# openGemini/openGemini

Hardware: NVIDIA B200
Metric: decoded+aggregated rows/s (higher is better)
Workload: dtype f64

## Files before the change

opengemini_b200/csrc/agg_kernels.cuh:

```cuda
#pragma once
#include "agg_ops.cuh"
#include "decode.cuh"
#include "internal.h"

namespace ogpu {

#define OG_NO_BUCKET 0xFFFFFFFFu

struct DirP {
    const uint8_t *data;
    const uint64_t *page_off;
    const uint32_t *page_len;
    const uint32_t *seg_series, *seg_rows, *series_seg_begin;
    const int64_t *seg_tmin, *seg_tmax;
    uint32_t n_segments, n_columns;
};

struct ChunkP {
    uint32_t series_begin, series_end;
    uint32_t seg_begin, seg_end;
    Tri cells[OG_MAX_CALLS];
    uint32_t nb;
    Tri edges[OG_MAX_CALLS];
    uint32_t *edge_bucket;
    Tri gcells[OG_MAX_CALLS];
    uint32_t gc_cols, gc_edge0, gc_col0;
    uint32_t J;
    int *err;
    int *flags;
};

__device__ __forceinline__ size_t cell_idx(const ChunkP &ch, uint32_t series, uint32_t b) { return (size_t)(series - ch.series_begin) * ch.nb + b; }

__device__ __forceinline__ void report_err(int *err, int code, uint32_t seg) {
    if (atomicCAS(&err[0], 0, code) == 0) err[1] = (int)seg;
}

__device__ __forceinline__ void store_part(const Tri &a, size_t i, const Part &p) {
    a.val[i] = p.v; a.ok[i] = (uint8_t)p.ok;
    if (a.tim) a.tim[i] = p.t;
}
__device__ __forceinline__ Part load_part(const Tri &a, size_t i) {
    Part p; p.ok = a.ok[i]; p.v = a.val[i]; p.t = a.tim ? a.tim[i] : 0; return p;
}
__device__ __forceinline__ void store_cell(const ChunkP &ch, int call, uint32_t series, uint32_t b, const Part &p) {
    store_part(ch.cells[call], cell_idx(ch, series, b), p);
    ch.flags[0] = 1;
}

struct LastTime { int64_t last; int unsorted = 0; __device__ __forceinline__ void operator()(uint32_t i, int64_t t) { if (i && t < last) unsorted = 1; last = t; } };

__global__ void k_validate(DirP d, const int32_t *col_types, uint32_t *seg_rows, unsigned long long *totals ,
                           uint32_t *max_rows, int *err) {
    uint32_t seg = blockIdx.x * blockDim.x + threadIdx.x;
    if (seg >= d.n_segments) return;
    size_t ti = (size_t)d.n_columns * d.n_segments + seg;
    TimeDesc t;
    int rc = parse_time_page(d.data + d.page_off[ti], d.page_len[ti], t);
    if (rc == D_OK && t.rows == 0) rc = D_CORRUPT;
    if (rc == D_OK) {
        LastTime lt; lt.last = t.t0;
        if (t.kind == 0) lt.last = (int64_t)((uint64_t)t.t0 + (uint64_t)(t.rows - 1) * t.delta);
        else rc = decode_time_values(t, lt);
        if (rc == D_OK && (t.t0 < d.seg_tmin[seg] || lt.last > d.seg_tmax[seg] || lt.last < t.t0 || lt.unsorted)) rc = D_CORRUPT;
    }
    if (rc != D_OK) { report_err(err, rc, seg); seg_rows[seg] = 0; return; }
    seg_rows[seg] = t.rows;
    unsigned long long bytes = d.page_len[ti];
    for (uint32_t c = 0; c < d.n_columns; c++) {
        size_t pi = (size_t)c * d.n_segments + seg;
        uint32_t len = d.page_len[pi];
        if (len == 0) continue;
        bytes += len;
        PageHdr h;
        rc = parse_field_header(d.data + d.page_off[pi], len, col_types[c], t.rows, h);
        if (rc == D_OK && h.rows != t.rows) rc = D_CORRUPT;
        if (rc == D_OK && !h.one_row && h.nil_count < h.rows) {
            if (h.block_len < 1) rc = D_CORRUPT;
            else {
                int tag = __ldg(h.block) >> 4, ty = col_types[c];
                if (ty == OG_TYPE_FLOAT) rc = (tag == 0 || tag == 3 || tag == 4 || tag == 5) ? D_OK : (tag == 1 || tag == 2 || tag == 6) ? D_UNSUPPORTED : D_CORRUPT;
                else if (ty == OG_TYPE_INT) rc = (tag == 1 || tag == 2 || tag == 4) ? D_OK : tag == 3 ? D_UNSUPPORTED : D_CORRUPT;
                else if (ty == OG_TYPE_BOOL) rc = tag == 1 ? D_OK : D_CORRUPT;
                else if (ty == OG_TYPE_STRING) rc = D_OK;
                else rc = D_UNSUPPORTED;
            }
        }
        if (rc != D_OK) { report_err(err, rc, seg); return; }
    }
    atomicAdd(&totals[0], (unsigned long long)t.rows);
    atomicAdd(&totals[1], bytes);
    atomicMax(max_rows, t.rows);
    if (t.kind != 0 && t.kind != 3) atomicAdd(&totals[2], 1ull);
}

__global__ void k_fill_seg_series(const uint32_t *series_seg_begin, uint32_t n_series, uint32_t *seg_series) {
    uint32_t s = blockIdx.x;
    if (s >= n_series) return;
    for (uint32_t g = series_seg_begin[s] + threadIdx.x; g < series_seg_begin[s + 1]; g += blockDim.x) seg_series[g] = s;
}

struct TileP {
    uint32_t tile_begin, tile_end, R;
    uint32_t S;
    uint64_t *vals[OG_MAX_COLS];
    uint8_t *okb[OG_MAX_COLS];
    int64_t *times;
    uint8_t *keep;
};

struct ExpandEmit {
    uint64_t *out; uint8_t *okb; const PageHdr *h; uint32_t row; size_t stride;
    __device__ __forceinline__ void operator()(uint32_t, uint64_t bits) {
        while (row < h->rows && !hdr_row_valid(*h, row)) { out[row * stride] = 0; okb[row * stride] = 0; row++; }
        if (row < h->rows) { out[row * stride] = bits; okb[row * stride] = 1; row++; }
    }
};
struct TimeStore { int64_t *out; size_t stride; __device__ __forceinline__ void operator()(uint32_t i, int64_t t) { out[i * stride] = t; } };

__global__ void k_decode_tile(DirP d, QueryP q, TileP tp, int *err) {
    uint32_t seg = tp.tile_begin + blockIdx.x * blockDim.x + threadIdx.x;
    if (seg >= tp.tile_end) return;
    uint32_t slot = blockIdx.y;
    const size_t base = seg - tp.tile_begin, S = tp.S;
    uint32_t rows = d.seg_rows[seg];
    if (slot == q.n_cols) {
        size_t ti = (size_t)d.n_columns * d.n_segments + seg;
        TimeDesc t;
        int rc = parse_time_page(d.data + d.page_off[ti], d.page_len[ti], t);
        if (rc == D_OK) { TimeStore ts{tp.times + base, S}; rc = decode_time_values(t, ts); }
        if (rc != D_OK) report_err(err, rc, seg);
        return;
    }
    int col = q.col_index[slot], type = q.col_type[slot];
    size_t pi = (size_t)col * d.n_segments + seg;
    uint64_t *out = tp.vals[slot] + base; uint8_t *okb = tp.okb[slot] + base;
    uint32_t len = d.page_len[pi];
    if (len == 0) { for (uint32_t i = 0; i < rows; i++) { out[i * S] = 0; okb[i * S] = 0; } return; }
    PageHdr h;
    int rc = parse_field_header(d.data + d.page_off[pi], len, type, rows, h);
    if (rc == D_OK) {
        ExpandEmit em{out, okb, &h, 0, S};
        rc = decode_block(type, h, em);
        for (uint32_t i = em.row; i < rows; i++) { out[i * S] = 0; okb[i * S] = 0; }
    }
    if (rc != D_OK) report_err(err, rc, seg);
}

__device__ __forceinline__ bool term_pass(const FilterP &f, uint64_t raw) {
    if (f.type == OG_TYPE_FLOAT || (f.type == OG_TYPE_INT && f.const_is_float)) {
        double v = f.type == OG_TYPE_FLOAT ? u2d(raw) : (double)(int64_t)raw;
        double c = f.const_is_float ? f.fval : (double)f.ival;
        switch (f.op) {
        case OG_OP_LT: return !(v >= c);
        case OG_OP_LTE: return !(v > c);
        case OG_OP_GT: return !(v <= c);
        case OG_OP_GTE: return !(v < c);
        case OG_OP_EQ: return !(v != c);
        default: return !(v == c);
        }
    }
    int64_t v = f.type == OG_TYPE_BOOL ? (int64_t)(raw != 0) : (int64_t)raw, c = f.ival;
    switch (f.op) {
    case OG_OP_LT: return !(v >= c);
    case OG_OP_LTE: return !(v > c);
    case OG_OP_GT: return !(v <= c);
    case OG_OP_GTE: return !(v < c);
    case OG_OP_EQ: return !(v != c);
    default: return !(v == c);
    }
}

__global__ void k_filter_tile(DirP d, QueryP q, TileP tp) {
    size_t idx = (size_t)blockIdx.x * blockDim.x + threadIdx.x;
    size_t total = (size_t)tp.S * tp.R;
    if (idx >= total) return;
    uint32_t row = (uint32_t)(idx / tp.S), sl = (uint32_t)(idx % tp.S);
    if (sl >= tp.tile_end - tp.tile_begin) return;
    if (row >= d.seg_rows[tp.tile_begin + sl]) { tp.keep[idx] = 0; return; }
    int64_t t = tp.times[idx];
    bool keep = t >= q.tmin && t <= q.tmax;
    if (keep && q.n_filter) {
        uint32_t stack = 0; int sp = 0;
        for (uint32_t i = 0; i < q.n_filter; i++) {
            const FilterP &f = q.filter[i];
            if (f.kind == OG_F_TERM) {
                bool pass = tp.okb[f.col_slot][idx] && term_pass(f, tp.vals[f.col_slot][idx]);
                stack |= (uint32_t)pass << sp; sp++;
            } else {
                uint32_t b = (stack >> (sp - 1)) & 1, a = (stack >> (sp - 2)) & 1;
                uint32_t r = f.kind == OG_F_AND ? (a & b) : (a | b);
                sp -= 2; stack &= ~(3u << sp); stack |= r << sp; sp++;
            }
        }
        keep = stack & 1;
    }
    tp.keep[idx] = keep;
}

__device__ __forceinline__ void emit_window(const QueryP &q, const ChunkP &ch, uint32_t seg, uint32_t series, uint32_t b,
                                            bool is_head, bool is_tail, int call, const Part &p) {
    if (is_head) store_part(ch.edges[call], 2 * (size_t)(seg - ch.seg_begin), p);
    else if (is_tail) store_part(ch.edges[call], 2 * (size_t)(seg - ch.seg_begin) + 1, p);
    else if (p.ok) store_cell(ch, call, series, b, p);
}

__global__ void k_window_reduce(DirP d, QueryP q, TileP tp, ChunkP ch) {
    uint32_t sl = blockIdx.x * blockDim.x + threadIdx.x;
    uint32_t seg = tp.tile_begin + sl;
    if (seg >= tp.tile_end) return;
    const uint32_t rows = d.seg_rows[seg], series = d.seg_series[seg];
    const size_t S = tp.S, e = 2 * (size_t)(seg - ch.seg_begin);
    Part parts[OG_MAX_CALLS];
    uint32_t cur_b = OG_NO_BUCKET, head_b = OG_NO_BUCKET; bool head_done = false;
    int64_t we = 0;
    auto flush = [&](bool final) {
        if (cur_b == OG_NO_BUCKET) return;
        for (uint32_t c = 0; c < q.n_calls; c++) {
            if (!head_done) store_part(ch.edges[c], e, parts[c]);
            else if (final) store_part(ch.edges[c], e + 1, parts[c]);
            else if (parts[c].ok) store_cell(ch, (int)c, series, cur_b, parts[c]);
        }
        if (!head_done) { head_done = true; head_b = cur_b; }
    };
    for (uint32_t r = 0; r < rows; r++) {
        const size_t ix = (size_t)r * S + sl;
        const int64_t t = tp.times[ix];
        if (t < q.tmin) continue;
        if (t > q.tmax) break;
        if (cur_b == OG_NO_BUCKET || t >= we) {
            flush(false);
            cur_b = bucket_of(t, q.start, q.interval);
            if (cur_b >= q.n_buckets) { report_err(ch.err, D_CORRUPT, seg); cur_b = OG_NO_BUCKET; break; }
            we = q.start + (int64_t)(cur_b + 1) * q.interval;
#pragma unroll
            for (uint32_t c = 0; c < OG_MAX_CALLS; c++) parts[c] = part_empty();
        }
        if (!tp.keep[ix]) continue;
#pragma unroll
        for (uint32_t c = 0; c < OG_MAX_CALLS; c++) {
            if (c >= q.n_calls) break;
            const CallP &cp = q.calls[c];
            if (tp.okb[cp.col_slot][ix]) acc_row(cp.func, cp.type, parts[c], tp.vals[cp.col_slot][ix], t);
        }
    }
    flush(true);
    ch.edge_bucket[e] = head_b;
    ch.edge_bucket[e + 1] = (head_b == OG_NO_BUCKET || cur_b == head_b) ? OG_NO_BUCKET : cur_b;
}

struct EdgeRuns { uint32_t hb, tb, s_end; bool head_leader; };
__device__ __forceinline__ EdgeRuns edge_runs(const DirP &d, const ChunkP &ch, uint32_t seg, uint32_t series) {
    EdgeRuns r;
    const uint32_t s_first = d.series_seg_begin[series];
    r.s_end = d.series_seg_begin[series + 1];
    const uint32_t *eb = ch.edge_bucket;
    const size_t e = 2 * (size_t)(seg - ch.seg_begin);
    r.hb = eb[e]; r.tb = eb[e + 1];
    r.head_leader = true;
    if (r.hb != OG_NO_BUCKET && seg > s_first) {
        const size_t pe = e - 2;
        const uint32_t pb = eb[pe + 1] != OG_NO_BUCKET ? eb[pe + 1] : eb[pe];
        if (pb != OG_NO_BUCKET && pb == r.hb) r.head_leader = false;
    }
    return r;
}
__device__ __forceinline__ Part edge_stitch(const QueryP &q, const ChunkP &ch, const EdgeRuns &r, uint32_t seg, int which, uint32_t c) {
    const CallP &cp = q.calls[c];
    const uint32_t *eb = ch.edge_bucket;
    const size_t e = 2 * (size_t)(seg - ch.seg_begin);
    const uint32_t b = which == 0 ? r.hb : r.tb;
    Part acc = load_part(ch.edges[c], e + which);
    if (which == 1 || r.tb == OG_NO_BUCKET) {
        for (uint32_t nx = seg + 1; nx < r.s_end; nx++) {
            const size_t ne = 2 * (size_t)(nx - ch.seg_begin);
            if (eb[ne] != b) break;
            acc = series_merge(cp.func, cp.type, acc, load_part(ch.edges[c], ne));
            if (eb[ne + 1] != OG_NO_BUCKET) break;
        }
    }
    return acc;
}

__global__ void k_fix_edges(DirP d, QueryP q, ChunkP ch) {
    uint32_t seg = ch.seg_begin + blockIdx.x * blockDim.x + threadIdx.x;
    if (seg >= ch.seg_end) return;
    const uint32_t series = d.seg_series[seg];
    const EdgeRuns r = edge_runs(d, ch, seg, series);
    if (r.hb == OG_NO_BUCKET) return;
    for (int which = 0; which < 2; which++) {
        if (which == 0 && !r.head_leader) continue;
        if (which == 1 && r.tb == OG_NO_BUCKET) continue;
        const uint32_t b = which == 0 ? r.hb : r.tb;
        if (b >= q.n_buckets) { report_err(ch.err, D_CORRUPT, seg); continue; }
        for (uint32_t c = 0; c < q.n_calls; c++) {
            const Part acc = edge_stitch(q, ch, r, seg, which, c);
            if (acc.ok) store_cell(ch, (int)c, series, b, acc);
        }
    }
}

__device__ __forceinline__ Part shfl_xor_part(const Part &p, int o, bool with_time) {
    Part r; r.v = __shfl_xor_sync(0xffffffffu, p.v, o); r.ok = __shfl_xor_sync(0xffffffffu, p.ok, o);
    r.t = with_time ? __shfl_xor_sync(0xffffffffu, p.t, o) : 0;
    return r;
}
__device__ __forceinline__ Part warp_fold(int func, int type, bool multi, Part p, bool with_time) {
#pragma unroll
    for (int o = 16; o; o >>= 1) { const Part other = shfl_xor_part(p, o, with_time); group_update(func, type, multi, p, other); }
    return p;
}
__device__ __forceinline__ bool call_has_time(const QueryP &q, uint32_t c) { return q.calls[c].func >= OG_AGG_MIN && !(q.multi && q.calls[c].func <= OG_AGG_MAX); }
__device__ __forceinline__ int call_ftype(const QueryP &q, uint32_t c) { return q.calls[c].func == OG_AGG_COUNT ? OG_TYPE_INT : q.calls[c].type; }

__global__ void k_fix_edges_fold(DirP d, QueryP q, ChunkP ch) {
    const uint32_t w = (blockIdx.x * blockDim.x + threadIdx.x) >> 5, lane = threadIdx.x & 31;
    const uint32_t n_blk = (ch.series_end - ch.series_begin + 31) / 32;
    if (w >= n_blk * ch.J) return;
    const uint32_t blk = w / ch.J, j = w % ch.J;
    const uint32_t series = ch.series_begin + blk * 32 + lane;
    const bool in = series < ch.series_end;
    const uint32_t seg = in ? d.series_seg_begin[series] + j : 0;
    EdgeRuns r; r.hb = r.tb = OG_NO_BUCKET; r.head_leader = false; r.s_end = 0;
    if (in) r = edge_runs(d, ch, seg, series);
    const uint32_t gcol = ch.gc_edge0 + ch.series_begin / 32 + blk - ch.gc_col0;
    for (int which = 0; which < 2; which++) {
        const bool has = r.hb != OG_NO_BUCKET && (which == 0 ? r.head_leader : r.tb != OG_NO_BUCKET);
        const uint32_t b = which == 0 ? r.hb : r.tb;
        const uint32_t hm = __ballot_sync(0xffffffffu, has);
        if (hm == 0) continue;
        const int leader = __ffs(hm) - 1;
        const uint32_t bL = __shfl_sync(0xffffffffu, b, leader);
        const bool unif = __all_sync(0xffffffffu, !has || b == bL) && bL < q.n_buckets;
        if (!unif && has && b >= q.n_buckets) { report_err(ch.err, D_CORRUPT, seg); continue; }
        for (uint32_t c = 0; c < q.n_calls; c++) {
            Part acc = part_empty();
            if (has) acc = edge_stitch(q, ch, r, seg, which, c);
            if (unif) {
                acc = warp_fold(q.calls[c].func, call_ftype(q, c), q.multi != 0, acc, call_has_time(q, c));
                if ((int)lane == leader && acc.ok) store_part(ch.gcells[c], (size_t)bL * ch.gc_cols + gcol, acc);
            } else if (has && acc.ok) store_cell(ch, (int)c, series, b, acc);
        }
    }
}

struct GroupP {
    const uint32_t *grp_begin;
    const uint32_t *grp_series;
    uint32_t n_groups;
    Tri dense[OG_MAX_CALLS];
};

__global__ void k_merge_groups(QueryP q, ChunkP ch, GroupP gp) {
    if (ch.flags[0] == 0) return;
    size_t idx = (size_t)blockIdx.x * blockDim.x + threadIdx.x;
    size_t total = (size_t)gp.n_groups * q.n_buckets;
    if (idx >= total) return;
    uint32_t g = (uint32_t)(idx / q.n_buckets), b = (uint32_t)(idx % q.n_buckets);
    uint32_t lo = gp.grp_begin[g], hi = gp.grp_begin[g + 1];
    {
        uint32_t a = lo, z = hi;
        while (a < z) { uint32_t m = (a + z) >> 1; if (gp.grp_series[m] < ch.series_begin) a = m + 1; else z = m; }
        lo = a;
    }
    if (lo >= hi || gp.grp_series[lo] >= ch.series_end) return;
    {
        const uint32_t c = blockIdx.y;
        const CallP &cp = q.calls[c];
        Part acc = load_part(gp.dense[c], idx);
        const Tri cells = ch.cells[c];
        constexpr int U = 16;
        for (uint32_t i = lo; i < hi; i += U) {
            uint32_t okv[U]; uint64_t vv[U]; int64_t tt[U];
#pragma unroll
            for (int u = 0; u < U; u++) {
                uint32_t ii = i + u;
                uint32_t s = ii < hi ? gp.grp_series[ii] : 0xffffffffu;
                bool in = s < ch.series_end;
                size_t ci = in ? cell_idx(ch, s, b) : 0;
                okv[u] = in ? cells.ok[ci] : 0;
                vv[u] = okv[u] ? cells.val[ci] : 0;
                tt[u] = (okv[u] && cells.tim) ? cells.tim[ci] : 0;
            }
#pragma unroll
            for (int u = 0; u < U; u++) {
                if (!okv[u]) continue;
                Part p; p.ok = 1; p.v = vv[u]; p.t = tt[u];
                group_update(cp.func, cp.out_type == OG_TYPE_INT && cp.func == OG_AGG_COUNT ? OG_TYPE_INT : cp.type, q.multi != 0, acc, p);
            }
        }
        store_part(gp.dense[c], idx, acc);
    }
}

__global__ void k_merge_per_series(QueryP q, ChunkP ch, GroupP gp) {
    const uint32_t c = blockIdx.y;
    const size_t n = (size_t)(ch.series_end - ch.series_begin) * q.n_buckets;
    const size_t i = (size_t)blockIdx.x * blockDim.x + threadIdx.x;
    if (i >= n) return;
    const CallP &cp = q.calls[c];
    const int ftype = cp.out_type == OG_TYPE_INT && cp.func == OG_AGG_COUNT ? OG_TYPE_INT : cp.type;
    const uint32_t b = (uint32_t)(i % q.n_buckets);
    Part p; p.ok = ch.cells[c].ok[i]; p.v = p.ok ? ch.cells[c].val[i] : 0; p.t = (p.ok && ch.cells[c].tim) ? ch.cells[c].tim[i] : 0;
    Part a; a.v = 0; a.ok = 0; a.t = q.multi ? 0 : q.start + (int64_t)b * q.interval;
    group_update(cp.func, ftype, q.multi != 0, a, p);
    store_part(gp.dense[c], (size_t)ch.series_begin * q.n_buckets + i, a);
}

#define OG_MERGE_SB 256u
__global__ void __launch_bounds__(128) k_merge_all_blocks(QueryP q, ChunkP ch, GroupP gp) {
    if (ch.flags[0] == 0) return;
    const uint32_t b = blockIdx.x * blockDim.x + threadIdx.x, blk = blockIdx.y, c = blockIdx.z;
    if (b >= q.n_buckets) return;
    const uint32_t nS = ch.series_end - ch.series_begin;
    const uint32_t s0 = blk * OG_MERGE_SB, s1 = min(nS, s0 + OG_MERGE_SB);
    const int func = q.calls[c].func, ftype = call_ftype(q, c);
    const bool multi = q.multi != 0;
    const Tri cells = ch.cells[c];
    Part acc = part_empty();
    constexpr int U = 8;
    for (uint32_t s = s0; s < s1; s += U) {
        uint32_t okv[U]; uint64_t vv[U]; int64_t tt[U];
#pragma unroll
        for (int u = 0; u < U; u++) {
            const bool in = s + u < s1;
            const size_t ci = in ? (size_t)(s + u) * ch.nb + b : 0;
            okv[u] = in ? cells.ok[ci] : 0;
            vv[u] = okv[u] ? cells.val[ci] : 0;
            tt[u] = (okv[u] && cells.tim) ? cells.tim[ci] : 0;
        }
#pragma unroll
        for (int u = 0; u < U; u++) {
            if (!okv[u]) continue;
            Part p; p.ok = 1; p.v = vv[u]; p.t = tt[u];
            group_update(func, ftype, multi, acc, p);
        }
    }
    if (acc.ok) store_part(ch.gcells[c], (size_t)b * ch.gc_cols + blk, acc);
}

__global__ void k_merge_folded(QueryP q, ChunkP ch, GroupP gp) {
    const uint32_t b = (blockIdx.x * blockDim.x + threadIdx.x) >> 5, lane = threadIdx.x & 31, c = blockIdx.y;
    if (b >= q.n_buckets) return;
    const int func = q.calls[c].func, ftype = call_ftype(q, c);
    const bool wt = call_has_time(q, c), multi = q.multi != 0;
    const Tri g = ch.gcells[c];
    Part acc = part_empty();
    const size_t row = (size_t)b * ch.gc_cols;
    for (uint32_t col = lane; col < ch.gc_cols; col += 32) {
        if (!g.ok[row + col]) continue;
        Part p; p.ok = 1; p.v = g.val[row + col]; p.t = wt ? g.tim[row + col] : 0;
        group_update(func, ftype, multi, acc, p);
    }
    acc = warp_fold(func, ftype, multi, acc, wt);
    if (lane == 0 && acc.ok) {
        Part a = load_part(gp.dense[c], b);
        group_update(func, ftype, multi, a, acc);
        store_part(gp.dense[c], b, a);
    }
}

__global__ void k_init_dense(QueryP q, GroupP gp) {
    size_t idx = (size_t)blockIdx.x * blockDim.x + threadIdx.x;
    size_t total = (size_t)gp.n_groups * q.n_buckets;
    if (idx >= total) return;
    uint32_t b = (uint32_t)(idx % q.n_buckets);
    for (uint32_t c = 0; c < q.n_calls; c++) {
        gp.dense[c].val[idx] = 0; gp.dense[c].ok[idx] = 0;
        if (gp.dense[c].tim) gp.dense[c].tim[idx] = q.multi ? 0 : q.start + (int64_t)b * q.interval;
    }
}

__global__ void k_merge_dense(QueryP q, GroupP mine, GroupP other) {
    size_t idx = (size_t)blockIdx.x * blockDim.x + threadIdx.x;
    size_t total = (size_t)mine.n_groups * q.n_buckets;
    if (idx >= total) return;
    for (uint32_t c = 0; c < q.n_calls; c++) {
        const CallP &cp = q.calls[c];
        Part a = load_part(mine.dense[c], idx), p = load_part(other.dense[c], idx);
        group_update(cp.func, cp.func == OG_AGG_COUNT ? OG_TYPE_INT : cp.type, q.multi != 0, a, p);
        store_part(mine.dense[c], idx, a);
    }
}

}
```

opengemini_b200/csrc/agg_ops.cuh:

```cuda
#pragma once
#include <cstdint>

#include "../../include/ogpu.h"

namespace ogpu {

__device__ __forceinline__ double u2d(uint64_t u) { return __longlong_as_double((long long)u); }
__device__ __forceinline__ uint64_t d2u(double d) { return (uint64_t)__double_as_longlong(d); }

__device__ __forceinline__ bool v_lt(int type, uint64_t a, uint64_t b) {
    if (type == OG_TYPE_FLOAT) return u2d(a) < u2d(b);
    if (type == OG_TYPE_INT) return (int64_t)a < (int64_t)b;
    return a != b && !a;
}
__device__ __forceinline__ bool v_gt(int type, uint64_t a, uint64_t b) {
    if (type == OG_TYPE_FLOAT) return u2d(a) > u2d(b);
    if (type == OG_TYPE_INT) return (int64_t)a > (int64_t)b;
    return a != b && a;
}
__device__ __forceinline__ bool v_eq(int type, uint64_t a, uint64_t b) { return type == OG_TYPE_FLOAT ? u2d(a) == u2d(b) : a == b; }
__device__ __forceinline__ bool v_le(int type, uint64_t a, uint64_t b) {
    if (type == OG_TYPE_FLOAT) return u2d(a) <= u2d(b);
    if (type == OG_TYPE_INT) return (int64_t)a <= (int64_t)b;
    return a == b || !a;
}
__device__ __forceinline__ bool v_ge(int type, uint64_t a, uint64_t b) {
    if (type == OG_TYPE_FLOAT) return u2d(a) >= u2d(b);
    if (type == OG_TYPE_INT) return (int64_t)a >= (int64_t)b;
    return a == b || a;
}

struct Part { uint64_t v; int64_t t; uint32_t ok; };

__device__ __forceinline__ void acc_row(int func, int type, Part &p, uint64_t v, int64_t t) {
    switch (func) {
    case OG_AGG_COUNT: p.v += 1; p.ok = 1; break;
    case OG_AGG_SUM:
        if (type == OG_TYPE_FLOAT) p.v = d2u(u2d(p.v) + u2d(v)); else p.v += v;
        p.ok = 1; break;
    case OG_AGG_MIN:
        if (!p.ok || v_gt(type, p.v, v)) { p.v = v; p.t = t; }
        p.ok = 1; break;
    case OG_AGG_MAX:
        if (!p.ok || v_lt(type, p.v, v)) { p.v = v; p.t = t; }
        p.ok = 1; break;
    case OG_AGG_FIRST: if (!p.ok) { p.v = v; p.t = t; p.ok = 1; } break;
    default: p.v = v; p.t = t; p.ok = 1; break;
    }
}
__device__ __forceinline__ Part part_empty() { Part p; p.v = 0; p.t = 0; p.ok = 0; return p; }

__device__ __forceinline__ Part series_merge(int func, int type, const Part &prev, const Part &curr) {
    if (!curr.ok) return prev;
    if (!prev.ok) return curr;
    Part r = prev;
    switch (func) {
    case OG_AGG_COUNT: r.v = prev.v + curr.v; break;
    case OG_AGG_SUM: r.v = type == OG_TYPE_FLOAT ? d2u(u2d(prev.v) + u2d(curr.v)) : prev.v + curr.v; break;
    case OG_AGG_MIN: if (v_lt(type, curr.v, prev.v)) r = curr; break;
    case OG_AGG_MAX: if (v_gt(type, curr.v, prev.v)) r = curr; break;
    case OG_AGG_FIRST: break;
    default: r = curr; break;
    }
    return r;
}

__device__ __forceinline__ void group_update(int func, int type, bool multi, Part &a, const Part &p) {
    if (!p.ok) return;
    switch (func) {
    case OG_AGG_COUNT: a.v = (uint64_t)((int64_t)p.v + (int64_t)a.v); a.ok = 1; return;
    case OG_AGG_SUM:
        a.v = type == OG_TYPE_FLOAT ? d2u(u2d(p.v) + u2d(a.v)) : p.v + a.v; a.ok = 1; return;
    case OG_AGG_MIN:
    case OG_AGG_MAX: {
        bool is_min = func == OG_AGG_MIN;
        if (multi) {
            if ((is_min ? v_le(type, a.v, p.v) : v_ge(type, a.v, p.v)) && a.ok) return;
            a.v = p.v; a.ok = 1; return;
        }
        if ((is_min ? v_lt(type, a.v, p.v) : v_gt(type, a.v, p.v)) && a.ok) return;
        bool t_le = type == OG_TYPE_FLOAT ? (__longlong_as_double(a.t) <= __longlong_as_double(p.t)) : (a.t <= p.t);
        if (v_eq(type, a.v, p.v) && t_le && a.ok) return;
        a = p; a.ok = 1; return;
    }
    default: {
        bool is_first = func == OG_AGG_FIRST;
        int64_t t1 = a.t, t2 = p.t;
        if (is_first ? (t1 > t2) : (t1 < t2)) { a = p; a.ok = 1; return; }
        if (a.ok && (is_first ? (t2 > t1) : (t2 < t1))) return;
        if (a.ok && v_ge(type, a.v, p.v)) return;
        a = p; a.ok = 1; return;
    }
    }
}

__device__ __forceinline__ uint32_t bucket_of(int64_t t, int64_t start, int64_t interval) {
    return (uint32_t)((uint64_t)(t - start) / (uint64_t)interval);
}

}
```

opengemini_b200/csrc/api.cu:

```cuda
#include <algorithm>
#include <cstdarg>
#include <cstdio>
#include <cstring>
#include <numeric>

#include "agg_kernels.cuh"
#include "fused.cuh"
#include "il_build.cuh"
#include "fused_multi.cuh"
#include "fused_cols.cuh"
#include "snappy_load.cuh"
#include <cub/device/device_scan.cuh>
#include <cub/device/device_radix_sort.cuh>
#include "internal.h"

namespace ogpu {

static thread_local char g_err[512] = "";
void set_error(const char *fmt, ...) {
    va_list ap; va_start(ap, fmt); vsnprintf(g_err, sizeof g_err, fmt, ap); va_end(ap);
}
int cuda_fail(cudaError_t e, const char *what, const char *file, int line) {
    set_error("CUDA error %d (%s) at %s:%d: %s", (int)e, cudaGetErrorString(e), file, line, what);
    return OG_E_CUDA;
}
static int g_device = -1;
cudaError_t dev_mem_info(size_t *free_b, size_t *total_b) {
    cudaError_t e = cudaMemGetInfo(free_b, total_b);
    if (e != cudaSuccess) return e;
    cudaMemPool_t pool; uint64_t reserved = 0, used = 0; int dev = 0;
    if (cudaGetDevice(&dev) == cudaSuccess && cudaDeviceGetDefaultMemPool(&pool, dev) == cudaSuccess &&
        cudaMemPoolGetAttribute(pool, cudaMemPoolAttrReservedMemCurrent, &reserved) == cudaSuccess &&
        cudaMemPoolGetAttribute(pool, cudaMemPoolAttrUsedMemCurrent, &used) == cudaSuccess && reserved > used) *free_b += (size_t)(reserved - used);
    else cudaGetLastError();
    return cudaSuccess;
}

static int map_dev_err(int code) {
    switch (code) {
    case D_UNSUPPORTED: return OG_E_UNSUPPORTED;
    case D_TYPE: return OG_E_TYPE;
    case D_WATCHDOG: return OG_E_CUDA;
    default: return OG_E_CORRUPT;
    }
}

template <class T> static int dalloc(T **p, size_t n) {
    *p = nullptr;
    if (n == 0) n = 1;
    cudaError_t e = dev_malloc((void **)p, n * sizeof(T));
    if (e != cudaSuccess) { set_error("cudaMalloc(%zu bytes) failed: %s", n * sizeof(T), cudaGetErrorString(e)); return e == cudaErrorMemoryAllocation ? OG_E_NOMEM : OG_E_CUDA; }
    return OG_OK;
}

static DirP make_dir(const og_shard *s) {
    DirP d;
    d.data = s->d_data; d.page_off = s->d_page_off; d.page_len = s->d_page_len; d.seg_series = s->d_seg_series;
    d.seg_rows = s->d_seg_rows; d.series_seg_begin = s->d_series_seg_begin; d.seg_tmin = s->d_tmin; d.seg_tmax = s->d_tmax;
    d.n_segments = s->n_segments; d.n_columns = s->n_columns;
    return d;
}

int shard_finalize(og_shard *s, bool scan_snappy) {
    int rc;
    s->il.resize(s->n_columns);
    if ((rc = dalloc(&s->d_seg_series, s->n_segments))) return rc;
    if ((rc = dalloc(&s->d_seg_rows, s->n_segments))) return rc;
    int32_t *d_types; unsigned long long *d_tot; uint32_t *d_max; int *d_err;
    if ((rc = dalloc(&d_types, s->n_columns))) return rc;
    if ((rc = dalloc(&d_tot, 3))) return rc;
    if ((rc = dalloc(&d_max, 1))) return rc;
    if ((rc = dalloc(&d_err, 2))) return rc;
    CU(cudaMemcpy(d_types, s->col_types.data(), s->n_columns * sizeof(int32_t), cudaMemcpyHostToDevice));
    CU(cudaMemset(d_tot, 0, 24)); CU(cudaMemset(d_max, 0, 4)); CU(cudaMemset(d_err, 0, 8));
    if (s->n_series) k_fill_seg_series<<<s->n_series, 128>>>(s->d_series_seg_begin, s->n_series, s->d_seg_series);
    if (s->n_segments && scan_snappy) {
        const size_t n_pages = (size_t)(s->n_columns + 1) * s->n_segments;
        uint32_t *tr_size; unsigned long long *d_cnt;
        if ((rc = dalloc(&tr_size, n_pages))) return rc;
        if ((rc = dalloc(&d_cnt, 3))) { dev_free(tr_size); return rc; }
        struct Free2 { void *a, *b; ~Free2() { dev_free(a); dev_free(b); } } f2{tr_size, d_cnt};
        CU(cudaMemset(d_cnt, 0, 24));
        k_snappy_scan<<<(s->n_segments + 127) / 128, 128>>>(make_dir(s), d_types, tr_size, d_cnt);
        unsigned long long cnt[3];
        CU(cudaMemcpy(cnt, d_cnt, 24, cudaMemcpyDeviceToHost));
        if (cnt[0]) {
            if (!s->owns_data) { set_error("shard has %llu Snappy pages: they are transcoded at open, which needs a library-owned copy of the data (do not pass OG_SHARD_DEVICE_DATA)", cnt[0]); return OG_E_UNSUPPORTED; }
            uint64_t *tr_off; void *tmp = nullptr; size_t tb = 0;
            if ((rc = dalloc(&tr_off, n_pages))) return rc;
            struct Free1 { void *a; ~Free1() { dev_free(a); } } f1{tr_off};
            CU(cub::DeviceScan::ExclusiveSum(nullptr, tb, tr_size, tr_off, (int)n_pages));
            CU(dev_malloc((void **)&tmp, tb ? tb : 1));
            struct Free3 { void *a; ~Free3() { dev_free(a); } } f3{tmp};
            CU(cub::DeviceScan::ExclusiveSum(tmp, tb, tr_size, tr_off, (int)n_pages));
            const uint64_t new_base = (s->data_len + 15) & ~15ull, new_len = new_base + cnt[2];
            uint8_t *nd;
            if ((rc = dalloc(&nd, (size_t)new_len + 1024))) return rc;
            CU(cudaMemcpy(nd, s->d_data, s->data_len, cudaMemcpyDeviceToDevice));
            CU(cudaMemset(nd + s->data_len, 0, new_len + 1024 - s->data_len));
            k_snappy_transcode<<<(unsigned)((n_pages + 127) / 128), 128>>>(make_dir(s), tr_size, tr_off, nd, new_base, s->d_page_off, s->d_page_len, d_err);
            CU(cudaGetLastError());
            CU(cudaDeviceSynchronize());
            dev_free(s->d_data); s->d_data = nd; s->data_len = new_len;
            s->snappy_pages = cnt[0]; s->snappy_bytes_in = cnt[1]; s->snappy_bytes_out = cnt[2];
        }
    }
    if (s->n_segments) k_validate<<<(s->n_segments + 127) / 128, 128>>>(make_dir(s), d_types, s->d_seg_rows, d_tot, d_max, d_err);
    CU(cudaGetLastError());
    unsigned long long tot[3]; int err[2]; uint32_t mx;
    CU(cudaMemcpy(tot, d_tot, 24, cudaMemcpyDeviceToHost));
    CU(cudaMemcpy(err, d_err, 8, cudaMemcpyDeviceToHost));
    CU(cudaMemcpy(&mx, d_max, 4, cudaMemcpyDeviceToHost));
    dev_free(d_types); dev_free(d_tot); dev_free(d_max); dev_free(d_err);
    if (err[0]) {
        set_error("segment %d: %s page (device validation code %d)", err[1], err[0] == D_UNSUPPORTED ? "unsupported codec in" : err[0] == D_TYPE ? "type mismatch in" : "corrupt", err[0]);
        return map_dev_err(err[0]);
    }
    s->n_rows = tot[0]; s->page_bytes = tot[1] - s->snappy_bytes_out + s->snappy_bytes_in;
    s->max_seg_rows = mx; s->irregular_time_pages = tot[2];
    return OG_OK;
}

}

using namespace ogpu;

extern "C" {

OG_API int og_device_count(void) { int n = 0; if (cudaGetDeviceCount(&n) != cudaSuccess) return 0; return n; }

OG_API int og_init(int device_ordinal) {
    int n = og_device_count();
    if (n <= 0) { set_error("no CUDA device visible: libogpu has no CPU path"); return OG_E_CUDA; }
    if (device_ordinal < 0 || device_ordinal >= n) { set_error("device ordinal %d out of range (%d devices)", device_ordinal, n); return OG_E_INVAL; }
    CU(cudaSetDevice(device_ordinal));
    CU(cudaFree(0));
    {
        cudaMemPool_t pool; uint64_t thr = ~0ull;
        if (cudaDeviceGetDefaultMemPool(&pool, device_ordinal) == cudaSuccess) cudaMemPoolSetAttribute(pool, cudaMemPoolAttrReleaseThreshold, &thr);
        else cudaGetLastError();
    }
    g_device = device_ordinal;
    return OG_OK;
}

OG_API const char *og_strerror(int st) {
    switch (st) {
    case OG_OK: return "ok";
    case OG_EOF: return "end of stream";
    case OG_E_INVAL: return "invalid argument";
    case OG_E_CUDA: return "CUDA failure or no device bound";
    case OG_E_NOMEM: return "out of device memory";
    case OG_E_UNSUPPORTED: return "unsupported codec or option on the GPU path";
    case OG_E_CORRUPT: return "corrupt page";
    case OG_E_ABORTED: return "query aborted";
    case OG_E_TYPE: return "column type mismatch";
    case OG_E_STATE: return "call sequence error";
    default: return "unknown status";
    }
}
OG_API const char *og_last_error(void) { return g_err; }
OG_API const char *og_version(void) { return "ogpu 0.2 (sm_100a)"; }
OG_API int og_release_cached_memory(void) {
    if (g_device < 0) return OG_OK;
    CU(cudaSetDevice(g_device));
    CU(cudaDeviceSynchronize());
    cudaMemPool_t pool;
    CU(cudaDeviceGetDefaultMemPool(&pool, g_device));
    CU(cudaMemPoolTrimTo(pool, 0));
    return OG_OK;
}

}
namespace ogpu {
int ensure_device() {
    if (g_device < 0) { int rc = og_init(0); if (rc != OG_OK) return rc; }
    else CU(cudaSetDevice(g_device));
    return OG_OK;
}
}
static int need_device() { return ogpu::ensure_device(); }
extern "C" {

OG_API void og_shard_close(og_shard *s) {
    if (!s) return;
    if (s->owns_data && s->d_data) dev_free(s->d_data);
    dev_free(s->d_series_seg_begin); dev_free(s->d_seg_series); dev_free(s->d_seg_rows); dev_free(s->d_tmin); dev_free(s->d_tmax);
    dev_free(s->d_page_off); dev_free(s->d_page_len); dev_free(s->d_sids);
    if (s->h_seg_buf) cudaFreeHost(s->h_seg_buf);
    if (s->d_seg_buf) dev_free(s->d_seg_buf);
    for (auto &c : s->il) {
        dev_free(c.words); dev_free(c.grp_off); dev_free(c.grp_rows); dev_free(c.grp_col); dev_free(c.ok); dev_free(c.lane_seg); dev_free(c.lane_rows);
        dev_free(c.lane_series); dev_free(c.lane_t0); dev_free(c.lane_dt); dev_free(c.gen_list);
    }
    delete s;
}

OG_API int og_shard_open(const og_shard_desc *d, og_shard **out) {
    if (!d || !out) { set_error("null argument"); return OG_E_INVAL; }
    *out = nullptr;
    int rc = need_device(); if (rc) return rc;
    if (d->n_columns > 64 || (d->n_segments && (!d->seg_tmin || !d->seg_tmax || !d->time_page_off || !d->time_page_len)) || (d->n_series && !d->series_seg_begin)) { set_error("bad shard descriptor"); return OG_E_INVAL; }
    for (uint32_t s = 0; s < d->n_series; s++) if (d->series_seg_begin[s] > d->series_seg_begin[s + 1]) { set_error("series_seg_begin not monotone at %u", s); return OG_E_INVAL; }
    if (d->n_series && d->series_seg_begin[d->n_series] != d->n_segments) { set_error("series_seg_begin[n_series] != n_segments"); return OG_E_INVAL; }
    og_shard *s = new og_shard;
    s->device = g_device; s->n_series = d->n_series; s->n_segments = d->n_segments; s->n_columns = d->n_columns;
    s->data_len = d->data_len;
    for (uint32_t c = 0; c < d->n_columns; c++) {
        s->col_types.push_back(d->columns[c].type);
        s->col_names.push_back(d->columns[c].name ? d->columns[c].name : "");
        if (d->columns[c].type != OG_TYPE_INT && d->columns[c].type != OG_TYPE_FLOAT && d->columns[c].type != OG_TYPE_BOOL && d->columns[c].type != OG_TYPE_STRING) {
            set_error("column %u: unknown column type %d", c, d->columns[c].type); delete s; return OG_E_UNSUPPORTED;
        }
    }
    s->sids.assign(d->sids, d->sids + d->n_series);
    s->h_series_seg_begin.assign(d->series_seg_begin, d->series_seg_begin + d->n_series + 1);
    size_t nseg = d->n_segments, ncol1 = (size_t)d->n_columns + 1;
    std::vector<uint64_t> off(ncol1 * nseg); std::vector<uint32_t> len(ncol1 * nseg);
    for (size_t c = 0; c < ncol1; c++) {
        const uint64_t *po = c < d->n_columns ? d->columns[c].page_off : d->time_page_off;
        const uint32_t *pl = c < d->n_columns ? d->columns[c].page_len : d->time_page_len;
        for (size_t g = 0; g < nseg; g++) {
            if (po[g] + pl[g] > d->data_len) { set_error("column %zu segment %zu: page [%llu,+%u) outside data (%llu bytes)", c, g, (unsigned long long)po[g], pl[g], (unsigned long long)d->data_len); delete s; return OG_E_INVAL; }
            off[c * nseg + g] = po[g]; len[c * nseg + g] = pl[g];
        }
    }
    s->tmin = INT64_MAX; s->tmax = INT64_MIN;
    for (uint32_t sr = 0; sr < d->n_series; sr++)
        for (uint32_t g = d->series_seg_begin[sr]; g < d->series_seg_begin[sr + 1]; g++) {
            if (d->seg_tmin[g] > d->seg_tmax[g] || (g > d->series_seg_begin[sr] && d->seg_tmin[g] <= d->seg_tmax[g - 1])) {
                set_error("series %u: segment %u is not time-ordered (only ordered TSSP files are supported)", sr, g); delete s; return OG_E_UNSUPPORTED;
            }
            s->tmin = std::min(s->tmin, d->seg_tmin[g]); s->tmax = std::max(s->tmax, d->seg_tmax[g]);
        }
#define TRY(x) do { rc = (x); if (rc) { og_shard_close(s); return rc; } } while (0)
#define TRYCU(x) do { cudaError_t e_ = (x); if (e_ != cudaSuccess) { rc = cuda_fail(e_, #x, __FILE__, __LINE__); og_shard_close(s); return rc; } } while (0)
    if (d->flags & OG_SHARD_DEVICE_DATA) { s->d_data = (uint8_t *)d->data; s->owns_data = false; }
    else {
        TRY(dalloc(&s->d_data, d->data_len + 1024));
        TRYCU(cudaMemcpy(s->d_data, d->data, d->data_len, cudaMemcpyHostToDevice));
        TRYCU(cudaMemset(s->d_data + d->data_len, 0, 1024));
    }
    TRY(dalloc(&s->d_series_seg_begin, (size_t)d->n_series + 1));
    TRY(dalloc(&s->d_tmin, nseg)); TRY(dalloc(&s->d_tmax, nseg));
    TRY(dalloc(&s->d_page_off, ncol1 * nseg)); TRY(dalloc(&s->d_page_len, ncol1 * nseg)); TRY(dalloc(&s->d_sids, (size_t)d->n_series));
    TRYCU(cudaMemcpy(s->d_series_seg_begin, d->series_seg_begin, ((size_t)d->n_series + 1) * 4, cudaMemcpyHostToDevice));
    TRYCU(cudaMemcpy(s->d_tmin, d->seg_tmin, nseg * 8, cudaMemcpyHostToDevice));
    TRYCU(cudaMemcpy(s->d_tmax, d->seg_tmax, nseg * 8, cudaMemcpyHostToDevice));
    TRYCU(cudaMemcpy(s->d_page_off, off.data(), off.size() * 8, cudaMemcpyHostToDevice));
    TRYCU(cudaMemcpy(s->d_page_len, len.data(), len.size() * 4, cudaMemcpyHostToDevice));
    TRYCU(cudaMemcpy(s->d_sids, d->sids, (size_t)d->n_series * 8, cudaMemcpyHostToDevice));
    TRY(shard_finalize(s, true));
    *out = s;
    return OG_OK;
}

OG_API int og_shard_info(const og_shard *s, uint64_t *n_series, uint64_t *n_segments, uint64_t *n_rows, uint64_t *page_bytes, int64_t *tmin, int64_t *tmax) {
    if (!s) return OG_E_INVAL;
    if (n_series) *n_series = s->n_series;
    if (n_segments) *n_segments = s->n_segments;
    if (n_rows) *n_rows = s->n_rows;
    if (page_bytes) *page_bytes = s->page_bytes;
    if (tmin) *tmin = s->tmin;
    if (tmax) *tmax = s->tmax;
    return OG_OK;
}

OG_API int og_shard_layout_get(const og_shard *s, og_shard_layout *out) {
    if (!s || !out) return OG_E_INVAL;
    out->data_len = s->data_len; out->n_series = s->n_series; out->n_segments = s->n_segments; out->n_columns = s->n_columns;
    return OG_OK;
}

OG_API int og_shard_export(const og_shard *s, uint8_t *data, uint64_t *sids, uint32_t *series_seg_begin, int64_t *seg_tmin,
                           int64_t *seg_tmax, uint64_t *page_off, uint32_t *page_len, int32_t *col_types) {
    if (!s) return OG_E_INVAL;
    CU(cudaSetDevice(s->device));
    size_t nseg = s->n_segments, ncol1 = (size_t)s->n_columns + 1;
    if (data) CU(cudaMemcpy(data, s->d_data, s->data_len, cudaMemcpyDeviceToHost));
    if (sids) memcpy(sids, s->sids.data(), s->sids.size() * 8);
    if (series_seg_begin) memcpy(series_seg_begin, s->h_series_seg_begin.data(), s->h_series_seg_begin.size() * 4);
    if (seg_tmin) CU(cudaMemcpy(seg_tmin, s->d_tmin, nseg * 8, cudaMemcpyDeviceToHost));
    if (seg_tmax) CU(cudaMemcpy(seg_tmax, s->d_tmax, nseg * 8, cudaMemcpyDeviceToHost));
    if (page_off) CU(cudaMemcpy(page_off, s->d_page_off, ncol1 * nseg * 8, cudaMemcpyDeviceToHost));
    if (page_len) CU(cudaMemcpy(page_len, s->d_page_len, ncol1 * nseg * 4, cudaMemcpyDeviceToHost));
    if (col_types) memcpy(col_types, s->col_types.data(), s->col_types.size() * 4);
    return OG_OK;
}

static const int64_t MIN_TIME = INT64_MIN + 2, MAX_TIME = INT64_MAX - 1;
static void window_of(int64_t interval, int64_t offset, int64_t tmin, int64_t tmax, int64_t t, int64_t *s, int64_t *e) {
    if (interval == 0) { *s = tmin; *e = tmax + 1; return; }
    t -= offset;
    int64_t dt = t % interval;
    if (dt < 0) dt += interval;
    int64_t st = ((int64_t)((uint64_t)MIN_TIME + (uint64_t)dt) >= t) ? MIN_TIME : t - dt;
    st += offset;
    int64_t d2 = interval - dt;
    int64_t en = (MAX_TIME - d2 <= t) ? MAX_TIME : t + d2;
    en += offset;
    *s = st; *e = en;
}

}
namespace { void free_plan(void *plan); }
extern "C" {
void og_query_free_merge_state(void *p);
OG_API void og_query_destroy(og_query *q) {
    if (!q) return;
    if (q->merge_state) og_query_free_merge_state(q->merge_state);
    free_plan(q->plan);
    for (void *p : q->scratch) dev_free(p);
    for (int c = 0; c < OG_MAX_CALLS; c++) { dev_free(q->dense[c].val); dev_free(q->dense[c].ok); dev_free(q->dense[c].tim); }
    dev_free(q->d_group_of_series);
    if (q->ev0) cudaEventDestroy(q->ev0);
    if (q->ev1) cudaEventDestroy(q->ev1);
    for (cudaEvent_t e : q->main_ev) cudaEventDestroy(e);
    if (q->stream) cudaStreamDestroy(q->stream);
    delete q;
}

OG_API int og_query_create(og_shard *s, const og_query_desc *d_in, og_query **out) {
    if (!s || !d_in || !out) { set_error("null argument"); return OG_E_INVAL; }
    *out = nullptr;
    og_query_desc d_clamped = *d_in;
    d_clamped.tmin = std::max(d_in->tmin, MIN_TIME); d_clamped.tmax = std::min(d_in->tmax, MAX_TIME);
    const og_query_desc *d = &d_clamped;
    CU(cudaSetDevice(s->device));
    if (d->n_calls == 0 || d->n_calls > OG_MAX_CALLS) { set_error("n_calls must be 1..%d", OG_MAX_CALLS); return OG_E_INVAL; }
    if (d->n_filter > OG_MAX_FILTER) { set_error("filter too long (max %d items)", OG_MAX_FILTER); return OG_E_INVAL; }
    if (d->interval < 0 || d->tmin > d->tmax) { set_error("bad interval or time range"); return OG_E_INVAL; }
    og_query *q = new og_query;
    q->sh = s; q->desc = *d;
    q->calls.assign(d->calls, d->calls + d->n_calls);
    if (d->n_filter) q->filter.assign(d->filter, d->filter + d->n_filter);
    q->desc.calls = q->calls.data(); q->desc.filter = q->filter.data();
    QueryP &p = q->qp;
    memset(&p, 0, sizeof p);
    auto slot_of = [&](int col) -> int {
        for (uint32_t i = 0; i < p.n_cols; i++) if (p.col_index[i] == col) return (int)i;
        if (p.n_cols >= OG_MAX_COLS) return -1;
        p.col_index[p.n_cols] = col; p.col_type[p.n_cols] = s->col_types[col];
        return (int)p.n_cols++;
    };
    for (uint32_t i = 0; i < d->n_calls; i++) {
        const og_call &c = d->calls[i];
        if (c.column < 0 || (uint32_t)c.column >= s->n_columns || c.func < OG_AGG_COUNT || c.func > OG_AGG_LAST) { set_error("call %u: bad column or function", i); delete q; return OG_E_INVAL; }
        int type = s->col_types[c.column];
        if (type == OG_TYPE_STRING && c.func != OG_AGG_COUNT) { set_error("call %u: only count() is pushed down for string columns (their values are never decoded on the GPU path)", i); delete q; return OG_E_UNSUPPORTED; }
        if (c.func == OG_AGG_SUM && type == OG_TYPE_BOOL) { set_error("sum() over a boolean column (unsupported sum iterator type, series_call_processor.go:140)"); delete q; return OG_E_INVAL; }
        int sl = slot_of(c.column);
        if (sl < 0) { set_error("too many distinct columns"); delete q; return OG_E_INVAL; }
        p.calls[i].func = c.func; p.calls[i].col_slot = sl; p.calls[i].type = type;
        p.calls[i].out_type = c.func == OG_AGG_COUNT ? OG_TYPE_INT : type;
    }
    p.n_calls = d->n_calls; p.multi = d->n_calls > 1;
    int sp = 0;
    for (uint32_t i = 0; i < d->n_filter; i++) {
        const og_filter_item &f = d->filter[i];
        FilterP &fp = p.filter[i];
        fp.kind = f.kind;
        if (f.kind == OG_F_TERM) {
            if (f.column < 0 || (uint32_t)f.column >= s->n_columns || f.op < OG_OP_LT || f.op > OG_OP_NEQ) { set_error("filter item %u: bad column or op", i); delete q; return OG_E_INVAL; }
            if (s->col_types[f.column] == OG_TYPE_STRING) { set_error("filter item %u: WHERE on a string column is not pushed down", i); delete q; return OG_E_UNSUPPORTED; }
            int sl = slot_of(f.column);
            if (sl < 0) { set_error("too many distinct columns"); delete q; return OG_E_INVAL; }
            fp.col_slot = sl; fp.op = f.op; fp.type = s->col_types[f.column]; fp.const_is_float = f.const_is_float; fp.fval = f.fval; fp.ival = f.ival;
            sp++;
        } else if (f.kind == OG_F_AND || f.kind == OG_F_OR) {
            if (sp < 2) { set_error("filter RPN underflow at item %u", i); delete q; return OG_E_INVAL; }
            sp--;
        } else { set_error("filter item %u: bad kind", i); delete q; return OG_E_INVAL; }
    }
    if (d->n_filter && sp != 1) { set_error("filter RPN does not reduce to one value"); delete q; return OG_E_INVAL; }
    p.n_filter = d->n_filter;
    int64_t gmin = std::max(d->tmin, s->tmin), gmax = std::min(d->tmax, s->tmax);
    if (gmin > gmax) gmin = gmax = d->tmin;
    if (d->flags & OG_Q_QUERY_GRID) {
        if (d_in->tmin <= MIN_TIME || d_in->tmax >= MAX_TIME) { set_error("OG_Q_QUERY_GRID needs a bounded time range"); delete q; return OG_E_INVAL; }
        gmin = d->tmin; gmax = d->tmax;
    }
    int64_t s0, e0, s1, e1;
    if (d->interval == 0) { s0 = gmin; e0 = gmax + 1; s1 = s0; e1 = e0; }
    else {
        window_of(d->interval, d->offset, d->tmin, d->tmax, gmin, &s0, &e0);
        window_of(d->interval, d->offset, d->tmin, d->tmax, gmax + 1, &s1, &e1);
    }
    p.tmin = d->tmin; p.tmax = d->tmax; p.start = s0; p.interval = e0 - s0;
    if (p.interval <= 0) { set_error("degenerate window"); delete q; return OG_E_INVAL; }
    uint64_t nb = d->interval ? (uint64_t)(e1 - s0) / (uint64_t)p.interval : 1;
    if (nb == 0 || nb > 0x7fffffffull) { set_error("query range yields %llu buckets", (unsigned long long)nb); delete q; return OG_E_INVAL; }
    p.n_buckets = (uint32_t)nb;
    q->n_groups = d->group_mode == OG_GROUP_ALL ? 1 : d->group_mode == OG_GROUP_PER_SERIES ? s->n_series : d->n_groups;
    if (d->group_mode == OG_GROUP_MAP) {
        if (!d->series_group || d->n_groups == 0) { set_error("OG_GROUP_MAP needs series_group and n_groups"); delete q; return OG_E_INVAL; }
        q->series_group.assign(d->series_group, d->series_group + s->n_series);
        for (uint32_t g : q->series_group) if (g >= d->n_groups) { set_error("series_group entry out of range"); delete q; return OG_E_INVAL; }
    } else if (d->group_mode != OG_GROUP_ALL && d->group_mode != OG_GROUP_PER_SERIES) { set_error("bad group_mode"); delete q; return OG_E_INVAL; }
    if (q->n_groups == 0) q->n_groups = 1;
    cudaError_t e = cudaStreamCreateWithFlags(&q->stream, cudaStreamNonBlocking);
    if (e != cudaSuccess) { delete q; return cuda_fail(e, "cudaStreamCreate", __FILE__, __LINE__); }
    cudaEventCreate(&q->ev0); cudaEventCreate(&q->ev1);
    *out = q;
    return OG_OK;
}

OG_API void og_query_abort(og_query *q) { if (q) q->aborted = 1; }

}
namespace {
struct Plan {
    ChunkP ch; TileP tp; GroupP gp;
    bool fused;
    bool cols;
    bool multi;
    bool fast;
    bool blockmerge;
    bool fold;
    int fm; bool times;
    IlP il;
    const og_shard::IlCol *ic;
};
void free_plan(void *plan) { delete (Plan *)plan; }
template <class T> int salloc(og_query *q, T **p, size_t n) { int rc = dalloc(p, n); if (rc == OG_OK) q->scratch.push_back(*p); return rc; }

template <int NC> void launch_fused(const DirP &d, const QueryP &p, const ChunkP &ch, const uint32_t *list, uint32_t n, cudaStream_t st) {
    if (n) k_fused_segment<NC><<<(n + 127) / 128, 128, 0, st>>>(d, p, ch, list, n);
}
template <int FM, bool TIMES> void launch_fast_t(bool fold, const IlP &il, uint32_t g0, uint32_t g1, const QueryP &p, const ChunkP &ch, cudaStream_t st) {
    constexpr uint32_t WPB = OG_FAST_THREADS / 32;
    dim3 grid((g1 - g0 + WPB - 1) / WPB), block(OG_FAST_THREADS);
    if (fold) k_fused_il<FM, TIMES, true><<<grid, block, WPB * il_acc_bytes(p.n_calls, TIMES), st>>>(p, ch, il, g0, g1);
    else k_fused_il<FM, TIMES, false><<<grid, block, 0, st>>>(p, ch, il, g0, g1);
}
void launch_fast(int fm, bool times, bool fold, const IlP &il, uint32_t g0, uint32_t g1, const QueryP &p, const ChunkP &ch, cudaStream_t st) {
    if (g1 <= g0) return;
    if (!times) {
        switch (fm) {
        case FM_SUM | FM_COUNT: return launch_fast_t<FM_SUM | FM_COUNT, false>(fold, il, g0, g1, p, ch, st);
        case FM_SUM | FM_COUNT | FM_MAX: return launch_fast_t<FM_SUM | FM_COUNT | FM_MAX, false>(fold, il, g0, g1, p, ch, st);
        case FM_SUM | FM_COUNT | FM_MIN | FM_MAX: return launch_fast_t<FM_SUM | FM_COUNT | FM_MIN | FM_MAX, false>(fold, il, g0, g1, p, ch, st);
        case FM_COUNT: return launch_fast_t<FM_COUNT, false>(fold, il, g0, g1, p, ch, st);
        default: break;
        }
    } else {
        switch (fm) {
        case FM_MAX | FM_COUNT: return launch_fast_t<FM_MAX | FM_COUNT, true>(fold, il, g0, g1, p, ch, st);
        case FM_MIN | FM_COUNT: return launch_fast_t<FM_MIN | FM_COUNT, true>(fold, il, g0, g1, p, ch, st);
        default: break;
        }
    }
    return launch_fast_t<63, true>(fold, il, g0, g1, p, ch, st);
}

template <int NCOL, int NCALL> void launch_multi_t(const QueryP &p, const DirP &d, const ChunkP &ch, uint32_t nseg, cudaStream_t st) {
    bool simple = true;
    for (uint32_t c = 0; c < p.n_calls; c++) simple &= p.calls[c].func == OG_AGG_COUNT || p.calls[c].func == OG_AGG_SUM;
    const unsigned gb = (nseg + 127) / 128;
    if (simple) k_fused_multi<NCOL, NCALL, true><<<gb, 128, 0, st>>>(d, p, ch);
    else k_fused_multi<NCOL, NCALL, false><<<gb, 128, 0, st>>>(d, p, ch);
}
template <int NCOL> void launch_multi_c(const QueryP &p, const DirP &d, const ChunkP &ch, uint32_t nseg, cudaStream_t st) {
    switch (p.n_calls) {
    case 1: return launch_multi_t<NCOL, 1>(p, d, ch, nseg, st);
    case 2: return launch_multi_t<NCOL, 2>(p, d, ch, nseg, st);
    case 3: return launch_multi_t<NCOL, 3>(p, d, ch, nseg, st);
    case 4: return launch_multi_t<NCOL, 4>(p, d, ch, nseg, st);
    case 5: return launch_multi_t<NCOL, 5>(p, d, ch, nseg, st);
    case 6: return launch_multi_t<NCOL, 6>(p, d, ch, nseg, st);
    case 7: return launch_multi_t<NCOL, 7>(p, d, ch, nseg, st);
    default: return launch_multi_t<NCOL, 8>(p, d, ch, nseg, st);
    }
}
void launch_cols(const QueryP &p, const DirP &d, const ChunkP &ch, uint32_t nseg, cudaStream_t st) {
    bool simple = true;
    for (uint32_t c = 0; c < p.n_calls; c++) simple &= p.calls[c].func == OG_AGG_COUNT || p.calls[c].func == OG_AGG_SUM;
    const unsigned gb = (nseg + 127) / 128;
    if (simple) k_fused_cols<true><<<gb, 128, 0, st>>>(d, p, ch);
    else k_fused_cols<false><<<gb, 128, 0, st>>>(d, p, ch);
}
void launch_multi(const QueryP &p, const DirP &d, const ChunkP &ch, uint32_t nseg, cudaStream_t st) {
    switch (p.n_cols) {
    case 1: return launch_multi_c<1>(p, d, ch, nseg, st);
    case 2: return launch_multi_c<2>(p, d, ch, nseg, st);
    case 3: return launch_multi_c<3>(p, d, ch, nseg, st);
    default: return launch_multi_c<4>(p, d, ch, nseg, st);
    }
}

struct TmpBufs { std::vector<void *> v; ~TmpBufs() { for (void *p : v) dev_free(p); } template <class T> int get(T **p, size_t n) { int rc = dalloc(p, n); if (rc == OG_OK) v.push_back(*p); return rc; } };

int ensure_il(og_shard *s, int col, cudaStream_t st) {
    std::lock_guard<std::mutex> lock(s->il_mu);
    if (s->il.size() != s->n_columns) s->il.resize(s->n_columns);
    og_shard::IlCol &ic = s->il[col];
    if (ic.state != 0) return OG_OK;
    ic.state = -1;
    if (s->n_segments == 0 || s->col_types[col] != OG_TYPE_FLOAT) return OG_OK;
    const uint32_t nseg = s->n_segments;
    uint32_t J = s->n_series ? s->h_series_seg_begin[1] - s->h_series_seg_begin[0] : 0;
    for (uint32_t i = 0; i < s->n_series && J; i++) if (s->h_series_seg_begin[i + 1] - s->h_series_seg_begin[i] != J) J = 0;
    const uint32_t n_super = J ? (s->n_series + OG_IL_SUPER - 1) / OG_IL_SUPER : 1;
    const uint64_t n_dom64 = J ? (uint64_t)n_super * J : 1;
    if (n_dom64 >= (1ull << 31)) return OG_OK;
    const uint32_t n_dom = (uint32_t)n_dom64;
    int rc;
    struct Ev { cudaEvent_t e = nullptr; Ev() { cudaEventCreate(&e); } ~Ev() { if (e) cudaEventDestroy(e); } } ev0, ev1;
    cudaEventRecord(ev0.e, st);
    TmpBufs tmp;
    IlScanOut so{};
    uint32_t *seg_words; uint64_t *keys2; uint32_t *vals2;
    if ((rc = dalloc(&ic.ok, (size_t)nseg))) return rc;
    so.ok = ic.ok;
    if ((rc = tmp.get(&seg_words, nseg)) || (rc = tmp.get(&so.seg_t0, nseg)) || (rc = tmp.get(&so.seg_dt, nseg)) || (rc = tmp.get(&so.keys, nseg)) ||
        (rc = tmp.get(&so.vals, nseg)) || (rc = tmp.get(&keys2, nseg)) || (rc = tmp.get(&vals2, nseg)) || (rc = tmp.get(&so.dom_cnt, n_dom))) return rc;
    so.seg_words = seg_words;
    CU(cudaMemsetAsync(so.dom_cnt, 0, (size_t)n_dom * 4, st));
    DirP d = make_dir(s);
    k_il_scan<<<(nseg + 255) / 256, 256, 0, st>>>(d, col, s->col_types[col], J, so);
    CU(cudaGetLastError());
    int dbits = 1; while ((1ull << dbits) < n_dom64 + 1) dbits++;
    {
        size_t tb = 0;
        CU(cub::DeviceRadixSort::SortPairs(nullptr, tb, so.keys, keys2, so.vals, vals2, (int)nseg, 0, (int)OG_IL_WORD_BITS + dbits, st));
        void *dtmp; if ((rc = tmp.get((uint8_t **)&dtmp, tb))) return rc;
        CU(cub::DeviceRadixSort::SortPairs(dtmp, tb, so.keys, keys2, so.vals, vals2, (int)nseg, 0, (int)OG_IL_WORD_BITS + dbits, st));
    }
    std::vector<uint32_t> dom_cnt(n_dom);
    CU(cudaMemcpyAsync(dom_cnt.data(), so.dom_cnt, (size_t)n_dom * 4, cudaMemcpyDeviceToHost, st));
    CU(cudaStreamSynchronize(st));
    std::vector<uint32_t> elem_first(n_dom), grp_first(n_dom);
    uint64_t n_elig = 0, ng64 = 0;
    for (uint32_t i = 0; i < n_dom; i++) { elem_first[i] = (uint32_t)n_elig; grp_first[i] = (uint32_t)ng64; n_elig += dom_cnt[i]; ng64 += (dom_cnt[i] + 31) / 32; }
    const uint32_t n_gen = nseg - (uint32_t)n_elig;
    if (n_gen) {
        if ((rc = dalloc(&ic.gen_list, (size_t)n_gen))) return rc;
        CU(cudaMemcpyAsync(ic.gen_list, vals2 + n_elig, (size_t)n_gen * 4, cudaMemcpyDeviceToDevice, st));
        ic.gen_host.resize(n_gen);
        CU(cudaMemcpyAsync(ic.gen_host.data(), vals2 + n_elig, (size_t)n_gen * 4, cudaMemcpyDeviceToHost, st));
        CU(cudaStreamSynchronize(st));
    }
    if (n_elig == 0) return OG_OK;
    const uint32_t ng = (uint32_t)ng64;
    ic.n_groups = ng; ic.J = J; ic.n_super = n_super; ic.cols_per_super = OG_IL_SUPER / 32 + 1;
    ic.super_grp_first.assign(n_super + 1, ng);
    for (uint32_t sp = 0; sp < n_super; sp++) ic.super_grp_first[sp] = grp_first[J ? sp * J : 0];
    uint32_t *d_elem_first, *d_grp_first;
    if ((rc = tmp.get(&d_elem_first, n_dom)) || (rc = tmp.get(&d_grp_first, n_dom))) return rc;
    CU(cudaMemcpyAsync(d_elem_first, elem_first.data(), (size_t)n_dom * 4, cudaMemcpyHostToDevice, st));
    CU(cudaMemcpyAsync(d_grp_first, grp_first.data(), (size_t)n_dom * 4, cudaMemcpyHostToDevice, st));
    const size_t n_slots = (size_t)ng * 32;
    if ((rc = dalloc(&ic.lane_seg, n_slots)) || (rc = dalloc(&ic.lane_rows, n_slots)) || (rc = dalloc(&ic.lane_series, n_slots)) ||
        (rc = dalloc(&ic.lane_t0, n_slots)) || (rc = dalloc(&ic.lane_dt, n_slots)) || (rc = dalloc(&ic.grp_col, (size_t)ng)) ||
        (rc = dalloc(&ic.grp_rows, (size_t)ng)) || (rc = dalloc(&ic.grp_off, (size_t)ng))) return rc;
    CU(cudaMemsetAsync(ic.lane_seg, 0xff, n_slots * 4, st));
    CU(cudaMemsetAsync(ic.lane_rows, 0, n_slots * 4, st));
    IlAssign as{};
    as.keys = keys2; as.segs = vals2; as.elem_first = d_elem_first; as.grp_first = d_grp_first;
    as.seg_words = seg_words; as.seg_t0 = so.seg_t0; as.seg_dt = so.seg_dt; as.ok = ic.ok;
    as.lane_seg = ic.lane_seg; as.lane_rows = ic.lane_rows; as.lane_series = ic.lane_series; as.grp_col = ic.grp_col; as.lane_t0 = ic.lane_t0; as.lane_dt = ic.lane_dt;
    as.n_elig = (uint32_t)n_elig; as.J = J; as.cols_per_super = ic.cols_per_super;
    k_il_assign<<<(unsigned)((n_elig + 255) / 256), 256, 0, st>>>(d, as);
    k_il_group_rows<<<(unsigned)((n_slots + 255) / 256), 256, 0, st>>>(ng, ic.lane_seg, seg_words, ic.grp_rows);
    CU(cudaGetLastError());
    std::vector<uint32_t> gw(ng); std::vector<uint64_t> go(ng);
    CU(cudaMemcpyAsync(gw.data(), ic.grp_rows, (size_t)ng * 4, cudaMemcpyDeviceToHost, st));
    CU(cudaStreamSynchronize(st));
    uint64_t total = 0;
    for (uint32_t g = 0; g < ng; g++) { go[g] = total; total += (uint64_t)gw[g] * 32; }
    size_t free_b = 0, total_b = 0;
    CU(dev_mem_info(&free_b, &total_b));
    size_t headroom = (size_t)8 << 30;
    if (const char *ov = getenv("OGPU_IL_HEADROOM_MB")) headroom = (size_t)atoll(ov) << 20;
    if (total * 4 + headroom > free_b || dev_malloc((void **)&ic.words, total * 4) != cudaSuccess) {
        cudaGetLastError(); ic.words = nullptr; ic.state = -2;
        return OG_OK;
    }
    CU(cudaMemcpyAsync(ic.grp_off, go.data(), (size_t)ng * 8, cudaMemcpyHostToDevice, st));
    k_il_repack<<<(unsigned)((n_slots + 127) / 128), 128, 0, st>>>(d, col, ic.ok, ic.lane_seg, ic.grp_off, ic.grp_rows, ng, ic.words);
    CU(cudaGetLastError());
    cudaEventRecord(ev1.e, st);
    CU(cudaStreamSynchronize(st));
    float ms = 0; cudaEventElapsedTime(&ms, ev0.e, ev1.e);
    ic.n_words = total; ic.build_ms = ms; ic.state = 1;
    return OG_OK;
}

int build_plan(og_query *q) {
    og_shard *s = q->sh;
    const QueryP &p = q->qp;
    cudaStream_t st = q->stream;
    int rc;
    Plan *pl = new Plan;
    memset((void *)pl, 0, sizeof *pl);
    q->plan = pl;
    size_t cells_dense = (size_t)q->n_groups * p.n_buckets;
    for (uint32_t c = 0; c < p.n_calls; c++) {
        bool sel = p.calls[c].func >= OG_AGG_MIN && !(p.multi && p.calls[c].func <= OG_AGG_MAX);
        if ((rc = dalloc(&q->dense[c].val, cells_dense))) return rc;
        if ((rc = dalloc(&q->dense[c].ok, cells_dense))) return rc;
        if (sel && (rc = dalloc(&q->dense[c].tim, cells_dense))) return rc;
    }
    std::vector<uint32_t> grp_begin(q->n_groups + 1, 0), grp_series(s->n_series);
    if (q->desc.group_mode == OG_GROUP_MAP) {
        for (uint32_t sr = 0; sr < s->n_series; sr++) grp_begin[q->series_group[sr] + 1]++;
        for (uint32_t g = 0; g < q->n_groups; g++) grp_begin[g + 1] += grp_begin[g];
        std::vector<uint32_t> cur(grp_begin.begin(), grp_begin.end() - 1);
        for (uint32_t sr = 0; sr < s->n_series; sr++) grp_series[cur[q->series_group[sr]]++] = sr;
    } else if (q->desc.group_mode == OG_GROUP_PER_SERIES) {
        for (uint32_t g = 0; g <= q->n_groups; g++) grp_begin[g] = std::min(g, s->n_series);
        std::iota(grp_series.begin(), grp_series.end(), 0u);
    } else { grp_begin[1] = s->n_series; std::iota(grp_series.begin(), grp_series.end(), 0u); }
    uint32_t *d_grp_begin, *d_grp_series;
    if ((rc = salloc(q, &d_grp_begin, grp_begin.size()))) return rc;
    if ((rc = salloc(q, &d_grp_series, grp_series.size()))) return rc;
    if ((rc = salloc(q, &q->d_err, 8))) return rc;
    CU(cudaMemcpyAsync(d_grp_begin, grp_begin.data(), grp_begin.size() * 4, cudaMemcpyHostToDevice, st));
    CU(cudaMemcpyAsync(d_grp_series, grp_series.data(), grp_series.size() * 4, cudaMemcpyHostToDevice, st));
    CU(cudaStreamSynchronize(st));
    pl->gp.grp_begin = d_grp_begin; pl->gp.grp_series = d_grp_series; pl->gp.n_groups = q->n_groups;
    for (uint32_t c = 0; c < p.n_calls; c++) pl->gp.dense[c] = q->dense[c];

    bool has_string = false;
    for (uint32_t k = 0; k < p.n_cols; k++) has_string |= p.col_type[k] == OG_TYPE_STRING;
    pl->fused = p.n_cols == 1 && p.n_filter == 0 && !has_string && !(q->desc.flags & OG_Q_NO_FUSED);
    const bool multi_ok = !pl->fused && (has_string || !(q->desc.flags & OG_Q_NO_FUSED));
    pl->cols = false;
    if (multi_ok && !(q->desc.flags & OG_Q_NO_FAST) && s->irregular_time_pages == 0 && s->max_seg_rows <= OG_COLS_MAXROWS &&
        (p.n_filter == 0 || (p.n_filter == 1 && p.filter[0].kind == OG_F_TERM)) && !getenv("OGPU_NO_COLS")) {
        pl->cols = true;
        for (uint32_t k = 0; k < p.n_cols; k++) {
            int n = 0;
            for (uint32_t c = 0; c < p.n_calls; c++) n += p.calls[c].col_slot == (int)k;
            if (n > OG_COLS_MAXMINE) pl->cols = false;
        }
    }
    if (has_string && !pl->cols && p.n_cols > OG_MULTI_MAXC) { set_error("a query that counts a string column may touch at most %d columns on this shard", OG_MULTI_MAXC); return OG_E_UNSUPPORTED; }
    pl->multi = pl->cols || (multi_ok && p.n_cols <= OG_MULTI_MAXC);
    q->path_used = pl->fused ? 1 : pl->cols ? 5 : pl->multi ? 4 : 0;
    const bool want_fast = pl->fused && p.col_type[0] == OG_TYPE_FLOAT && !(q->desc.flags & OG_Q_NO_FAST) && s->n_segments;
    if (want_fast && (rc = ensure_il(s, p.col_index[0], st))) return rc;
    pl->fast = want_fast && s->il[p.col_index[0]].state == 1;
    const og_shard::IlCol *ic = pl->fast ? &s->il[p.col_index[0]] : nullptr;
    pl->ic = ic;
    pl->fold = pl->fast && ic->J != 0 && q->desc.group_mode == OG_GROUP_ALL && !(q->desc.flags & OG_Q_STRICT_ORDER);

    size_t cell_bytes_per_series = 0;
    for (uint32_t c = 0; c < p.n_calls; c++) cell_bytes_per_series += (size_t)p.n_buckets * (9 + (p.calls[c].func >= OG_AGG_MIN ? 8 : 0));
    size_t free_b = 0, total_b = 0;
    CU(dev_mem_info(&free_b, &total_b));
    size_t budget = std::min<size_t>(free_b / 3, (size_t)24 << 30);
    q->chunk_series = (uint32_t)std::max<size_t>(1, std::min<size_t>(s->n_series, budget / std::max<size_t>(1, cell_bytes_per_series)));
    if (const char *ov = getenv("OGPU_CHUNK_SERIES")) {
        long v = atol(ov);
        if (v > 0) q->chunk_series = (uint32_t)std::min<long>(v, (long)std::max<uint32_t>(1, s->n_series));
    }
    if (q->chunk_series < s->n_series) {
        if (q->chunk_series >= OG_IL_SUPER) q->chunk_series = q->chunk_series / OG_IL_SUPER * OG_IL_SUPER;
        else q->chunk_series = std::max<uint32_t>(32, q->chunk_series & ~31u);
    }
    uint32_t max_chunk_segs = 0;
    for (uint32_t a = 0; a < s->n_series; a += q->chunk_series) {
        uint32_t b = std::min(s->n_series, a + q->chunk_series);
        max_chunk_segs = std::max(max_chunk_segs, s->h_series_seg_begin[b] - s->h_series_seg_begin[a]);
    }
    ChunkP &ch = pl->ch;
    ch.err = q->d_err; ch.flags = q->d_err + 2;
    ch.nb = p.n_buckets;
    ch.J = ic ? ic->J : 0;
    size_t chunk_cells = (size_t)std::min(q->chunk_series, s->n_series) * p.n_buckets;
    for (uint32_t c = 0; c < p.n_calls; c++) {
        bool sel = p.calls[c].func >= OG_AGG_MIN;
        if ((rc = salloc(q, &ch.cells[c].val, chunk_cells))) return rc;
        if ((rc = salloc(q, &ch.cells[c].ok, chunk_cells))) return rc;
        if (sel && (rc = salloc(q, &ch.cells[c].tim, chunk_cells))) return rc;
        if ((rc = salloc(q, &ch.edges[c].val, 2 * (size_t)max_chunk_segs))) return rc;
        if ((rc = salloc(q, &ch.edges[c].ok, 2 * (size_t)max_chunk_segs))) return rc;
        if (sel && (rc = salloc(q, &ch.edges[c].tim, 2 * (size_t)max_chunk_segs))) return rc;
    }
    if ((rc = salloc(q, &ch.edge_bucket, 2 * (size_t)max_chunk_segs))) return rc;
    pl->blockmerge = !pl->fold && q->desc.group_mode == OG_GROUP_ALL && !(q->desc.flags & OG_Q_STRICT_ORDER) &&
                     (s->n_series > 2 * OG_MERGE_SB || getenv("OGPU_FORCE_BLOCKMERGE") );
    if (pl->blockmerge) {
        ch.gc_edge0 = 0; ch.gc_col0 = 0;
        ch.gc_cols = (std::min(q->chunk_series, s->n_series) + OG_MERGE_SB - 1) / OG_MERGE_SB;
        const size_t n = (size_t)p.n_buckets * ch.gc_cols;
        for (uint32_t c = 0; c < p.n_calls; c++) {
            bool sel = p.calls[c].func >= OG_AGG_MIN;
            if ((rc = salloc(q, &ch.gcells[c].val, n))) return rc;
            if ((rc = salloc(q, &ch.gcells[c].ok, n))) return rc;
            if (sel && (rc = salloc(q, &ch.gcells[c].tim, n))) return rc;
        }
    }
    if (pl->fold) {
        ch.gc_edge0 = ic->n_super * ic->cols_per_super; ch.gc_col0 = 0;
        ch.gc_cols = ch.gc_edge0 + (s->n_series + 31) / 32;
        const size_t n = (size_t)p.n_buckets * ch.gc_cols;
        for (uint32_t c = 0; c < p.n_calls; c++) {
            bool sel = p.calls[c].func >= OG_AGG_MIN;
            if ((rc = salloc(q, &ch.gcells[c].val, n))) return rc;
            if ((rc = salloc(q, &ch.gcells[c].ok, n))) return rc;
            if (sel && (rc = salloc(q, &ch.gcells[c].tim, n))) return rc;
        }
    }
    if (pl->fast) {
        pl->il.words = ic->words; pl->il.grp_off = ic->grp_off; pl->il.grp_rows = ic->grp_rows; pl->il.grp_col = ic->grp_col;
        pl->il.lane_seg = ic->lane_seg; pl->il.lane_rows = ic->lane_rows; pl->il.lane_series = ic->lane_series; pl->il.lane_t0 = ic->lane_t0; pl->il.lane_dt = ic->lane_dt;
        pl->fm = 0; pl->times = false;
        for (uint32_t c = 0; c < p.n_calls; c++) {
            pl->fm |= 1 << (p.calls[c].func - 1);
            if (p.calls[c].func >= OG_AGG_MIN && !(p.multi && p.calls[c].func <= OG_AGG_MAX)) pl->times = true;
        }
        pl->fm |= FM_COUNT;
        q->path_used = pl->fold ? 3 : 2;
    }
    if (!pl->fused && !pl->multi) {
        TileP &tp = pl->tp;
        tp.R = std::max<uint32_t>(1, s->max_seg_rows);
        size_t per_seg = (size_t)tp.R * (p.n_cols * 9 + 8 + 1);
        size_t fb = 0, tb = 0;
        CU(dev_mem_info(&fb, &tb));
        const size_t tile_budget = std::max<size_t>((size_t)96 << 20, std::min<size_t>(fb / 4, (size_t)12 << 30));
        q->tile_segs = (uint32_t)std::max<size_t>(1, std::min<size_t>(std::max<uint32_t>(1, max_chunk_segs), tile_budget / per_seg));
        q->tile_segs = std::max<uint32_t>(32, q->tile_segs & ~31u);
        tp.S = q->tile_segs;
        for (uint32_t k = 0; k < p.n_cols; k++) {
            if ((rc = salloc(q, &tp.vals[k], (size_t)q->tile_segs * tp.R))) return rc;
            if ((rc = salloc(q, &tp.okb[k], (size_t)q->tile_segs * tp.R))) return rc;
        }
        if ((rc = salloc(q, &tp.times, (size_t)q->tile_segs * tp.R))) return rc;
        if ((rc = salloc(q, &tp.keep, (size_t)q->tile_segs * tp.R))) return rc;
    }
    q->planned = true;
    return OG_OK;
}
}
extern "C" {

OG_API int og_query_run(og_query *q) {
    if (!q) return OG_E_INVAL;
    og_shard *s = q->sh;
    CU(cudaSetDevice(s->device));
    const QueryP &p = q->qp;
    cudaStream_t st = q->stream;
    int rc;
    q->host_ready = false; q->next_group = 0; q->next_row = 0;
    if (!q->planned) {
        if (q->plan) { set_error("query plan failed earlier"); return OG_E_STATE; }
        if ((rc = build_plan(q))) return rc;
    }
    Plan *pl = (Plan *)q->plan;
    ChunkP ch = pl->ch; TileP tp = pl->tp; const GroupP &gp = pl->gp;
    size_t cells_dense = (size_t)q->n_groups * p.n_buckets;
    DirP dir = make_dir(s);
    uint32_t launches = 0, n_chunks = (s->n_series + q->chunk_series - 1) / q->chunk_series;
    while (q->main_ev.size() < 2 * (size_t)n_chunks) { cudaEvent_t e; CU(cudaEventCreate(&e)); q->main_ev.push_back(e); }
    CU(cudaMemsetAsync(q->d_err, 0, 32, st));
    CU(cudaEventRecord(q->ev0, st));
    const bool per_series = q->desc.group_mode == OG_GROUP_PER_SERIES;
    if (!per_series) { k_init_dense<<<(unsigned)((cells_dense + 255) / 256), 256, 0, st>>>(p, gp); launches++; }
    const bool clear_cells = !pl->fold || q->cells_dirty || n_chunks > 1;
    uint64_t segs_scanned = 0; uint32_t ci = 0, chunks_run = 0;
    for (uint32_t a = 0; a < s->n_series; a += q->chunk_series, ci++) {
        if (q->aborted) { cudaStreamSynchronize(st); set_error("query aborted"); return OG_E_ABORTED; }
        uint32_t b = std::min(s->n_series, a + q->chunk_series);
        ch.series_begin = a; ch.series_end = b;
        ch.seg_begin = s->h_series_seg_begin[a]; ch.seg_end = s->h_series_seg_begin[b];
        uint32_t nseg = ch.seg_end - ch.seg_begin;
        const size_t chunk_cells = (size_t)(b - a) * p.n_buckets;
        if (nseg == 0) {
            if (per_series) {
                for (uint32_t c = 0; c < p.n_calls; c++) CU(cudaMemsetAsync(ch.cells[c].ok, 0, chunk_cells, st));
                k_merge_per_series<<<dim3((unsigned)((chunk_cells + 255) / 256), p.n_calls), 256, 0, st>>>(p, ch, gp);
                launches++;
            }
            continue;
        }
        segs_scanned += nseg;
        if (clear_cells) for (uint32_t c = 0; c < p.n_calls; c++) CU(cudaMemsetAsync(ch.cells[c].ok, 0, chunk_cells, st));
        if (pl->fold || pl->blockmerge) for (uint32_t c = 0; c < p.n_calls; c++) CU(cudaMemsetAsync(ch.gcells[c].ok, 0, (size_t)p.n_buckets * ch.gc_cols, st));
        CU(cudaEventRecord(q->main_ev[2 * chunks_run], st));
        if (pl->fused) {
            const uint32_t *gl = nullptr; uint32_t gn = nseg;
            if (pl->fast) {
                const og_shard::IlCol &ic = *pl->ic;
                uint32_t g0 = 0, g1 = ic.n_groups;
                if (ic.J) { g0 = ic.super_grp_first[a / OG_IL_SUPER]; g1 = ic.super_grp_first[std::min<uint32_t>(ic.n_super, (b + OG_IL_SUPER - 1) / OG_IL_SUPER)]; }
                launch_fast(pl->fm, pl->times, pl->fold, pl->il, g0, g1, p, ch, st); launches++;
                auto lo = std::lower_bound(ic.gen_host.begin(), ic.gen_host.end(), ch.seg_begin);
                auto hi = std::lower_bound(ic.gen_host.begin(), ic.gen_host.end(), ch.seg_end);
                gl = ic.gen_list + (lo - ic.gen_host.begin()); gn = (uint32_t)(hi - lo);
            }
            if (gn) {
                switch (p.n_calls) {
                case 1: launch_fused<1>(dir, p, ch, gl, gn, st); break;
                case 2: launch_fused<2>(dir, p, ch, gl, gn, st); break;
                case 3: launch_fused<3>(dir, p, ch, gl, gn, st); break;
                case 4: launch_fused<4>(dir, p, ch, gl, gn, st); break;
                case 5: launch_fused<5>(dir, p, ch, gl, gn, st); break;
                case 6: launch_fused<6>(dir, p, ch, gl, gn, st); break;
                case 7: launch_fused<7>(dir, p, ch, gl, gn, st); break;
                default: launch_fused<8>(dir, p, ch, gl, gn, st); break;
                }
                launches++;
            }
        } else if (pl->cols) {
            launch_cols(p, dir, ch, nseg, st);
        } else if (pl->multi) {
            launch_multi(p, dir, ch, nseg, st);
            launches++;
        } else {
            for (uint32_t t0 = ch.seg_begin; t0 < ch.seg_end; t0 += q->tile_segs) {
                tp.tile_begin = t0; tp.tile_end = std::min(ch.seg_end, t0 + q->tile_segs);
                uint32_t n = tp.tile_end - tp.tile_begin;
                dim3 g((n + 127) / 128, p.n_cols + 1);
                k_decode_tile<<<g, 128, 0, st>>>(dir, p, tp, q->d_err);
                size_t rows_total = (size_t)tp.S * tp.R;
                k_filter_tile<<<(unsigned)((rows_total + 255) / 256), 256, 0, st>>>(dir, p, tp);
                k_window_reduce<<<(n + 127) / 128, 128, 0, st>>>(dir, p, tp, ch);
                launches += 3;
            }
        }
        CU(cudaEventRecord(q->main_ev[2 * chunks_run + 1], st));
        chunks_run++;
        if (pl->fold) k_fix_edges_fold<<<(unsigned)(((size_t)((b - a + 31) / 32) * ch.J * 32 + 127) / 128), 128, 0, st>>>(dir, p, ch);
        else k_fix_edges<<<(nseg + 127) / 128, 128, 0, st>>>(dir, p, ch);
        if (per_series) k_merge_per_series<<<dim3((unsigned)((chunk_cells + 255) / 256), p.n_calls), 256, 0, st>>>(p, ch, gp);
        else if (pl->blockmerge) k_merge_all_blocks<<<dim3((p.n_buckets + 127) / 128, (b - a + OG_MERGE_SB - 1) / OG_MERGE_SB, p.n_calls), 128, 0, st>>>(p, ch, gp);
        else k_merge_groups<<<dim3((unsigned)((cells_dense + 127) / 128), p.n_calls), 128, 0, st>>>(p, ch, gp);
        launches += 2;
        if (pl->fold || pl->blockmerge) { k_merge_folded<<<dim3((unsigned)(((size_t)p.n_buckets * 32 + 127) / 128), p.n_calls), 128, 0, st>>>(p, ch, gp); launches++; }
    }
    CU(cudaEventRecord(q->ev1, st));
    CU(cudaGetLastError());
    CU(cudaStreamSynchronize(st));
    int err[8];
    CU(cudaMemcpy(err, q->d_err, 32, cudaMemcpyDeviceToHost));
    if (getenv("OGPU_IL_STATS")) fprintf(stderr, "[ogpu] fused rounds: common %d rare %d (lanes not resident in %d, sit-outs %d)\n", err[4], err[5], err[6], err[7]);
    q->cells_dirty = err[2] != 0;
    if (err[0]) { set_error("segment %d failed to decode (device code %d)", err[1], err[0]); return map_dev_err(err[0]); }
    float ms = 0; cudaEventElapsedTime(&ms, q->ev0, q->ev1);
    double main_ms = 0;
    for (uint32_t i = 0; i < chunks_run; i++) { float m = 0; cudaEventElapsedTime(&m, q->main_ev[2 * i], q->main_ev[2 * i + 1]); main_ms += m; }
    og_stats &stt = q->stats;
    uint64_t keep_pb = stt.page_bytes, keep_rows = stt.rows_decoded, keep_segs = stt.segments_scanned;
    memset(&stt, 0, sizeof stt);
    stt.kernel_ms = ms; stt.main_kernel_ms = main_ms; stt.kernel_launches = launches; stt.path = q->path_used;
    stt.page_bytes = keep_pb; stt.rows_decoded = keep_pb ? keep_rows : s->n_rows; stt.segments_scanned = keep_pb ? keep_segs : segs_scanned;
    stt.dir_bytes = (uint64_t)segs_scanned * 32;
    stt.out_bytes = 0;
    for (uint32_t c = 0; c < p.n_calls; c++) stt.out_bytes += cells_dense * (9 + (q->dense[c].tim ? 8 : 0));
    if (p.n_cols == 1 && p.col_type[0] == OG_TYPE_FLOAT && p.col_index[0] < (int)s->il.size()) {
        const og_shard::IlCol &ic = s->il[p.col_index[0]];
        stt.il_state = ic.state; stt.il_build_ms = ic.build_ms; stt.il_bytes = ic.n_words * 4;
        stt.general_segments = ic.state == 1 ? (uint64_t)ic.gen_host.size() : s->n_segments;
    }
    stt.per_series_cells_used = err[2] != 0;
    q->ran = true;
    return OG_OK;
}

OG_API int og_query_dense(og_query *q, og_dense_view *out) {
    if (!q || !out) return OG_E_INVAL;
    if (!q->ran) { set_error("og_query_dense before og_query_run"); return OG_E_STATE; }
    const QueryP &p = q->qp;
    out->n_groups = q->n_groups; out->n_buckets = p.n_buckets; out->start = q->desc.interval ? p.start : 0; out->interval = q->desc.interval ? p.interval : 0;
    out->n_cols = p.n_calls;
    for (uint32_t c = 0; c < p.n_calls; c++) {
        q->dense_cols[c].values = q->dense[c].val; q->dense_cols[c].valid = q->dense[c].ok; q->dense_cols[c].times = q->dense[c].tim;
        q->dense_cols[c].type = p.calls[c].out_type; q->dense_cols[c].func = p.calls[c].func;
    }
    out->cols = q->dense_cols; out->stream = q->stream;
    return OG_OK;
}

}
namespace {
__global__ void k_sum_page_bytes(DirP d, QueryP q, int64_t tmin, int64_t tmax, unsigned long long *out ) {
    uint32_t seg = blockIdx.x * blockDim.x + threadIdx.x;
    if (seg >= d.n_segments) return;
    if (d.seg_tmax[seg] < tmin || d.seg_tmin[seg] > tmax) return;
    unsigned long long b = d.page_len[(size_t)d.n_columns * d.n_segments + seg];
    for (uint32_t k = 0; k < q.n_cols; k++) b += d.page_len[(size_t)q.col_index[k] * d.n_segments + seg];
    atomicAdd(&out[0], b); atomicAdd(&out[1], (unsigned long long)d.seg_rows[seg]); atomicAdd(&out[2], 1ull);
}
}
extern "C" {

OG_API int og_query_stats(const og_query *q, og_stats *out) {
    if (!q || !out) return OG_E_INVAL;
    og_query *mq = const_cast<og_query *>(q);
    if (q->ran && q->stats.page_bytes == 0) {
        CU(cudaSetDevice(q->sh->device));
        unsigned long long *d_o; int rc = dalloc(&d_o, 3); if (rc) return rc;
        cudaMemset(d_o, 0, 24);
        if (q->sh->n_segments) k_sum_page_bytes<<<(q->sh->n_segments + 255) / 256, 256>>>(make_dir(q->sh), q->qp, q->qp.tmin, q->qp.tmax, d_o);
        unsigned long long h[3]; CU(cudaMemcpy(h, d_o, 24, cudaMemcpyDeviceToHost)); dev_free(d_o);
        mq->stats.page_bytes = h[0]; mq->stats.rows_decoded = h[1]; mq->stats.segments_scanned = h[2];
    }
    *out = q->stats;
    return OG_OK;
}

OG_API int og_query_merge_dense(og_query *q, const og_dense_view *other) {
    if (!q || !other) return OG_E_INVAL;
    if (!q->ran) return OG_E_STATE;
    const QueryP &p = q->qp;
    if (other->n_groups != q->n_groups || other->n_buckets != p.n_buckets || other->n_cols != p.n_calls) { set_error("dense shapes differ"); return OG_E_INVAL; }
    if (other->start != (q->desc.interval ? p.start : 0) || other->interval != (q->desc.interval ? p.interval : 0)) {
        set_error("dense grids differ (start %lld vs %lld, interval %lld vs %lld): create the queries with OG_Q_QUERY_GRID", (long long)other->start,
                  (long long)(q->desc.interval ? p.start : 0), (long long)other->interval, (long long)(q->desc.interval ? p.interval : 0));
        return OG_E_INVAL;
    }
    CU(cudaSetDevice(q->sh->device));
    GroupP mine, oth; memset(&mine, 0, sizeof mine); memset(&oth, 0, sizeof oth);
    mine.n_groups = oth.n_groups = q->n_groups;
    for (uint32_t c = 0; c < p.n_calls; c++) {
        mine.dense[c] = q->dense[c];
        oth.dense[c].val = (uint64_t *)other->cols[c].values; oth.dense[c].ok = other->cols[c].valid; oth.dense[c].tim = other->cols[c].times;
        if ((q->dense[c].tim != nullptr) != (oth.dense[c].tim != nullptr)) { set_error("dense column %u: times presence differs", c); return OG_E_INVAL; }
    }
    size_t total = (size_t)q->n_groups * p.n_buckets;
    k_merge_dense<<<(unsigned)((total + 255) / 256), 256, 0, q->stream>>>(p, mine, oth);
    CU(cudaGetLastError());
    CU(cudaStreamSynchronize(q->stream));
    q->host_ready = false;
    return OG_OK;
}

OG_API int og_query_next(og_query *q, og_record_view *out) {
    if (!q || !out) return OG_E_INVAL;
    if (!q->ran) { set_error("og_query_next before og_query_run"); return OG_E_STATE; }
    if (q->aborted) return OG_E_ABORTED;
    const QueryP &p = q->qp;
    size_t total = (size_t)q->n_groups * p.n_buckets;
    if (!q->host_ready) {
        CU(cudaSetDevice(q->sh->device));
        for (uint32_t c = 0; c < p.n_calls; c++) {
            q->h_val[c].resize(total); q->h_ok[c].resize(total);
            CU(cudaMemcpy(q->h_val[c].data(), q->dense[c].val, total * 8, cudaMemcpyDeviceToHost));
            CU(cudaMemcpy(q->h_ok[c].data(), q->dense[c].ok, total, cudaMemcpyDeviceToHost));
            if (q->dense[c].tim) { q->h_tim[c].resize(total); CU(cudaMemcpy(q->h_tim[c].data(), q->dense[c].tim, total * 8, cudaMemcpyDeviceToHost)); }
        }
        q->host_ready = true; q->next_group = 0; q->next_row = 0;
    }
    int chunk = q->desc.chunk_size > 0 ? q->desc.chunk_size : 1024;
    uint32_t nc = p.n_calls;
    q->rv_val.assign(nc, {}); q->rv_bitmap.assign(nc, {}); q->rv_coltimes.assign(nc, {}); q->rv_times.clear(); q->rv_cols.assign(nc, og_colval_view{});
    while (q->next_group < q->n_groups) {
        uint32_t g = q->next_group;
        std::vector<int32_t> nil(nc, 0);
        int rows = 0;
        uint32_t b = q->next_row;
        uint32_t b_end = (uint32_t)std::min<uint64_t>(p.n_buckets, (uint64_t)b + (uint64_t)chunk);
        for (; b < b_end; b++) {
            const uint32_t bb = q->desc.ascending ? b : p.n_buckets - 1 - b;
            size_t i = (size_t)g * p.n_buckets + bb;
            bool any = false;
            for (uint32_t c = 0; c < nc; c++) any |= q->h_ok[c][i] != 0;
            if (!any) continue;
            int64_t row_time = p.start + (int64_t)bb * p.interval;
            if (q->desc.interval == 0) row_time = 0;
            for (uint32_t c = 0; c < nc; c++) {
                bool ok = q->h_ok[c][i] != 0;
                if ((size_t)(rows >> 3) >= q->rv_bitmap[c].size()) q->rv_bitmap[c].push_back(0);
                if (ok) {
                    q->rv_bitmap[c][rows >> 3] |= (uint8_t)(1 << (rows & 7));
                    if (p.calls[c].out_type == OG_TYPE_BOOL) q->rv_val[c].push_back((uint8_t)(q->h_val[c][i] != 0));
                    else { const uint8_t *pv = (const uint8_t *)&q->h_val[c][i]; q->rv_val[c].insert(q->rv_val[c].end(), pv, pv + 8); }
                } else nil[c]++;
                if (q->dense[c].tim) {
                    if (p.multi) q->rv_coltimes[c].push_back(ok ? q->h_tim[c][i] : 0);
                    else if (ok) row_time = q->h_tim[c][i];
                }
            }
            q->rv_times.push_back(row_time);
            rows++;
        }
        q->next_row = b_end;
        if (q->next_row >= p.n_buckets) { q->next_group++; q->next_row = 0; }
        if (rows == 0) continue;
        for (uint32_t c = 0; c < nc; c++) {
            og_colval_view &v = q->rv_cols[c];
            v.val = q->rv_val[c].data(); v.val_bytes = q->rv_val[c].size(); v.bitmap = q->rv_bitmap[c].data();
            v.times = (p.multi && q->dense[c].tim) ? q->rv_coltimes[c].data() : nullptr;
            v.type = p.calls[c].out_type; v.len = rows; v.nil_count = nil[c]; v.bitmap_offset = 0;
        }
        out->n_cols = nc; out->cols = q->rv_cols.data(); out->times = q->rv_times.data(); out->rows = rows; out->group = g;
        out->sid = q->desc.group_mode == OG_GROUP_PER_SERIES ? q->sh->sids[g] : 0;
        return OG_OK;
    }
    return OG_EOF;
}

}
namespace {
struct DenseEmit { uint8_t *out; int wide; __device__ __forceinline__ void operator()(uint32_t i, uint64_t bits) { if (wide) ((uint64_t *)out)[i] = bits; else out[i] = (uint8_t)bits; } };

__global__ void k_decode_column(DirP d, uint32_t column, int type, uint32_t seg_begin, uint32_t seg_end, uint8_t *out, uint64_t stride,
                                uint32_t *rows_out, uint8_t *bitmap_out, uint32_t bitmap_stride, int *err) {
    uint32_t seg = seg_begin + blockIdx.x * blockDim.x + threadIdx.x;
    if (seg >= seg_end) return;
    uint8_t *o = out + (size_t)(seg - seg_begin) * stride;
    uint32_t rows = d.seg_rows[seg];
    size_t pi = (size_t)column * d.n_segments + seg;
    if (column == d.n_columns) {
        TimeDesc t;
        int rc = parse_time_page(d.data + d.page_off[pi], d.page_len[pi], t);
        if (rc == D_OK) { TimeStore ts{(int64_t *)o, 1}; rc = decode_time_values(t, ts); }
        if (rc != D_OK) report_err(err, rc, seg);
        if (rows_out) rows_out[seg - seg_begin] = rows;
        return;
    }
    uint32_t len = d.page_len[pi];
    uint8_t *bm = bitmap_out ? bitmap_out + (size_t)(seg - seg_begin) * bitmap_stride : nullptr;
    if (len == 0) {
        if (rows_out) rows_out[seg - seg_begin] = 0;
        if (bm) for (uint32_t i = 0; i < (rows + 7) / 8; i++) bm[i] = 0;
        return;
    }
    PageHdr h;
    int rc = parse_field_header(d.data + d.page_off[pi], len, type, rows, h);
    if (rc == D_OK) {
        DenseEmit em{o, type != OG_TYPE_BOOL};
        rc = decode_block(type, h, em);
        if (rows_out) rows_out[seg - seg_begin] = h.rows - h.nil_count;
        if (bm) {
            for (uint32_t i = 0; i < (rows + 7) / 8; i++) {
                uint8_t v = 0;
                for (uint32_t k = 0; k < 8 && i * 8 + k < rows; k++) v |= (uint8_t)(hdr_row_valid(h, i * 8 + k) ? 1 : 0) << k;
                bm[i] = v;
            }
        }
    }
    if (rc != D_OK) report_err(err, rc, seg);
}
}
extern "C" {

OG_API int og_decode_column_device(og_shard *s, uint32_t column, uint32_t seg_begin, uint32_t seg_end, void *d_values,
                                   uint64_t value_stride_bytes, uint32_t *d_rows_out) {
    if (!s || !d_values || column > s->n_columns || seg_begin > seg_end || seg_end > s->n_segments) { set_error("bad argument"); return OG_E_INVAL; }
    CU(cudaSetDevice(s->device));
    if (seg_begin == seg_end) return OG_OK;
    int *d_err; int rc = dalloc(&d_err, 2); if (rc) return rc;
    cudaMemset(d_err, 0, 8);
    int type = column == s->n_columns ? OG_TYPE_INT : s->col_types[column];
    uint32_t n = seg_end - seg_begin;
    k_decode_column<<<(n + 127) / 128, 128>>>(make_dir(s), column, type, seg_begin, seg_end, (uint8_t *)d_values, value_stride_bytes, d_rows_out, nullptr, 0, d_err);
    int err[2]; cudaError_t e = cudaMemcpy(err, d_err, 8, cudaMemcpyDeviceToHost); dev_free(d_err);
    if (e != cudaSuccess) return cuda_fail(e, "k_decode_column", __FILE__, __LINE__);
    if (err[0]) { set_error("segment %d failed to decode (device code %d)", err[1], err[0]); return map_dev_err(err[0]); }
    return OG_OK;
}

__global__ void k_reverse_segment(uint8_t *vals, uint32_t elem_bytes, uint32_t n_vals, uint8_t *bitmap, uint32_t rows) {
    for (uint32_t i = threadIdx.x; i < n_vals / 2; i += blockDim.x) {
        const uint32_t j = n_vals - 1 - i;
        if (elem_bytes == 8) { uint64_t *v = (uint64_t *)vals; const uint64_t a = v[i]; v[i] = v[j]; v[j] = a; }
        else { const uint8_t a = vals[i]; vals[i] = vals[j]; vals[j] = a; }
    }
    if (!bitmap) return;
    __syncthreads();
    __shared__ uint8_t sbm[8192];
    const uint32_t nb = (rows + 7) / 8;
    for (uint32_t i = threadIdx.x; i < nb; i += blockDim.x) sbm[i] = bitmap[i];
    __syncthreads();
    for (uint32_t i = threadIdx.x; i < nb; i += blockDim.x) {
        uint8_t o = 0;
        for (uint32_t k = 0; k < 8 && i * 8 + k < rows; k++) { const uint32_t src = rows - 1 - (i * 8 + k); o |= (uint8_t)((sbm[src >> 3] >> (src & 7)) & 1) << k; }
        bitmap[i] = o;
    }
}
}
static int decode_segment_impl(og_shard *s, uint32_t segment, uint32_t flags, og_record_view *out);
extern "C" {
OG_API int og_decode_segment(og_shard *s, uint32_t segment, og_record_view *out) { return decode_segment_impl(s, segment, 0, out); }
OG_API int og_decode_segment_ex(og_shard *s, uint32_t segment, uint32_t flags, og_record_view *out) { return decode_segment_impl(s, segment, flags, out); }
}
static int decode_segment_impl(og_shard *s, uint32_t segment, uint32_t flags, og_record_view *out) {
    if (!s || !out || segment >= s->n_segments) { set_error("bad argument"); return OG_E_INVAL; }
    CU(cudaSetDevice(s->device));
    uint32_t R = std::max<uint32_t>(1, s->max_seg_rows);
    size_t ncol1 = (size_t)s->n_columns + 1;
    size_t val_stride = (size_t)R * 8, bm_stride = (((size_t)R + 7) / 8 + 7) & ~(size_t)7;
    size_t need = ncol1 * (val_stride + bm_stride + 16);
    if (s->d_seg_buf_bytes < need) {
        if (s->d_seg_buf) dev_free(s->d_seg_buf);
        if (s->h_seg_buf) cudaFreeHost(s->h_seg_buf);
        CU(dev_malloc((void **)&s->d_seg_buf, need)); CU(cudaMallocHost(&s->h_seg_buf, need));
        s->d_seg_buf_bytes = s->h_seg_buf_bytes = need;
    }
    uint8_t *dv = (uint8_t *)s->d_seg_buf, *dbm = dv + ncol1 * val_stride;
    uint32_t *drows = (uint32_t *)(dbm + ncol1 * bm_stride);
    int *d_err; int rc = dalloc(&d_err, 2); if (rc) return rc;
    cudaMemset(d_err, 0, 8);
    DirP dir = make_dir(s);
    for (uint32_t c = 0; c <= s->n_columns; c++) {
        int type = c == s->n_columns ? OG_TYPE_INT : s->col_types[c];
        k_decode_column<<<1, 32>>>(dir, c, type, segment, segment + 1, dv + c * val_stride, val_stride, drows + c, dbm + c * bm_stride, (uint32_t)bm_stride, d_err);
    }
    int err[2]; cudaError_t e = cudaMemcpy(err, d_err, 8, cudaMemcpyDeviceToHost); dev_free(d_err);
    if (e != cudaSuccess) return cuda_fail(e, "k_decode_column", __FILE__, __LINE__);
    if (err[0]) { set_error("segment %d failed to decode (device code %d)", err[1], err[0]); return map_dev_err(err[0]); }
    if (flags & OG_DECODE_DESCENDING) {
        if (R > 65536) { set_error("descending materialisation supports segments of up to 65536 rows"); return OG_E_UNSUPPORTED; }
        uint32_t hr[65];
        CU(cudaMemcpy(hr, drows, (ncol1) * 4, cudaMemcpyDeviceToHost));
        const uint32_t rows_seg = hr[s->n_columns];
        for (uint32_t c = 0; c <= s->n_columns; c++) {
            const bool is_time = c == s->n_columns;
            const uint32_t eb = (!is_time && s->col_types[c] == OG_TYPE_BOOL) ? 1 : 8;
            k_reverse_segment<<<1, 256>>>(dv + c * val_stride, eb, is_time ? rows_seg : hr[c], is_time ? nullptr : dbm + c * bm_stride, rows_seg);
        }
        CU(cudaGetLastError());
    }
    CU(cudaMemcpy(s->h_seg_buf, s->d_seg_buf, need, cudaMemcpyDeviceToHost));
    uint8_t *hv = (uint8_t *)s->h_seg_buf, *hbm = hv + ncol1 * val_stride;
    uint32_t *hrows = (uint32_t *)(hbm + ncol1 * bm_stride);
    uint32_t rows = hrows[s->n_columns];
    s->seg_views.assign(s->n_columns, og_colval_view{});
    for (uint32_t c = 0; c < s->n_columns; c++) {
        og_colval_view &v = s->seg_views[c];
        uint32_t nv = hrows[c];
        v.val = hv + c * val_stride; v.val_bytes = (uint64_t)nv * (s->col_types[c] == OG_TYPE_BOOL ? 1 : 8);
        v.bitmap = hbm + c * bm_stride; v.times = nullptr; v.type = s->col_types[c]; v.len = (int32_t)rows; v.nil_count = (int32_t)(rows - nv); v.bitmap_offset = 0;
    }
    out->n_cols = s->n_columns; out->cols = s->seg_views.data(); out->times = (const int64_t *)(hv + s->n_columns * val_stride); out->rows = (int32_t)rows; out->group = 0;
    uint32_t sr = (uint32_t)(std::upper_bound(s->h_series_seg_begin.begin(), s->h_series_seg_begin.end(), segment) - s->h_series_seg_begin.begin()) - 1;
    out->sid = s->sids[sr];
    return OG_OK;
}
```

opengemini_b200/csrc/fused.cuh:

```cuda
#pragma once
#include "agg_kernels.cuh"

namespace ogpu {

struct TimeIter {
    TimeDesc d; uint64_t cur; uint32_t idx; uint32_t w; unsigned k, n, bits; uint64_t word;
    __device__ __forceinline__ void init(const TimeDesc &t) { d = t; cur = (uint64_t)t.t0; idx = 0; w = 0; k = 0; n = 0; bits = 0; word = 0; }
    __device__ __forceinline__ int64_t next() {
        int64_t t;
        if (d.kind == 0 || d.kind == 3) { t = (int64_t)cur; cur += d.delta; }
        else if (d.kind == 2) { t = zigzag_dec(ld_be64(d.words + 8ull * idx)); }
        else {
            if (idx != 0) {
                while (k == n) {
                    if (w >= d.n_words) { idx++; return (int64_t)cur; }
                    word = ld_be64(d.words + 8ull * w); w++;
                    s8b_sel((unsigned)(word >> 60), n, bits); k = 0;
                }
                uint64_t dv = bits == 0 ? 1ull : ((word >> (k * bits)) & ((1ull << bits) - 1));
                k++;
                cur += dv * d.delta;
            }
            t = (int64_t)cur;
        }
        idx++;
        return t;
    }
};

template <int NC>
struct FusedState {
    const QueryP &q; const ChunkP &ch; const PageHdr &h;
    TimeIter ti;
    Part parts[NC];
    uint32_t seg, series, row, cur_b, head_b;
    int64_t we;
    bool head_done;

    __device__ __forceinline__ FusedState(const QueryP &q_, const ChunkP &ch_, const PageHdr &h_) : q(q_), ch(ch_), h(h_) {}

    __device__ __forceinline__ void flush(bool final) {
        if (cur_b == OG_NO_BUCKET) return;
        size_t e = 2 * (size_t)(seg - ch.seg_begin);
        if (!head_done) {
#pragma unroll
            for (int c = 0; c < NC; c++) store_part(ch.edges[c], e, parts[c]);
            head_done = true; head_b = cur_b;
        } else if (final) {
#pragma unroll
            for (int c = 0; c < NC; c++) store_part(ch.edges[c], e + 1, parts[c]);
        } else {
#pragma unroll
            for (int c = 0; c < NC; c++) if (parts[c].ok) store_cell(ch, c, series, cur_b, parts[c]);
        }
    }
    __device__ __forceinline__ void row_step(bool valid, uint64_t bits) {
        int64_t t = ti.next();
        row++;
        if (t < q.tmin || t > q.tmax) return;
        if (cur_b == OG_NO_BUCKET || t >= we) {
            flush(false);
            cur_b = bucket_of(t, q.start, q.interval);
            if (cur_b >= q.n_buckets) { report_err(ch.err, D_CORRUPT, seg); cur_b = OG_NO_BUCKET; return; }
            we = q.start + (int64_t)(cur_b + 1) * q.interval;
#pragma unroll
            for (int c = 0; c < NC; c++) parts[c] = part_empty();
        }
        if (valid) {
#pragma unroll
            for (int c = 0; c < NC; c++) acc_row(q.calls[c].func, q.calls[c].type, parts[c], bits, t);
        }
    }
    __device__ __forceinline__ void operator()(uint32_t, uint64_t bits) {
        while (row < h.rows && !hdr_row_valid(h, row)) row_step(false, 0);
        if (row < h.rows) row_step(true, bits);
    }
};

template <int NC>
__global__ void __launch_bounds__(128) k_fused_segment(DirP d, QueryP q, ChunkP ch, const uint32_t *list, uint32_t n) {
    uint32_t i = blockIdx.x * blockDim.x + threadIdx.x;
    if (i >= n) return;
    uint32_t seg = list ? list[i] : ch.seg_begin + i;
    size_t e = 2 * (size_t)(seg - ch.seg_begin);
    uint32_t rows = d.seg_rows[seg];
    if (d.seg_tmax[seg] < q.tmin || d.seg_tmin[seg] > q.tmax || rows == 0) {
        ch.edge_bucket[e] = OG_NO_BUCKET; ch.edge_bucket[e + 1] = OG_NO_BUCKET; return;
    }
    size_t ti_idx = (size_t)d.n_columns * d.n_segments + seg;
    TimeDesc td;
    int rc = parse_time_page(d.data + d.page_off[ti_idx], d.page_len[ti_idx], td);
    if (rc != D_OK) { report_err(ch.err, rc, seg); ch.edge_bucket[e] = OG_NO_BUCKET; ch.edge_bucket[e + 1] = OG_NO_BUCKET; return; }
    int col = q.col_index[0], type = q.col_type[0];
    size_t pi = (size_t)col * d.n_segments + seg;
    uint32_t len = d.page_len[pi];
    PageHdr h;
    if (len == 0) { h.rows = rows; h.nil_count = rows; h.bitmap = nullptr; h.bm_off = 0; h.block = nullptr; h.block_len = 0; h.one_row = 0; }
    else {
        rc = parse_field_header(d.data + d.page_off[pi], len, type, rows, h);
        if (rc != D_OK) { report_err(ch.err, rc, seg); ch.edge_bucket[e] = OG_NO_BUCKET; ch.edge_bucket[e + 1] = OG_NO_BUCKET; return; }
    }
    FusedState<NC> st(q, ch, h);
    st.ti.init(td);
    st.seg = seg; st.series = d.seg_series[seg]; st.row = 0; st.cur_b = OG_NO_BUCKET; st.head_b = OG_NO_BUCKET; st.we = 0; st.head_done = false;
    if (h.nil_count < h.rows) {
        rc = decode_block(type, h, st);
        if (rc != D_OK) report_err(ch.err, rc, seg);
    }
    while (st.row < rows) st.row_step(false, 0);
    uint32_t last_b = st.cur_b;
    bool single = !st.head_done;
    st.flush(true);
    ch.edge_bucket[e] = st.head_b;
    ch.edge_bucket[e + 1] = (single || st.head_b == OG_NO_BUCKET) ? OG_NO_BUCKET : last_b;
}

}
```

opengemini_b200/csrc/fused_cols.cuh:

```cuda
#pragma once
#include "fused_multi.cuh"
#include "fused_il.cuh"
#include <type_traits>

namespace ogpu {

#define OG_COLS_MAXROWS 1024u
#define OG_COLS_MAXMINE 4

struct BitWin {
    const uint32_t *base; uint32_t wa, wb, wc, wd, wi;
    __device__ __forceinline__ uint32_t ldw(uint32_t i) const { return __byte_perm(__ldg(base + i), 0, 0x0123); }
    __device__ __forceinline__ uint32_t init(const uint8_t *p) {
        const uintptr_t a = (uintptr_t)p;
        base = (const uint32_t *)(a & ~(uintptr_t)3);
        wi = 0; wa = ldw(0); wb = ldw(1); wc = ldw(2); wd = ldw(3);
        return (uint32_t)(a & 3) * 8;
    }
    __device__ __forceinline__ uint64_t peek(uint32_t P) {
        const uint32_t word = P >> 5;
        while (wi != word) { wa = wb; wb = wc; wc = wd; wi++; wd = ldw(wi + 3); }
        const uint32_t sh = P & 31;
        return ((uint64_t)__funnelshift_l(wb, wa, sh) << 32) | __funnelshift_l(wc, wb, sh);
    }
};

__device__ __forceinline__ void s8b_sel_packed(unsigned sel, unsigned &n, unsigned &bits) {
    const uint64_t NLO = 0x0a0c0f141e3c78f0ull, NHI = 0x0102030405060708ull;
    const uint64_t BLO = 0x0605040302010000ull, BHI = 0x3c1e140f0c0a0807ull;
    const unsigned sh = (sel & 7) * 8;
    n = (unsigned)(((sel & 8) ? NHI : NLO) >> sh) & 0xff;
    bits = (unsigned)(((sel & 8) ? BHI : BLO) >> sh) & 0xff;
}

enum { CK_GENERIC = 0, CK_GORILLA = 1, CK_S8B = 2, CK_BITS = 3 };

struct ColsSeg {
    uint32_t seg, series, rows, r_lo, r_hi; size_t e;
    int64_t t0, dt; uint64_t dtu;
    uint32_t b_first, rb_first, step_q; uint64_t rem_first, step_r;
};

template <int KIND, int MODE, bool SIMPLE>
__device__ __forceinline__ void cols_pass(const QueryP &q, const ChunkP &ch, const ColsSeg &sg, ColIter &it, uint32_t *keep,
                                          int nm, const int (&mc)[OG_COLS_MAXMINE]) {
    BitWin bw; uint32_t P = 0, gend = 0, tr = 0, mb = 64; uint64_t cur = it.cur;
    uint64_t sw = 0, smask = 0, snext = 0; uint32_t sbits = 0, sleft = 0, swords = it.words_left;
    const uint8_t *sp = it.p;
    if (KIND == CK_S8B && swords) snext = ld_be64(sp);
    uint32_t bbyte = 0;
    uint32_t idx = 0;
    if (KIND == CK_GORILLA) { const uint32_t b0 = bw.init(it.p); P = b0; gend = b0 + it.c; }
    auto next_value = [&]() -> uint64_t {
        const uint32_t i = idx++;
        if (KIND == CK_GORILLA) {
            if (i == 0) return cur;
            const uint64_t x = bw.peek(P);
            uint32_t used, m;
            if ((x >> 62) == 3) {
                const uint32_t lm = (uint32_t)(x >> 51) & 0x7ff, lead = (lm >> 6) & 0x1f;
                mb = lm & 0x3f;
                if (mb > 0) { if (lead + mb > 64) { it.err = D_CORRUPT; mb = 64; tr = 0; } else tr = 64 - lead - mb; }
                else { tr = 0; mb = 64; }
                used = 13; m = mb;
            } else { used = (x >> 63) ? 2u : 1u; m = (x >> 63) ? mb : 0u; }
            P += used;
            uint64_t y = x << used;
            if (used + m > 64) y = bw.peek(P);
            const uint64_t v = m == 0 ? 0ull : (y >> (64 - m));
            P += m;
            if (P > gend) { it.err = D_CORRUPT; return cur; }
            cur ^= v << tr;
            if (m && cur == OG_UVNAN) it.err = D_CORRUPT;
            return cur;
        } else if (KIND == CK_S8B) {
            if (i == 0) return cur;
            while (sleft == 0) {
                if (swords == 0) { it.err = D_CORRUPT; return cur; }
                sw = snext; sp += 8; swords--;
                if (swords) snext = ld_be64(sp);
                unsigned nn; s8b_sel_packed((unsigned)(sw >> 60), nn, sbits);
                sleft = nn;
                if (sbits == 0) { sw = ~0ull; smask = 1; }
                else smask = (1ull << sbits) - 1;
            }
            const uint64_t z = sw & smask;
            sw >>= sbits; sleft--;
            cur += (uint64_t)zigzag_dec(z);
            return cur;
        } else if (KIND == CK_BITS) {
            if ((i & 7) == 0) bbyte = __ldg(it.p + (i >> 3));
            return (uint64_t)((bbyte >> (7 - (i & 7))) & 1);
        } else return it.value();
    };
    const bool absent = it.kind == ColIter::K_ABSENT;
    const uint8_t *bm = absent ? nullptr : it.h.bitmap;
    const bool all_ok = !absent && !bm && it.h.nil_count == 0;
    const uint32_t bm_off = absent ? 0 : it.h.bm_off;
    uint32_t vb = 0, vb_i = 0xffffffffu;
    auto valid = [&](uint32_t r) -> bool {
        if (!bm) return all_ok;
        const uint32_t b = bm_off + r;
        if ((b >> 3) != vb_i) { vb_i = b >> 3; vb = __ldg(bm + vb_i); }
        return (vb >> (b & 7)) & 1;
    };
    const FilterP &f = q.filter[0];
    const int f_mode = f.type == OG_TYPE_FLOAT ? 0 : (f.type == OG_TYPE_INT && f.const_is_float) ? 1 : f.type == OG_TYPE_BOOL ? 3 : 2;
    const double f_cd = f.const_is_float ? f.fval : (double)f.ival;
    const int64_t f_ci = f.ival;
    const uint32_t f_lt = f.op == OG_OP_LT || f.op == OG_OP_LTE || f.op == OG_OP_NEQ, f_gt = f.op == OG_OP_GT || f.op == OG_OP_GTE || f.op == OG_OP_NEQ;
    const uint32_t f_eq = f.op == OG_OP_LTE || f.op == OG_OP_GTE || f.op == OG_OP_EQ, f_un = f.op != OG_OP_EQ;
    const uint32_t f_tab = f_un | (f_lt << 1) | (f_gt << 2) | (f_eq << 4);
    auto term = [&](uint64_t raw) -> bool {
        uint32_t idx;
        if (f_mode <= 1) {
            double v;
            if (f_mode == 0) v = u2d(raw); else v = (double)(int64_t)raw;
            idx = (uint32_t)(v < f_cd) + 2u * (uint32_t)(v > f_cd) + 4u * (uint32_t)(v == f_cd);
        } else {
            const int64_t v = f_mode == 3 ? (int64_t)(raw != 0) : (int64_t)raw;
            idx = (uint32_t)(v < f_ci) + 2u * (uint32_t)(v > f_ci) + 4u * (uint32_t)(v == f_ci);
        }
        return (f_tab >> idx) & 1;
    };
    int op[OG_COLS_MAXMINE];
#pragma unroll
    for (int j = 0; j < OG_COLS_MAXMINE; j++) {
        const CallP &cp = q.calls[mc[j]];
        op[j] = cp.func == OG_AGG_COUNT ? 0 : cp.type == OG_TYPE_FLOAT ? 1 : 2;
    }

    auto run = [&](auto nobm_tag) {
    constexpr bool NOBM = decltype(nobm_tag)::value;
    uint32_t r = 0;
    for (; r < sg.r_lo; r++) if (NOBM || valid(r)) (void)next_value();

    Part parts[OG_COLS_MAXMINE];
    uint32_t cur_b = sg.b_first, rb = sg.rb_first, w = 0; uint64_t rem = sg.rem_first;
    uint32_t kw = (MODE == 2) ? keep[r >> 5] >> (r & 31) : 0u;
    const bool fcol = it.type == OG_TYPE_FLOAT;
    uint64_t cnt = 0, isum = 0; double fsum = 0.0;
    while (r <= sg.r_hi) {
        const uint32_t stop = rb < sg.r_hi + 1 ? rb : sg.r_hi + 1;
        if (SIMPLE) { cnt = 0; isum = 0; fsum = 0.0; }
        else {
#pragma unroll
            for (int j = 0; j < OG_COLS_MAXMINE; j++) parts[j] = part_empty();
        }
        for (; r < stop; r++) {
            const bool ok = NOBM || valid(r);
            uint64_t v = 0;
            if (ok) v = next_value();
            bool kp = true;
            if (MODE == 1) {
                kp = ok && term(v);
                kw |= (uint32_t)kp << (r & 31);
                if ((r & 31) == 31) { keep[r >> 5] = kw; kw = 0; }
            } else if (MODE == 2) {
                if ((r & 31) == 0) kw = keep[r >> 5];
                kp = kw & 1; kw >>= 1;
            }
            const bool take = kp && ok;
            if (SIMPLE) {
                cnt += (uint64_t)take;
                if (fcol) fsum += take ? u2d(v) : 0.0;
                else isum += take ? v : 0ull;
            } else if (take) {
#pragma unroll
                for (int j = 0; j < OG_COLS_MAXMINE; j++) {
                    if (j >= nm) break;
                    const CallP &cp = q.calls[mc[j]];
                    acc_row(cp.func, cp.type, parts[j], v, sg.t0 + (int64_t)r * sg.dt);
                }
            }
        }
        const bool final = r > sg.r_hi;
#pragma unroll
        for (int j = 0; j < OG_COLS_MAXMINE; j++) {
            if (j >= nm) break;
            if (SIMPLE) { parts[j].t = 0; parts[j].ok = cnt != 0; parts[j].v = op[j] == 0 ? cnt : op[j] == 1 ? d2u(fsum) : isum; }
            if (w == 0) store_part(ch.edges[mc[j]], sg.e, parts[j]);
            else if (final) store_part(ch.edges[mc[j]], sg.e + 1, parts[j]);
            else if (parts[j].ok) store_cell(ch, mc[j], sg.series, cur_b, parts[j]);
        }
        w++;
        if (!final) while (r >= rb) {
            cur_b++;
            rem += sg.step_r; uint32_t adv = sg.step_q;
            if (rem >= sg.dtu) { rem -= sg.dtu; adv++; }
            rb = (rb > 0xffffffffu - adv) ? 0xffffffffu : rb + adv;
        }
    }
    if (MODE == 1 && (sg.r_hi & 31) != 31) keep[sg.r_hi >> 5] = kw;
    };
    if (!bm && all_ok) run(std::true_type{}); else run(std::false_type{});
}

template <int MODE, bool SIMPLE>
__device__ __forceinline__ void cols_column(const DirP &d, const QueryP &q, const ChunkP &ch, const ColsSeg &sg, int slot, uint32_t *keep) {
    int mc[OG_COLS_MAXMINE]; int nm = 0;
#pragma unroll
    for (int j = 0; j < OG_COLS_MAXMINE; j++) mc[j] = 0;
    for (uint32_t c = 0; c < q.n_calls; c++) if (q.calls[c].col_slot == slot) {
#pragma unroll
        for (int j = 0; j < OG_COLS_MAXMINE; j++) if (j == nm) mc[j] = (int)c;
        nm++;
    }
    if (MODE != 1 && nm == 0) return;
    const size_t pi = (size_t)q.col_index[slot] * d.n_segments + sg.seg;
    ColIter it;
    it.init(d.data + d.page_off[pi], d.page_len[pi], q.col_type[slot], sg.rows);
    if (it.err != D_OK) { report_err(ch.err, it.err, sg.seg); it.kind = ColIter::K_ABSENT; }
    switch (it.kind) {
    case ColIter::K_F_GORILLA: cols_pass<CK_GORILLA, MODE, SIMPLE>(q, ch, sg, it, keep, nm, mc); break;
    case ColIter::K_I_S8B: cols_pass<CK_S8B, MODE, SIMPLE>(q, ch, sg, it, keep, nm, mc); break;
    case ColIter::K_B_BITS: cols_pass<CK_BITS, MODE, SIMPLE>(q, ch, sg, it, keep, nm, mc); break;
    default: cols_pass<CK_GENERIC, MODE, SIMPLE>(q, ch, sg, it, keep, nm, mc); break;
    }
    if (it.err != D_OK) report_err(ch.err, it.err, sg.seg);
}

#ifndef OG_COLS_MINB
#define OG_COLS_MINB 10
#endif
template <bool SIMPLE>
__global__ void __launch_bounds__(128, SIMPLE ? OG_COLS_MINB : 4) k_fused_cols(DirP d, QueryP q, ChunkP ch) {
    const uint32_t i = blockIdx.x * blockDim.x + threadIdx.x;
    ColsSeg sg;
    sg.seg = ch.seg_begin + i;
    if (sg.seg >= ch.seg_end) return;
    sg.e = 2 * (size_t)(sg.seg - ch.seg_begin);
    sg.rows = d.seg_rows[sg.seg]; sg.series = d.seg_series[sg.seg];
    auto no_rows = [&]() { ch.edge_bucket[sg.e] = OG_NO_BUCKET; ch.edge_bucket[sg.e + 1] = OG_NO_BUCKET; };
    if (d.seg_tmax[sg.seg] < q.tmin || d.seg_tmin[sg.seg] > q.tmax || sg.rows == 0) { no_rows(); return; }
    const size_t ti_idx = (size_t)d.n_columns * d.n_segments + sg.seg;
    TimeDesc td;
    const int rc = parse_time_page(d.data + d.page_off[ti_idx], d.page_len[ti_idx], td);
    if (rc != D_OK || (td.kind != 0 && td.kind != 3) || sg.rows > OG_COLS_MAXROWS) {
        report_err(ch.err, rc != D_OK ? rc : D_CORRUPT, sg.seg); no_rows(); return;
    }
    sg.t0 = td.t0; sg.dtu = td.delta; sg.dt = (int64_t)td.delta;
    sg.r_lo = 0; sg.r_hi = sg.rows - 1;
    sg.step_q = 0; sg.step_r = 0; sg.rem_first = 0; sg.rb_first = 0xffffffffu;
    if (sg.dtu == 0) { if (sg.t0 < q.tmin || sg.t0 > q.tmax) { no_rows(); return; } }
    else {
        const double inv_dt = 1.0 / __ull2double_rn(sg.dtu);
        if (sg.t0 < q.tmin) { const uint64_t k = udiv_est((uint64_t)(q.tmin - sg.t0) + sg.dtu - 1, sg.dtu, inv_dt); sg.r_lo = k > sg.rows ? sg.rows : (uint32_t)k; }
        const int64_t t_last = sg.t0 + (int64_t)(sg.rows - 1) * sg.dt;
        if (t_last > q.tmax) { if (q.tmax < sg.t0) sg.r_lo = sg.rows; else sg.r_hi = (uint32_t)udiv_est((uint64_t)(q.tmax - sg.t0), sg.dtu, inv_dt); }
        if (sg.r_lo > sg.r_hi || sg.r_lo >= sg.rows) { no_rows(); return; }
    }
    const int64_t t_lo = sg.t0 + (int64_t)sg.r_lo * sg.dt;
    sg.b_first = bucket_of(t_lo, q.start, q.interval);
    if (sg.dtu != 0) {
        const double inv_dt = 1.0 / __ull2double_rn(sg.dtu);
        const uint64_t ivl = (uint64_t)q.interval;
        const uint64_t sq64 = udiv_est(ivl, sg.dtu, inv_dt);
        sg.step_q = sq64 > 0xffffffffull ? 0xffffffffu : (uint32_t)sq64;
        sg.step_r = ivl - sq64 * sg.dtu;
        const uint64_t D = (uint64_t)(q.start + (int64_t)(sg.b_first + 1) * q.interval - sg.t0) + sg.dtu - 1;
        const uint64_t qq = udiv_est(D, sg.dtu, inv_dt);
        sg.rem_first = D - qq * sg.dtu; sg.rb_first = qq > 0xffffffffull ? 0xffffffffu : (uint32_t)qq;
    }
    const uint32_t b_last = bucket_of(sg.t0 + (int64_t)sg.r_hi * sg.dt, q.start, q.interval);
    if (b_last >= q.n_buckets) { report_err(ch.err, D_CORRUPT, sg.seg); no_rows(); return; }

    uint32_t keep[OG_COLS_MAXROWS / 32];
    if (q.n_filter) {
        const int fs = q.filter[0].col_slot;
        cols_column<1, SIMPLE>(d, q, ch, sg, fs, keep);
        for (int k = 0; k < (int)q.n_cols; k++) if (k != fs) cols_column<2, SIMPLE>(d, q, ch, sg, k, keep);
    } else {
        for (int k = 0; k < (int)q.n_cols; k++) cols_column<0, SIMPLE>(d, q, ch, sg, k, keep);
    }
    ch.edge_bucket[sg.e] = sg.b_first;
    ch.edge_bucket[sg.e + 1] = b_last == sg.b_first ? OG_NO_BUCKET : b_last;
}

}
```

opengemini_b200/csrc/fused_il.cuh:

```cuda
#pragma once
#include "agg_kernels.cuh"

namespace ogpu {

__device__ __forceinline__ uint32_t smem_u32(const void *p) { return (uint32_t)__cvta_generic_to_shared(p); }
__device__ __forceinline__ uint32_t opaque(uint32_t x) { asm volatile("mov.u32 %0, %0;" : "+r"(x)); return x; }
template <int OFF> __device__ __forceinline__ uint32_t lds32o(uint32_t a) { uint32_t v; asm volatile("ld.shared.u32 %0, [%1+%2];" : "=r"(v) : "r"(a), "n"(OFF)); return v; }
__device__ __forceinline__ void mbar_init(uint32_t bar, uint32_t count) { asm volatile("mbarrier.init.shared::cta.b64 [%0], %1;" ::"r"(bar), "r"(count) : "memory"); }
__device__ __forceinline__ void mbar_init_fence() { asm volatile("fence.mbarrier_init.release.cluster;\nfence.proxy.async.shared::cta;" ::: "memory"); }
__device__ __forceinline__ void mbar_expect_tx(uint32_t bar, uint32_t bytes) { asm volatile("mbarrier.arrive.expect_tx.shared::cta.b64 _, [%0], %1;" ::"r"(bar), "r"(bytes) : "memory"); }
__device__ __forceinline__ void bulk_g2s(uint32_t dst, const void *src, uint32_t bytes, uint32_t bar) {
    asm volatile("cp.async.bulk.shared::cluster.global.mbarrier::complete_tx::bytes [%0], [%1], %2, [%3];" ::"r"(dst), "l"(src), "r"(bytes), "r"(bar) : "memory");
}
__device__ __forceinline__ bool mbar_wait(uint32_t bar, uint32_t parity) {
#pragma unroll 1
    for (uint32_t i = 0; i < (1u << 16); i++) {
        uint32_t ok;
        asm volatile("{\n.reg .pred p;\nmbarrier.try_wait.parity.shared::cta.b64 p, [%1], %2;\nselp.u32 %0, 1, 0, p;\n}" : "=r"(ok) : "r"(bar), "r"(parity) : "memory");
        if (ok) return true;
    }
    return false;
}

enum { FM_COUNT = 1, FM_SUM = 2, FM_MIN = 4, FM_MAX = 8, FM_FIRST = 16, FM_LAST = 32 };
enum { SEG_GENERAL = 0, SEG_FAST = 1, SEG_RAWX = 2 };

#ifndef OG_FAST_THREADS
#define OG_FAST_THREADS 128
#endif
#ifndef OG_FAST_MAXREG
#define OG_FAST_MAXREG 80
#endif
#ifndef OG_IL_NW
#define OG_IL_NW 64u
#endif
#ifndef OG_IL_B
#define OG_IL_B 16u
#endif
#ifndef OG_IL_K
#define OG_IL_K 10u
#endif
#ifndef OG_IL_UNROLL
#define OG_IL_UNROLL 2
#endif
#define OG_IL_NB (OG_IL_NW / OG_IL_B)
#define OG_IL_ROWS (OG_IL_NW + 2u)
#define OG_IL_PAD_WORDS 6u
#define OG_IL_HDR 7u
#define OG_IL_RAW_HDR 6u
#define OG_IL_NONE 0xffffffffu
#define OG_IL_RAWFLAG 0x80000000u
#define OG_IL_LOOKBITS (77u * OG_IL_K + 29u + 13u + 64u + 64u)
static_assert(OG_IL_NW % OG_IL_B == 0 && (OG_IL_NW & (OG_IL_NW - 1)) == 0, "ring geometry");
static_assert(OG_IL_NW - OG_IL_B > (OG_IL_LOOKBITS + 31u) / 32u + 2u, "ring too small for the round length: the slowest lane could not proceed");

struct IlP {
    const uint32_t *words;
    const uint64_t *grp_off;
    const uint32_t *grp_rows;
    const uint32_t *grp_col;
    const uint32_t *lane_seg;
    const uint32_t *lane_rows;
    const uint32_t *lane_series;
    const int64_t *lane_t0;
    const uint64_t *lane_dt;
};

__device__ __forceinline__ uint64_t udiv_est(uint64_t a, uint64_t b, double inv_b) {
    const double qd = __ull2double_rn(a) * inv_b;
    if ((a >> 63) || !(qd < 1125899906842624.0)) return a / b;
    uint64_t q = (uint64_t)qd;
    uint64_t r = a - q * b;
    if ((int64_t)r < 0) { do { q--; r += b; } while ((int64_t)r < 0); }
    else while (r >= b) { q++; r -= b; }
    return q;
}

__device__ __forceinline__ uint64_t fetch64(uint32_t col, uint32_t p) {
    uint32_t a = col + ((p << 2) & ((OG_IL_NW - 1) << 7));
    uint32_t a0 = lds32o<0>(a), a1 = lds32o<128>(a), a2 = lds32o<256>(a);
    uint32_t hi = __funnelshift_l(a1, a0, p), lo = __funnelshift_l(a2, a1, p);
    return ((uint64_t)hi << 32) | lo;
}

__device__ __forceinline__ Part fold32(int func, int type, bool multi, Part p, bool with_time) {
    constexpr uint32_t FULL = 0xffffffffu;
    if (func == OG_AGG_COUNT) { p.v = __reduce_add_sync(FULL, p.ok ? (uint32_t)p.v : 0u); p.ok = p.v != 0; return p; }
    if (type == OG_TYPE_FLOAT && func == OG_AGG_SUM) {
        double s = p.ok ? u2d(p.v) : 0.0;
#pragma unroll
        for (int o = 16; o; o >>= 1) s += __shfl_xor_sync(FULL, s, o);
        p.ok = __any_sync(FULL, p.ok != 0); p.v = d2u(s); return p;
    }
    if (type == OG_TYPE_FLOAT && !with_time && (func == OG_AGG_MIN || func == OG_AGG_MAX)) {
        double v = u2d(p.v); uint32_t ok = p.ok;
#pragma unroll
        for (int o = 16; o; o >>= 1) {
            const double ov = __shfl_xor_sync(FULL, v, o); const uint32_t ook = __shfl_xor_sync(FULL, ok, o);
            const bool keep = ok && (func == OG_AGG_MIN ? v <= ov : v >= ov);
            if (ook && !keep) v = ov;
            ok |= ook;
        }
        p.v = d2u(v); p.ok = ok; return p;
    }
    return warp_fold(func, type, multi, p, with_time);
}

#define OG_IL_WCAP 24u
__host__ __device__ inline uint32_t il_acc_bytes(uint32_t n_calls, bool times) { return OG_IL_WCAP * n_calls * (times ? 17u : 9u) + 8u & ~7u; }

template <int FM, bool TIMES, bool FOLD>
__global__ void __maxnreg__(OG_FAST_MAXREG) k_fused_il(QueryP q, ChunkP ch, IlP il, uint32_t grp_begin, uint32_t grp_end) {
    constexpr uint32_t NW = OG_IL_NW, B = OG_IL_B, NB = OG_IL_NB, K = OG_IL_K;
    constexpr uint32_t FULL = 0xffffffffu;
    constexpr uint32_t WPB = OG_FAST_THREADS / 32;
    constexpr int UNR = OG_IL_UNROLL;
    __shared__ __align__(128) uint32_t s_win[WPB * OG_IL_ROWS * 32];
    __shared__ __align__(8) uint64_t s_bar[WPB * NB];
    extern __shared__ __align__(8) uint8_t s_acc[];

    const uint32_t lane = threadIdx.x & 31;
    const uint32_t wid = __reduce_max_sync(FULL, threadIdx.x >> 5);
    const uint32_t grp = grp_begin + blockIdx.x * WPB + wid;
    if (grp >= grp_end) return;
    const uint32_t rows_w = __reduce_max_sync(FULL, il.grp_rows[grp]);
    if (rows_w == 0) return;
    const size_t slot = (size_t)grp * 32 + lane;
    const uint32_t seg = il.lane_seg[slot];
    bool active = seg != OG_IL_NONE && seg >= ch.seg_begin && seg < ch.seg_end;
    if (!__any_sync(FULL, active)) return;
    const size_t e = 2 * (size_t)(seg - ch.seg_begin);

    uint32_t rows = 0, series = 0, r_lo = 0, r_hi = 0; bool rawx = false;
    int64_t t0 = 0, dt = 1; uint64_t dtu = 1; double inv_dt = 1.0;
    const double inv_iv = 1.0 / __ull2double_rn((uint64_t)q.interval);
    if (active) {
        const uint32_t rf = il.lane_rows[slot];
        rows = rf & ~OG_IL_RAWFLAG; rawx = (rf & OG_IL_RAWFLAG) != 0; series = il.lane_series[slot];
        t0 = il.lane_t0[slot]; dtu = il.lane_dt[slot]; dt = (int64_t)dtu;
        inv_dt = 1.0 / __ull2double_rn(dtu);
        r_lo = 0; r_hi = rows - 1;
        if (t0 < q.tmin) { uint64_t k = udiv_est((uint64_t)(q.tmin - t0) + dtu - 1, dtu, inv_dt); r_lo = k > rows ? rows : (uint32_t)k; }
        { int64_t t_last = t0 + (int64_t)(rows - 1) * dt; if (t_last > q.tmax) { if (q.tmax < t0) r_lo = rows; else r_hi = (uint32_t)udiv_est((uint64_t)(q.tmax - t0), dtu, inv_dt); } }
        if (r_lo > r_hi || r_lo >= rows) { ch.edge_bucket[e] = OG_NO_BUCKET; ch.edge_bucket[e + 1] = OG_NO_BUCKET; active = false; }
    }
    if (!__any_sync(FULL, active)) return;

    const uint32_t win = smem_u32(s_win) + wid * (OG_IL_ROWS * 128);
    const uint32_t col = opaque(win + lane * 4);
    const uint32_t bar0 = smem_u32(s_bar) + wid * (NB * 8);
    if (lane == 0) {
#pragma unroll
        for (uint32_t i = 0; i < NB; i++) mbar_init(bar0 + i * 8, 1);
        mbar_init_fence();
    }
    __syncwarp();
    const uint32_t total_b = rows_w / B;
    uint64_t goff = il.grp_off[grp];
    goff = ((uint64_t)__reduce_max_sync(FULL, (uint32_t)(goff >> 32)) << 32) | __reduce_max_sync(FULL, (uint32_t)goff);
    const uint32_t *gsrc = il.words + goff;
    uint32_t issued_b = 0, ready_b = 0;
    uint32_t hung = 0;
    auto issue = [&](uint32_t k_any) {
        const uint32_t k = __reduce_max_sync(FULL, k_any);
        const uint32_t s = k % NB, dst = win + s * (B * 128), bar = bar0 + s * 8;
        const uint32_t *src = gsrc + (size_t)k * (B * 32);
        if (s == 0)
            asm volatile("{\n.reg .pred p;\nelect.sync _|p, 0xffffffff;\n@p mbarrier.arrive.expect_tx.shared::cta.b64 _, [%0], %1;\n"
                         "@p cp.async.bulk.shared::cluster.global.mbarrier::complete_tx::bytes [%2], [%3], %4, [%0];\n"
                         "@p cp.async.bulk.shared::cluster.global.mbarrier::complete_tx::bytes [%5], [%3], 256, [%0];\n}"
                         ::"r"(bar), "r"(B * 128 + 256u), "r"(dst), "l"(src), "r"(B * 128), "r"(win + NW * 128) : "memory");
        else
            asm volatile("{\n.reg .pred p;\nelect.sync _|p, 0xffffffff;\n@p mbarrier.arrive.expect_tx.shared::cta.b64 _, [%0], %1;\n"
                         "@p cp.async.bulk.shared::cluster.global.mbarrier::complete_tx::bytes [%2], [%3], %1, [%0];\n}"
                         ::"r"(bar), "r"(B * 128), "r"(dst), "l"(src) : "memory");
    };
    {
        const uint32_t first = total_b < NB ? total_b : NB;
        for (uint32_t k = 0; k < first; k++) issue(k);
        issued_b = first;
    }

    uint32_t cur_b = 0, rb = 0xffffffffu, step_q = 0; uint64_t rem = 0, step_r = 0;
    if (active) {
        const int64_t t_lo = t0 + (int64_t)r_lo * dt;
        cur_b = (uint32_t)udiv_est((uint64_t)(t_lo - q.start), (uint64_t)q.interval, inv_iv);
        const uint64_t ivl = (uint64_t)q.interval;
        const uint64_t sq64 = udiv_est(ivl, dtu, inv_dt);
        step_q = sq64 > 0xffffffffull ? 0xffffffffu : (uint32_t)sq64;
        step_r = ivl - sq64 * dtu;
        uint64_t D = (uint64_t)(q.start + (int64_t)(cur_b + 1) * q.interval - t0) + dtu - 1;
        uint64_t qq = udiv_est(D, dtu, inv_dt); rem = D - qq * dtu; rb = qq > 0xffffffffull ? 0xffffffffu : (uint32_t)qq;
    }

    bool uni = false; uint32_t b0 = 0;
    uint64_t *acc_v = nullptr; int64_t *acc_t = nullptr; uint8_t *acc_k = nullptr;
    if (FOLD) {
        const int leader = __ffs(__ballot_sync(FULL, active)) - 1;
        const int64_t t0L = __shfl_sync(FULL, t0, leader); const uint64_t dtL = __shfl_sync(FULL, dtu, leader);
        const uint32_t loL = __shfl_sync(FULL, r_lo, leader), hiL = __shfl_sync(FULL, r_hi, leader);
        b0 = __shfl_sync(FULL, cur_b, leader);
        const bool same = t0 == t0L && dtu == dtL && r_lo == loL && r_hi == hiL;
        const uint32_t b_last = active ? (uint32_t)udiv_est((uint64_t)(t0 + (int64_t)r_hi * dt - q.start), (uint64_t)q.interval, inv_iv) : b0;
        uni = __all_sync(FULL, !active || (same && b_last - b0 < OG_IL_WCAP));
        if (uni) {
            const uint32_t nacc = OG_IL_WCAP * q.n_calls;
            uint8_t *base = s_acc + (size_t)wid * il_acc_bytes(q.n_calls, TIMES);
            acc_v = (uint64_t *)base; acc_t = (int64_t *)(base + (size_t)nacc * 8); acc_k = base + (size_t)nacc * (TIMES ? 16 : 8);
            for (uint32_t i = lane; i < nacc; i += 32) acc_k[i] = 0;
            __syncwarp();
        }
    }
    const uint32_t gcol = FOLD ? il.grp_col[grp] - ch.gc_col0 : 0;

    double sum = 0.0, mn = 0.0, mx = 0.0; uint64_t fi = 0, lastv = 0;
    uint32_t n_mn = 0, n_mx = 0;
    uint32_t w_row0 = r_lo;
    bool head_done = false; uint32_t head_b = OG_NO_BUCKET;
    uint32_t stop = 0, n_ev = 0;
    auto part_of = [&](int func, uint32_t cnt) -> Part {
        Part pp; pp.ok = cnt != 0; pp.v = 0; pp.t = 0;
        switch (func) {
        case OG_AGG_COUNT: pp.v = cnt; break;
        case OG_AGG_SUM: if (FM & FM_SUM) pp.v = d2u(sum); break;
        case OG_AGG_MIN: if (FM & FM_MIN) { pp.v = d2u(mn); if (TIMES) pp.t = t0 + (int64_t)(stop - n_mn) * dt; } break;
        case OG_AGG_MAX: if (FM & FM_MAX) { pp.v = d2u(mx); if (TIMES) pp.t = t0 + (int64_t)(stop - n_mx) * dt; } break;
        case OG_AGG_FIRST: if (FM & FM_FIRST) { pp.v = fi; pp.t = t0 + (int64_t)w_row0 * dt; } break;
        default: if (FM & FM_LAST) { pp.v = lastv; pp.t = t0 + (int64_t)(stop - 1) * dt; } break;
        }
        return pp;
    };
    auto kind_of = [&]() -> int { return !head_done ? 0 : stop > r_hi ? 1 : 2; };
    auto flush_lane = [&](int kind) {
        const uint32_t cnt = stop - w_row0;
#pragma unroll 1
        for (uint32_t c = 0; c < q.n_calls; c++) {
            const Part pp = part_of(q.calls[c].func, cnt);
            if (kind == 2) { if (pp.ok) store_cell(ch, (int)c, series, cur_b, pp); }
            else store_part(ch.edges[c], e + kind, pp);
        }
        if (kind == 0) { head_done = true; head_b = cur_b; }
    };
    auto flush_fold = [&](bool ev) {
        uint32_t pend = __ballot_sync(FULL, ev);
#pragma unroll 1
        while (pend) {
            const int leader = __ffs(pend) - 1;
            const uint32_t bL = __shfl_sync(FULL, cur_b, leader);
            const bool mine = ev && cur_b == bL;
            const uint32_t cnt = mine ? stop - w_row0 : 0;
            const uint32_t w = bL - b0;
#pragma unroll 1
            for (uint32_t c = 0; c < q.n_calls; c++) {
                const int func = q.calls[c].func, ftype = func == OG_AGG_COUNT ? OG_TYPE_INT : q.calls[c].type;
                const bool wt = func >= OG_AGG_MIN && !(q.multi && func <= OG_AGG_MAX);
                Part pp = fold32(func, ftype, q.multi != 0, part_of(func, cnt), wt);
                if ((int)lane == leader && pp.ok) {
                    const uint32_t i = c * OG_IL_WCAP + w;
                    Part a; a.ok = acc_k[i]; a.v = a.ok ? acc_v[i] : 0; a.t = (TIMES && a.ok) ? acc_t[i] : 0;
                    group_update(func, ftype, q.multi != 0, a, pp);
                    acc_v[i] = a.v; acc_k[i] = 1; if (TIMES) acc_t[i] = a.t;
                }
            }
            pend &= ~__ballot_sync(FULL, mine);
        }
        __syncwarp();
    };

    uint32_t qp = 0, sr = 0, kfast = 0, CM = 0, CE = 0, m = 64, tr = 0, bad = 0; uint64_t MASK = 0;
    bool done = !active;
    uint64_t val = 0;

    if (issued_b && !mbar_wait(bar0, 0)) hung = 1; else ready_b = issued_b ? 1 : 0;
    if (active && !hung) {
        val = fetch64(col, 0); qp = 64;
        if (rawx) { MASK = ~0ull; kfast = 64; }
        else { CM = 0; CE = 1; }
    }

    bool skipping = r_lo > 0;
    stop = skipping ? r_lo : (rb < r_hi + 1 ? rb : r_hi + 1);
    n_ev = stop;
    if (!skipping) { fi = val; mn = mx = u2d(val); n_mn = n_mx = n_ev; }
    if (done) n_ev = 0xffffffffu;

    auto retire = [&]() { done = true; n_ev = 0xffffffffu; CM = 0; CE = 0; MASK = 0; kfast = 0; };
    auto advance = [&]() {
        bool fin = false;
        if (skipping) { skipping = false; sum = 0.0; }
        else {
            fin = stop > r_hi;
            sum = 0.0;
            if (!fin) while (stop >= rb) {
                cur_b++;
                rem += step_r; uint32_t adv = step_q;
                if (rem >= dtu) { rem -= dtu; adv++; }
                rb = (rb > 0xffffffffu - adv) ? 0xffffffffu : rb + adv;
            }
        }
        if (fin) retire();
        else {
            w_row0 = stop;
            uint32_t nstop = rb < r_hi + 1 ? rb : r_hi + 1;
            n_ev = nstop - stop; stop = nstop;
            fi = val; mn = mx = u2d(val); n_mn = n_mx = n_ev;
        }
    };
    auto slow_record = [&]() {
        uint32_t p = qp + sr;
        const uint64_t x = fetch64(col, p);
        const uint32_t ctrl = (uint32_t)(x >> 62);
        if (ctrl < 2) { qp += 1; return; }
        if (ctrl == 3) {
            const uint32_t lm = (uint32_t)(x >> 51) & 0x7ff;
            uint32_t lead = lm >> 6; m = lm & 0x3f;
            if (m == 0) { m = 64; tr = 0; lead = 0; }
            else { if (lead + m > 64) { if (!done) bad = 1; lead = 0; m = 64; } tr = 64 - lead - m; }
            p += 13;
            const bool slowwin = lead < 2;
            sr = slowwin ? 0 : lead - 2;
            CM = slowwin ? 0u : 3u << (30 - sr); CE = slowwin ? 1u : 2u << (30 - sr);
            kfast = 2 + m;
            MASK = (m == 64 ? ~0ull : ((1ull << m) - 1)) << tr;
        } else p += 2;
        const uint64_t y = fetch64(col, p);
        const uint64_t sig = m == 64 ? y : (y >> (64 - m));
        p += m;
        val ^= sig << tr;
        qp = p - sr;
    };
    auto accumulate = [&](uint32_t k_in_run) {
        if (FM & FM_SUM) sum = sum + u2d(val);
        if (FM & FM_MIN) { if (mn > u2d(val)) { mn = u2d(val); if (TIMES) n_mn = n_ev - k_in_run; } }
        if (FM & FM_MAX) { if (mx < u2d(val)) { mx = u2d(val); if (TIMES) n_mx = n_ev - k_in_run; } }
        if (FM & FM_LAST) lastv = val;
    };
    auto record = [&](uint32_t k_in_run) {
        accumulate(k_in_run);
        const uint64_t x = fetch64(col, qp);
        const bool slow = (((uint32_t)(x >> 32) & CM) ^ CE) != 0;
        if (slow) slow_record();
        else { val ^= x & MASK; qp += kfast; }
    };
    auto record2 = [&](uint32_t k_in_run) {
        const uint64_t x0 = fetch64(col, qp), x1 = fetch64(col, qp + kfast);
        accumulate(k_in_run);
#ifdef OG_IL_REC2B
        uint64_t x1b = x1;
        if ((((uint32_t)(x0 >> 32) & CM) ^ CE) != 0) { slow_record(); x1b = fetch64(col, qp); }
        else { val ^= x0 & MASK; qp += kfast; }
        accumulate(k_in_run + 1);
        if ((((uint32_t)(x1b >> 32) & CM) ^ CE) != 0) slow_record();
        else { val ^= x1b & MASK; qp += kfast; }
#else
        if ((((uint32_t)(x0 >> 32) & CM) ^ CE) != 0) { slow_record(); record(k_in_run + 1); return; }
        val ^= x0 & MASK; qp += kfast;
        accumulate(k_in_run + 1);
        if ((((uint32_t)(x1 >> 32) & CM) ^ CE) != 0) slow_record();
        else { val ^= x1 & MASK; qp += kfast; }
#endif
    };

    uint32_t rounds_left = hung ? 0u : 40u * (__reduce_max_sync(FULL, rows) / K + 8u);
#ifdef OG_IL_STATS
    uint32_t st_common = 0, st_rare = 0, st_sit = 0, st_notgo = 0;
#endif
    for (;;) {
        const uint32_t qmin = __reduce_min_sync(FULL, done ? 0xffffffffu : qp);
        if (qmin == 0xffffffffu) break;
        const uint32_t f = qmin < 32 ? 0u : (qmin - 32) >> 5;
#pragma unroll 1
        while (issued_b < total_b && (issued_b + 1) * B <= f + NW) { issue(issued_b); issued_b++; }
        const uint32_t qmax = __reduce_max_sync(FULL, done ? 0u : qp);
        uint32_t need_max = ((qmax + OG_IL_LOOKBITS) >> 5) + 1; if (need_max > rows_w) need_max = rows_w;
        uint32_t want_b = (need_max + B - 1) / B; if (want_b > issued_b) want_b = issued_b;
#pragma unroll 1
        while (ready_b < want_b) { if (!mbar_wait(bar0 + (ready_b % NB) * 8, (ready_b / NB) & 1)) { hung = 1; break; } ready_b++; }
        if (hung) break;
        uint32_t need = ((qp + OG_IL_LOOKBITS) >> 5) + 1; if (need > rows_w) need = rows_w;
        bool go = done || need <= ready_b * B;
        uint32_t run = __reduce_min_sync(FULL, go ? n_ev : 0u);
        if (run >= K) {
            static_assert(K % 2 == 0, "records are decoded in pairs");
#pragma unroll UNR
            for (uint32_t k = 0; k < K; k += 2) record2(k);
            n_ev -= K;
#ifdef OG_IL_STATS
            st_common++;
#endif
            continue;
        }
#ifdef OG_IL_STATS
        st_rare++;
#endif
        if (rounds_left-- == 0) { hung = 2; break; }
        const bool all_go = __all_sync(FULL, go);
#ifdef OG_IL_STATS
        if (!all_go) { st_notgo++; st_sit += __popc(__ballot_sync(FULL, !go)); }
#endif
        uint32_t left = K;
        for (;;) {
            run = __reduce_min_sync(FULL, go ? n_ev : 0xffffffffu);
            if (run > left) run = left;
            if (all_go) {
#pragma unroll 1
                for (uint32_t k = 0; k < run; k++) record(k);
            } else {
#pragma unroll 1
                for (uint32_t k = 0; k < run; k++) if (go) record(k);
            }
            if (go) n_ev -= run;
            left -= run;
            if (left == 0) break;
            const bool ev = go && !done && n_ev == 0;
            if (FOLD && uni) {
                const bool fl = ev && !skipping;
                const int kind = kind_of();
                if (fl && kind != 2) flush_lane(kind);
                if (__any_sync(FULL, fl && kind == 2)) flush_fold(fl && kind == 2);
            } else if (ev && !skipping) flush_lane(kind_of());
            if (ev) advance();
            if (__all_sync(FULL, ev || done)) break;
        }
    }
    if (active && (qp >> 5) >= rows_w) bad = 1;
#ifdef OG_IL_STATS
    if (lane == 0) { atomicAdd((unsigned *)&ch.err[4], st_common); atomicAdd((unsigned *)&ch.err[5], st_rare); atomicAdd((unsigned *)&ch.err[6], st_notgo); atomicAdd((unsigned *)&ch.err[7], st_sit); }
#endif
    while (ready_b < issued_b && hung != 1) { if (!mbar_wait(bar0 + (ready_b % NB) * 8, (ready_b / NB) & 1)) hung = 1; ready_b++; }
    if (hung && lane == 0) report_err(ch.err, D_WATCHDOG, (grp << 2) | hung);
    if (FOLD && uni) {
        __syncwarp();
        for (uint32_t i = lane; i < OG_IL_WCAP * q.n_calls; i += 32) {
            if (!acc_k[i]) continue;
            const uint32_t c = i / OG_IL_WCAP, w = i % OG_IL_WCAP;
            Part a; a.ok = 1; a.v = acc_v[i]; a.t = TIMES ? acc_t[i] : 0;
            store_part(ch.gcells[c], (size_t)(b0 + w) * ch.gc_cols + gcol, a);
        }
    }
    if (active) {
        if (bad) report_err(ch.err, D_CORRUPT, seg);
        ch.edge_bucket[e] = head_b;
        ch.edge_bucket[e + 1] = (head_b == OG_NO_BUCKET || cur_b == head_b) ? OG_NO_BUCKET : cur_b;
    }
}

}
```

opengemini_b200/csrc/fused_multi.cuh:

```cuda
#pragma once
#include "fused.cuh"

namespace ogpu {

#define OG_MULTI_MAXC 4

struct ColIter {
    enum { K_ABSENT = 0, K_NULLMAP , K_ONE, K_F_RAW, K_F_GORILLA, K_F_SAME, K_F_RLE, K_I_CONST, K_I_S8B, K_I_RAW, K_B_BITS };
    PageHdr h;
    int kind, type;
    uint32_t row;
    uint32_t idx;
    const uint8_t *p;
    uint64_t cur;
    uint64_t aux;
    uint32_t a, b, c;
    uint32_t words_left;
    int err;

    __device__ __forceinline__ void init(const uint8_t *page, uint32_t len, int col_type, uint32_t seg_rows) {
        type = col_type; row = 0; idx = 0; err = D_OK; cur = 0; aux = 0; a = b = c = 0; words_left = 0; p = nullptr;
        if (len == 0) { kind = K_ABSENT; h.rows = seg_rows; h.nil_count = seg_rows; h.bitmap = nullptr; h.bm_off = 0; h.block = nullptr; h.block_len = 0; h.one_row = 0; return; }
        int rc = parse_field_header(page, len, col_type, seg_rows, h);
        if (rc != D_OK) { err = rc; kind = K_ABSENT; return; }
        const uint32_t n = h.rows - h.nil_count;
        if (n == 0) { kind = K_ABSENT; return; }
        if (col_type == OG_TYPE_STRING) { kind = K_NULLMAP; return; }
        if (h.one_row) { kind = K_ONE; cur = col_type == OG_TYPE_BOOL ? (uint64_t)__ldg(h.block) : (h.block_len >= 8 ? ld_le64(h.block) : 0); if (col_type != OG_TYPE_BOOL && h.block_len < 8) err = D_CORRUPT; return; }
        if (h.block_len < 1) { err = D_CORRUPT; kind = K_ABSENT; return; }
        const uint8_t *in = h.block; const uint32_t bl = h.block_len - 1;
        const int tag = __ldg(in) >> 4;
        p = in + 1;
        if (col_type == OG_TYPE_FLOAT) {
            switch (tag) {
            case 0: kind = K_F_RAW; if (bl < 8ull * n) err = D_CORRUPT; break;
            case 3: kind = K_F_GORILLA;
                if (bl < 9) { err = D_CORRUPT; break; }
                cur = ld_be64(p + 1); p += 9; aux = 0; a = 0; b = 64; c = (bl - 9) * 8;
                if (cur == OG_UVNAN) err = D_CORRUPT;
                break;
            case 4: kind = K_F_SAME; if (bl < 2 || ld_be16(p) != n) { err = D_CORRUPT; break; } cur = 0; if (bl != 2) { if (bl < 10) err = D_CORRUPT; else cur = ld_le64(p + 2); } break;
            case 5: kind = K_F_RLE; a = 0; c = bl; break;
            default: err = (tag == 1 || tag == 2 || tag == 6) ? D_UNSUPPORTED : D_CORRUPT; break;
            }
        } else if (col_type == OG_TYPE_INT) {
            if (bl < 4) { err = D_CORRUPT; kind = K_ABSENT; return; }
            switch (tag) {
            case 4: kind = K_I_RAW; if (bl - 4 < ld_be32(p) || (bl - 4) / 8 != n) err = D_CORRUPT; p += 4; break;
            case 1: { kind = K_I_CONST;
                if (bl < 8) { err = D_CORRUPT; break; }
                uint64_t d, cnt; int k = ld_uvarint(p + 8, bl - 8, &d);
                int k2 = k ? ld_uvarint(p + 8 + k, bl - 8 - k, &cnt) : 0;
                if (k == 0 || k2 == 0 || cnt + 1 != n) { err = D_CORRUPT; break; }
                cur = (uint64_t)zigzag_dec(ld_be64(p)); aux = (uint64_t)zigzag_dec(d);
                break; }
            case 2: { kind = K_I_S8B;
                if (bl < 16) { err = D_CORRUPT; break; }
                const uint32_t enc = ld_be32(p), src = ld_be32(p + 4);
                if (src != n || enc == 0 || bl - 8 < enc * 8ull) { err = D_CORRUPT; break; }
                cur = (uint64_t)zigzag_dec(ld_be64(p + 8)); p += 16; words_left = enc - 1; a = 0; b = 0; c = 0;
                break; }
            default: err = tag == 3 ? D_UNSUPPORTED : D_CORRUPT; break;
            }
        } else if (col_type == OG_TYPE_BOOL) {
            kind = K_B_BITS;
            if (tag != 1 || bl < 4 || ld_be32(p) != n || (uint64_t)(bl - 4) * 8 < n) err = D_CORRUPT;
            p += 4;
        } else err = D_UNSUPPORTED;
        if (err != D_OK) kind = K_ABSENT;
    }

    __device__ __forceinline__ uint64_t value() {
        const uint32_t i = idx++;
        switch (kind) {
        case K_ONE: return cur;
        case K_F_RAW: return ld_le64(p + 8ull * i);
        case K_F_SAME: return cur;
        case K_F_GORILLA: {
            if (i == 0) return cur;
            const uint8_t *bp = p + (aux >> 3);
            const unsigned sh = (unsigned)(aux & 7);
            const uint64_t w = ld_be64(bp) << sh;
            unsigned used = (w >> 63) ? 2u : 1u;
            if ((w >> 62) == 3) {
                const unsigned lm = (unsigned)(w >> 51) & 0x7ff;
                const unsigned lead = (lm >> 6) & 0x1f;
                b = lm & 0x3f;
                if (b > 0) { if (lead + b > 64) { err = D_CORRUPT; b = 64; a = 0; } else a = 64 - lead - b; }
                else { a = 0; b = 64; }
                used = 13;
            }
            const unsigned mb = (w >> 63) ? b : 0u;
            aux += used;
            const uint8_t *q2 = p + (aux >> 3);
            const unsigned s2 = (unsigned)(aux & 7);
            uint64_t v = ld_be64(q2) << s2;
            if (s2 + mb > 64) v |= (uint64_t)__ldg(q2 + 8) >> (8 - s2);
            v = mb == 64 ? v : mb == 0 ? 0ull : (v >> (64 - mb));
            aux += mb;
            if (aux > c) { err = D_CORRUPT; return cur; }
            cur ^= v << a;
            if (mb && cur == OG_UVNAN) err = D_CORRUPT;
            return cur; }
        case K_F_RLE: {
            if (a == 0) {
                if (c < 2) { err = D_CORRUPT; return 0; }
                uint32_t n = ld_be16(p);
                if (n >> 15) { n -= 1u << 15; cur = 0; p += 2; c -= 2; }
                else { if (c < 10) { err = D_CORRUPT; return 0; } cur = ld_le64(p + 2); p += 10; c -= 10; }
                if (n == 0) { err = D_CORRUPT; return 0; }
                a = n;
            }
            a--;
            return cur; }
        case K_I_RAW: return (uint64_t)zigzag_dec(ld_be64(p + 8ull * i));
        case K_I_CONST: { const uint64_t v = cur; cur += aux; return v; }
        case K_I_S8B: {
            if (i == 0) return cur;
            while (a == b) {
                if (words_left == 0) { err = D_CORRUPT; return cur; }
                aux = ld_be64(p); p += 8; words_left--;
                unsigned nn, bits; s8b_sel((unsigned)(aux >> 60), nn, bits);
                b = nn; c = bits; a = 0;
            }
            const uint64_t z = c == 0 ? 1ull : ((aux >> (a * c)) & ((1ull << c) - 1));
            a++;
            cur += (uint64_t)zigzag_dec(z);
            return cur; }
        case K_B_BITS: return (uint64_t)((__ldg(p + (i >> 3)) >> (7 - (i & 7))) & 1);
        default: return 0;
        }
    }
    __device__ __forceinline__ bool next(uint64_t &v) {
        const uint32_t r = row++;
        if (kind == K_ABSENT) return false;
        if (!hdr_row_valid(h, r)) return false;
        v = value();
        return true;
    }
};

template <int NCOL, int NCALL, bool SIMPLE>
__global__ void __launch_bounds__(128) k_fused_multi(DirP d, QueryP q, ChunkP ch) {
    const uint32_t i = blockIdx.x * blockDim.x + threadIdx.x;
    const uint32_t seg = ch.seg_begin + i;
    if (seg >= ch.seg_end) return;
    const size_t e = 2 * (size_t)(seg - ch.seg_begin);
    const uint32_t rows = d.seg_rows[seg], series = d.seg_series[seg];
    auto no_rows = [&]() { ch.edge_bucket[e] = OG_NO_BUCKET; ch.edge_bucket[e + 1] = OG_NO_BUCKET; };
    if (d.seg_tmax[seg] < q.tmin || d.seg_tmin[seg] > q.tmax || rows == 0) { no_rows(); return; }
    const size_t ti_idx = (size_t)d.n_columns * d.n_segments + seg;
    TimeDesc td;
    int rc = parse_time_page(d.data + d.page_off[ti_idx], d.page_len[ti_idx], td);
    if (rc != D_OK) { report_err(ch.err, rc, seg); no_rows(); return; }
    TimeIter ti; ti.init(td);
    ColIter col[NCOL];
#pragma unroll
    for (int k = 0; k < NCOL; k++) {
        const size_t pi = (size_t)q.col_index[k] * d.n_segments + seg;
        col[k].init(d.data + d.page_off[pi], d.page_len[pi], q.col_type[k], rows);
        if (col[k].err != D_OK) { report_err(ch.err, col[k].err, seg); no_rows(); return; }
    }
    Part parts[NCALL];
    uint32_t cur_b = OG_NO_BUCKET, head_b = OG_NO_BUCKET; bool head_done = false;
    int64_t we = 0;
    auto flush = [&](bool final) {
        if (cur_b == OG_NO_BUCKET) return;
#pragma unroll
        for (int c = 0; c < NCALL; c++) {
            if (!head_done) store_part(ch.edges[c], e, parts[c]);
            else if (final) store_part(ch.edges[c], e + 1, parts[c]);
            else if (parts[c].ok) store_cell(ch, (int)c, series, cur_b, parts[c]);
        }
        if (!head_done) { head_done = true; head_b = cur_b; }
    };
    for (uint32_t r = 0; r < rows; r++) {
        const int64_t t = ti.next();
        uint64_t v[NCOL]; bool ok[NCOL];
#pragma unroll
        for (int k = 0; k < NCOL; k++) { v[k] = 0; ok[k] = col[k].next(v[k]); }
        if (t < q.tmin) continue;
        if (t > q.tmax) break;
        if (cur_b == OG_NO_BUCKET || t >= we) {
            flush(false);
            cur_b = bucket_of(t, q.start, q.interval);
            if (cur_b >= q.n_buckets) { report_err(ch.err, D_CORRUPT, seg); cur_b = OG_NO_BUCKET; break; }
            we = q.start + (int64_t)(cur_b + 1) * q.interval;
#pragma unroll
            for (int c = 0; c < NCALL; c++) parts[c] = part_empty();
        }
        bool keep = true;
        if (q.n_filter == 1) {
            const FilterP &f = q.filter[0];
            keep = false;
#pragma unroll
            for (int k = 0; k < NCOL; k++) if (f.col_slot == k) keep = ok[k] && term_pass(f, v[k]);
        } else if (q.n_filter) {
            uint32_t stack = 0; int sp = 0;
            for (uint32_t fi = 0; fi < q.n_filter; fi++) {
                const FilterP &f = q.filter[fi];
                if (f.kind == OG_F_TERM) {
                    bool pass = false;
#pragma unroll
                    for (int k = 0; k < NCOL; k++) if (f.col_slot == k) pass = ok[k] && term_pass(f, v[k]);
                    stack |= (uint32_t)pass << sp; sp++;
                } else {
                    const uint32_t bb = (stack >> (sp - 1)) & 1, aa = (stack >> (sp - 2)) & 1;
                    const uint32_t rr = f.kind == OG_F_AND ? (aa & bb) : (aa | bb);
                    sp -= 2; stack &= ~(3u << sp); stack |= rr << sp; sp++;
                }
            }
            keep = stack & 1;
        }
        if (!keep) continue;
#pragma unroll
        for (int c = 0; c < NCALL; c++) {
            const CallP &cp = q.calls[c];
#pragma unroll
            for (int k = 0; k < NCOL; k++) {
                if (cp.col_slot != k || !ok[k]) continue;
                if (SIMPLE) {
                    if (cp.func == OG_AGG_COUNT) parts[c].v += 1;
                    else if (cp.type == OG_TYPE_FLOAT) parts[c].v = d2u(u2d(parts[c].v) + u2d(v[k]));
                    else parts[c].v += v[k];
                    parts[c].ok = 1;
                } else acc_row(cp.func, cp.type, parts[c], v[k], t);
            }
        }
    }
    for (int k = 0; k < NCOL; k++) if (col[k].err != D_OK) report_err(ch.err, col[k].err, seg);
    const uint32_t last_b = cur_b;
    const bool single = !head_done;
    flush(true);
    ch.edge_bucket[e] = head_b;
    ch.edge_bucket[e + 1] = (single || head_b == OG_NO_BUCKET) ? OG_NO_BUCKET : last_b;
}

}
```

Before: 635.1 billion.

## Transpose edge buffers to series-major strides and specialize fold kernels by aggregate mask

Edge partials and edge buckets move from interleaved per-segment pairs to a head/tail-split layout indexed by (kind, segment-within-series, series) when J is set. Adjacent lanes in k_fix_edges_fold (one series per lane) then read contiguous addresses, so the loads coalesce. k_fix_edges_fold and the interleaved fold flush are templated on the function mask through with_agg, which removes runtime dispatch on the aggregate function and folds each function once per window instead of once per call. Time buffers are now allocated only when call_has_time holds, which saves memory; the catch-all default branch in with_agg adds some risk of mis-specialization.

```diff
diff --git a/opengemini_b200/csrc/agg_kernels.cuh b/opengemini_b200/csrc/agg_kernels.cuh
--- a/opengemini_b200/csrc/agg_kernels.cuh
+++ b/opengemini_b200/csrc/agg_kernels.cuh
@@ -31,6 +31,13 @@
 };
 
 __device__ __forceinline__ size_t cell_idx(const ChunkP &ch, uint32_t series, uint32_t b) { return (size_t)(series - ch.series_begin) * ch.nb + b; }
+__device__ __forceinline__ size_t edge_idx(const ChunkP &ch, uint32_t series, uint32_t seg, uint32_t kind) {
+    if (ch.J == 0) return 2 * (size_t)(seg - ch.seg_begin) + kind;
+    const uint32_t ns = ch.series_end - ch.series_begin, s = series - ch.series_begin;
+    const uint32_t j = seg - ch.seg_begin - s * ch.J;
+    return ((size_t)kind * ch.J + j) * ns + s;
+}
+__device__ __forceinline__ size_t edge_tail_off(const ChunkP &ch) { return ch.J == 0 ? 1 : (size_t)ch.J * (ch.series_end - ch.series_begin); }
 
 __device__ __forceinline__ void report_err(int *err, int code, uint32_t seg) {
     if (atomicCAS(&err[0], 0, code) == 0) err[1] = (int)seg;
@@ -200,8 +207,8 @@
 
 __device__ __forceinline__ void emit_window(const QueryP &q, const ChunkP &ch, uint32_t seg, uint32_t series, uint32_t b,
                                             bool is_head, bool is_tail, int call, const Part &p) {
-    if (is_head) store_part(ch.edges[call], 2 * (size_t)(seg - ch.seg_begin), p);
-    else if (is_tail) store_part(ch.edges[call], 2 * (size_t)(seg - ch.seg_begin) + 1, p);
+    if (is_head) store_part(ch.edges[call], edge_idx(ch, series, seg, 0), p);
+    else if (is_tail) store_part(ch.edges[call], edge_idx(ch, series, seg, 1), p);
     else if (p.ok) store_cell(ch, call, series, b, p);
 }
 
@@ -210,15 +217,15 @@
     uint32_t seg = tp.tile_begin + sl;
     if (seg >= tp.tile_end) return;
     const uint32_t rows = d.seg_rows[seg], series = d.seg_series[seg];
-    const size_t S = tp.S, e = 2 * (size_t)(seg - ch.seg_begin);
+    const size_t S = tp.S, eh = edge_idx(ch, series, seg, 0), et = edge_idx(ch, series, seg, 1);
     Part parts[OG_MAX_CALLS];
     uint32_t cur_b = OG_NO_BUCKET, head_b = OG_NO_BUCKET; bool head_done = false;
     int64_t we = 0;
     auto flush = [&](bool final) {
         if (cur_b == OG_NO_BUCKET) return;
         for (uint32_t c = 0; c < q.n_calls; c++) {
-            if (!head_done) store_part(ch.edges[c], e, parts[c]);
-            else if (final) store_part(ch.edges[c], e + 1, parts[c]);
+            if (!head_done) store_part(ch.edges[c], eh, parts[c]);
+            else if (final) store_part(ch.edges[c], et, parts[c]);
             else if (parts[c].ok) store_cell(ch, (int)c, series, cur_b, parts[c]);
         }
         if (!head_done) { head_done = true; head_b = cur_b; }
@@ -245,38 +252,36 @@
         }
     }
     flush(true);
-    ch.edge_bucket[e] = head_b;
-    ch.edge_bucket[e + 1] = (head_b == OG_NO_BUCKET || cur_b == head_b) ? OG_NO_BUCKET : cur_b;
-}
-
-struct EdgeRuns { uint32_t hb, tb, s_end; bool head_leader; };
+    ch.edge_bucket[eh] = head_b;
+    ch.edge_bucket[et] = (head_b == OG_NO_BUCKET || cur_b == head_b) ? OG_NO_BUCKET : cur_b;
+}
+
+struct EdgeRuns { uint32_t series, hb, tb, s_end; bool head_leader; };
 __device__ __forceinline__ EdgeRuns edge_runs(const DirP &d, const ChunkP &ch, uint32_t seg, uint32_t series) {
     EdgeRuns r;
+    r.series = series;
     const uint32_t s_first = d.series_seg_begin[series];
     r.s_end = d.series_seg_begin[series + 1];
     const uint32_t *eb = ch.edge_bucket;
-    const size_t e = 2 * (size_t)(seg - ch.seg_begin);
-    r.hb = eb[e]; r.tb = eb[e + 1];
+    r.hb = eb[edge_idx(ch, series, seg, 0)]; r.tb = eb[edge_idx(ch, series, seg, 1)];
     r.head_leader = true;
     if (r.hb != OG_NO_BUCKET && seg > s_first) {
-        const size_t pe = e - 2;
-        const uint32_t pb = eb[pe + 1] != OG_NO_BUCKET ? eb[pe + 1] : eb[pe];
+        const uint32_t pt = eb[edge_idx(ch, series, seg - 1, 1)];
+        const uint32_t pb = pt != OG_NO_BUCKET ? pt : eb[edge_idx(ch, series, seg - 1, 0)];
         if (pb != OG_NO_BUCKET && pb == r.hb) r.head_leader = false;
     }
     return r;
 }
-__device__ __forceinline__ Part edge_stitch(const QueryP &q, const ChunkP &ch, const EdgeRuns &r, uint32_t seg, int which, uint32_t c) {
-    const CallP &cp = q.calls[c];
+__device__ __forceinline__ Part edge_stitch(const ChunkP &ch, const EdgeRuns &r, uint32_t seg, int which, const Tri &edges, int func, int type) {
     const uint32_t *eb = ch.edge_bucket;
-    const size_t e = 2 * (size_t)(seg - ch.seg_begin);
     const uint32_t b = which == 0 ? r.hb : r.tb;
-    Part acc = load_part(ch.edges[c], e + which);
+    Part acc = load_part(edges, edge_idx(ch, r.series, seg, which));
     if (which == 1 || r.tb == OG_NO_BUCKET) {
         for (uint32_t nx = seg + 1; nx < r.s_end; nx++) {
-            const size_t ne = 2 * (size_t)(nx - ch.seg_begin);
+            const size_t ne = edge_idx(ch, r.series, nx, 0);
             if (eb[ne] != b) break;
-            acc = series_merge(cp.func, cp.type, acc, load_part(ch.edges[c], ne));
-            if (eb[ne + 1] != OG_NO_BUCKET) break;
+            acc = series_merge(func, type, acc, load_part(edges, ne));
+            if (eb[edge_idx(ch, r.series, nx, 1)] != OG_NO_BUCKET) break;
         }
     }
     return acc;
@@ -294,7 +299,7 @@
         const uint32_t b = which == 0 ? r.hb : r.tb;
         if (b >= q.n_buckets) { report_err(ch.err, D_CORRUPT, seg); continue; }
         for (uint32_t c = 0; c < q.n_calls; c++) {
-            const Part acc = edge_stitch(q, ch, r, seg, which, c);
+            const Part acc = edge_stitch(ch, r, seg, which, ch.edges[c], q.calls[c].func, q.calls[c].type);
             if (acc.ok) store_cell(ch, (int)c, series, b, acc);
         }
     }
@@ -310,9 +315,10 @@
     for (int o = 16; o; o >>= 1) { const Part other = shfl_xor_part(p, o, with_time); group_update(func, type, multi, p, other); }
     return p;
 }
-__device__ __forceinline__ bool call_has_time(const QueryP &q, uint32_t c) { return q.calls[c].func >= OG_AGG_MIN && !(q.multi && q.calls[c].func <= OG_AGG_MAX); }
+__host__ __device__ __forceinline__ bool call_has_time(const QueryP &q, uint32_t c) { return q.calls[c].func >= OG_AGG_MIN && !(q.multi && q.calls[c].func <= OG_AGG_MAX); }
 __device__ __forceinline__ int call_ftype(const QueryP &q, uint32_t c) { return q.calls[c].func == OG_AGG_COUNT ? OG_TYPE_INT : q.calls[c].type; }
 
+template <int FM, bool TIMES>
 __global__ void k_fix_edges_fold(DirP d, QueryP q, ChunkP ch) {
     const uint32_t w = (blockIdx.x * blockDim.x + threadIdx.x) >> 5, lane = threadIdx.x & 31;
     const uint32_t n_blk = (ch.series_end - ch.series_begin + 31) / 32;
@@ -334,12 +340,16 @@
         const bool unif = __all_sync(0xffffffffu, !has || b == bL) && bL < q.n_buckets;
         if (!unif && has && b >= q.n_buckets) { report_err(ch.err, D_CORRUPT, seg); continue; }
         for (uint32_t c = 0; c < q.n_calls; c++) {
-            Part acc = part_empty();
-            if (has) acc = edge_stitch(q, ch, r, seg, which, c);
-            if (unif) {
-                acc = warp_fold(q.calls[c].func, call_ftype(q, c), q.multi != 0, acc, call_has_time(q, c));
-                if ((int)lane == leader && acc.ok) store_part(ch.gcells[c], (size_t)bL * ch.gc_cols + gcol, acc);
-            } else if (has && acc.ok) store_cell(ch, (int)c, series, b, acc);
+            with_agg<FM>(q.calls[c].func, [&](auto fc) {
+                constexpr int func = decltype(fc)::value, ftype = func == OG_AGG_COUNT ? OG_TYPE_INT : OG_TYPE_FLOAT;
+                const bool wt = func >= OG_AGG_FIRST || (TIMES && func >= OG_AGG_MIN && !q.multi);
+                Part acc = part_empty();
+                if (has) acc = edge_stitch(ch, r, seg, which, ch.edges[c], func, OG_TYPE_FLOAT);
+                if (unif) {
+                    acc = warp_fold(func, ftype, q.multi != 0, acc, wt);
+                    if ((int)lane == leader && acc.ok) store_part(ch.gcells[c], (size_t)bL * ch.gc_cols + gcol, acc);
+                } else if (has && acc.ok) store_cell(ch, (int)c, series, b, acc);
+            });
         }
     }
 }
diff --git a/opengemini_b200/csrc/agg_ops.cuh b/opengemini_b200/csrc/agg_ops.cuh
--- a/opengemini_b200/csrc/agg_ops.cuh
+++ b/opengemini_b200/csrc/agg_ops.cuh
@@ -1,5 +1,6 @@
 #pragma once
 #include <cstdint>
+#include <type_traits>
 
 #include "../../include/ogpu.h"
 
@@ -94,6 +95,18 @@
     }
 }
 
+enum { FM_COUNT = 1, FM_SUM = 2, FM_MIN = 4, FM_MAX = 8, FM_FIRST = 16, FM_LAST = 32 };
+template <int FM, class F> __device__ __forceinline__ void with_agg(int func, F &&f) {
+    switch (func) {
+    case OG_AGG_COUNT: if constexpr ((FM & FM_COUNT) != 0) f(std::integral_constant<int, OG_AGG_COUNT>()); break;
+    case OG_AGG_SUM: if constexpr ((FM & FM_SUM) != 0) f(std::integral_constant<int, OG_AGG_SUM>()); break;
+    case OG_AGG_MIN: if constexpr ((FM & FM_MIN) != 0) f(std::integral_constant<int, OG_AGG_MIN>()); break;
+    case OG_AGG_MAX: if constexpr ((FM & FM_MAX) != 0) f(std::integral_constant<int, OG_AGG_MAX>()); break;
+    case OG_AGG_FIRST: if constexpr ((FM & FM_FIRST) != 0) f(std::integral_constant<int, OG_AGG_FIRST>()); break;
+    default: if constexpr ((FM & FM_LAST) != 0) f(std::integral_constant<int, OG_AGG_LAST>()); break;
+    }
+}
+
 __device__ __forceinline__ uint32_t bucket_of(int64_t t, int64_t start, int64_t interval) {
     return (uint32_t)((uint64_t)(t - start) / (uint64_t)interval);
 }
diff --git a/opengemini_b200/csrc/api.cu b/opengemini_b200/csrc/api.cu
--- a/opengemini_b200/csrc/api.cu
+++ b/opengemini_b200/csrc/api.cu
@@ -433,24 +433,32 @@
     if (fold) k_fused_il<FM, TIMES, true><<<grid, block, WPB * il_acc_bytes(p.n_calls, TIMES), st>>>(p, ch, il, g0, g1);
     else k_fused_il<FM, TIMES, false><<<grid, block, 0, st>>>(p, ch, il, g0, g1);
 }
+template <class L> void with_fm(int fm, bool times, L &&l) {
+    using std::integral_constant; using std::bool_constant;
+    if (!times) {
+        switch (fm) {
+        case FM_SUM | FM_COUNT: return l(integral_constant<int, FM_SUM | FM_COUNT>(), bool_constant<false>());
+        case FM_SUM | FM_COUNT | FM_MAX: return l(integral_constant<int, FM_SUM | FM_COUNT | FM_MAX>(), bool_constant<false>());
+        case FM_SUM | FM_COUNT | FM_MIN | FM_MAX: return l(integral_constant<int, FM_SUM | FM_COUNT | FM_MIN | FM_MAX>(), bool_constant<false>());
+        case FM_COUNT: return l(integral_constant<int, FM_COUNT>(), bool_constant<false>());
+        default: break;
+        }
+    } else {
+        switch (fm) {
+        case FM_MAX | FM_COUNT: return l(integral_constant<int, FM_MAX | FM_COUNT>(), bool_constant<true>());
+        case FM_MIN | FM_COUNT: return l(integral_constant<int, FM_MIN | FM_COUNT>(), bool_constant<true>());
+        default: break;
+        }
+    }
+    return l(integral_constant<int, 63>(), bool_constant<true>());
+}
 void launch_fast(int fm, bool times, bool fold, const IlP &il, uint32_t g0, uint32_t g1, const QueryP &p, const ChunkP &ch, cudaStream_t st) {
     if (g1 <= g0) return;
-    if (!times) {
-        switch (fm) {
-        case FM_SUM | FM_COUNT: return launch_fast_t<FM_SUM | FM_COUNT, false>(fold, il, g0, g1, p, ch, st);
-        case FM_SUM | FM_COUNT | FM_MAX: return launch_fast_t<FM_SUM | FM_COUNT | FM_MAX, false>(fold, il, g0, g1, p, ch, st);
-        case FM_SUM | FM_COUNT | FM_MIN | FM_MAX: return launch_fast_t<FM_SUM | FM_COUNT | FM_MIN | FM_MAX, false>(fold, il, g0, g1, p, ch, st);
-        case FM_COUNT: return launch_fast_t<FM_COUNT, false>(fold, il, g0, g1, p, ch, st);
-        default: break;
-        }
-    } else {
-        switch (fm) {
-        case FM_MAX | FM_COUNT: return launch_fast_t<FM_MAX | FM_COUNT, true>(fold, il, g0, g1, p, ch, st);
-        case FM_MIN | FM_COUNT: return launch_fast_t<FM_MIN | FM_COUNT, true>(fold, il, g0, g1, p, ch, st);
-        default: break;
-        }
-    }
-    return launch_fast_t<63, true>(fold, il, g0, g1, p, ch, st);
+    with_fm(fm, times, [&](auto F, auto T) { launch_fast_t<decltype(F)::value, decltype(T)::value>(fold, il, g0, g1, p, ch, st); });
+}
+void launch_fix_edges_fold(int fm, bool times, const DirP &d, const QueryP &p, const ChunkP &ch, cudaStream_t st) {
+    const unsigned grid = (unsigned)(((size_t)((ch.series_end - ch.series_begin + 31) / 32) * ch.J * 32 + 127) / 128);
+    with_fm(fm, times, [&](auto F, auto T) { k_fix_edges_fold<decltype(F)::value, decltype(T)::value><<<grid, 128, 0, st>>>(d, p, ch); });
 }
 
 template <int NCOL, int NCALL> void launch_multi_t(const QueryP &p, const DirP &d, const ChunkP &ch, uint32_t nseg, cudaStream_t st) {
@@ -596,7 +604,7 @@
     q->plan = pl;
     size_t cells_dense = (size_t)q->n_groups * p.n_buckets;
     for (uint32_t c = 0; c < p.n_calls; c++) {
-        bool sel = p.calls[c].func >= OG_AGG_MIN && !(p.multi && p.calls[c].func <= OG_AGG_MAX);
+        const bool sel = call_has_time(p, c);
         if ((rc = dalloc(&q->dense[c].val, cells_dense))) return rc;
         if ((rc = dalloc(&q->dense[c].ok, cells_dense))) return rc;
         if (sel && (rc = dalloc(&q->dense[c].tim, cells_dense))) return rc;
@@ -670,7 +678,7 @@
     ch.J = ic ? ic->J : 0;
     size_t chunk_cells = (size_t)std::min(q->chunk_series, s->n_series) * p.n_buckets;
     for (uint32_t c = 0; c < p.n_calls; c++) {
-        bool sel = p.calls[c].func >= OG_AGG_MIN;
+        const bool sel = call_has_time(p, c);
         if ((rc = salloc(q, &ch.cells[c].val, chunk_cells))) return rc;
         if ((rc = salloc(q, &ch.cells[c].ok, chunk_cells))) return rc;
         if (sel && (rc = salloc(q, &ch.cells[c].tim, chunk_cells))) return rc;
@@ -686,7 +694,7 @@
         ch.gc_cols = (std::min(q->chunk_series, s->n_series) + OG_MERGE_SB - 1) / OG_MERGE_SB;
         const size_t n = (size_t)p.n_buckets * ch.gc_cols;
         for (uint32_t c = 0; c < p.n_calls; c++) {
-            bool sel = p.calls[c].func >= OG_AGG_MIN;
+            const bool sel = call_has_time(p, c);
             if ((rc = salloc(q, &ch.gcells[c].val, n))) return rc;
             if ((rc = salloc(q, &ch.gcells[c].ok, n))) return rc;
             if (sel && (rc = salloc(q, &ch.gcells[c].tim, n))) return rc;
@@ -697,7 +705,7 @@
         ch.gc_cols = ch.gc_edge0 + (s->n_series + 31) / 32;
         const size_t n = (size_t)p.n_buckets * ch.gc_cols;
         for (uint32_t c = 0; c < p.n_calls; c++) {
-            bool sel = p.calls[c].func >= OG_AGG_MIN;
+            const bool sel = call_has_time(p, c);
             if ((rc = salloc(q, &ch.gcells[c].val, n))) return rc;
             if ((rc = salloc(q, &ch.gcells[c].ok, n))) return rc;
             if (sel && (rc = salloc(q, &ch.gcells[c].tim, n))) return rc;
@@ -709,7 +717,7 @@
         pl->fm = 0; pl->times = false;
         for (uint32_t c = 0; c < p.n_calls; c++) {
             pl->fm |= 1 << (p.calls[c].func - 1);
-            if (p.calls[c].func >= OG_AGG_MIN && !(p.multi && p.calls[c].func <= OG_AGG_MAX)) pl->times = true;
+            if (call_has_time(p, c)) pl->times = true;
         }
         pl->fm |= FM_COUNT;
         q->path_used = pl->fold ? 3 : 2;
@@ -823,7 +831,7 @@
         }
         CU(cudaEventRecord(q->main_ev[2 * chunks_run + 1], st));
         chunks_run++;
-        if (pl->fold) k_fix_edges_fold<<<(unsigned)(((size_t)((b - a + 31) / 32) * ch.J * 32 + 127) / 128), 128, 0, st>>>(dir, p, ch);
+        if (pl->fold) launch_fix_edges_fold(pl->fm, pl->times, dir, p, ch, st);
         else k_fix_edges<<<(nseg + 127) / 128, 128, 0, st>>>(dir, p, ch);
         if (per_series) k_merge_per_series<<<dim3((unsigned)((chunk_cells + 255) / 256), p.n_calls), 256, 0, st>>>(p, ch, gp);
         else if (pl->blockmerge) k_merge_all_blocks<<<dim3((p.n_buckets + 127) / 128, (b - a + OG_MERGE_SB - 1) / OG_MERGE_SB, p.n_calls), 128, 0, st>>>(p, ch, gp);
diff --git a/opengemini_b200/csrc/fused.cuh b/opengemini_b200/csrc/fused.cuh
--- a/opengemini_b200/csrc/fused.cuh
+++ b/opengemini_b200/csrc/fused.cuh
@@ -41,14 +41,15 @@
 
     __device__ __forceinline__ void flush(bool final) {
         if (cur_b == OG_NO_BUCKET) return;
-        size_t e = 2 * (size_t)(seg - ch.seg_begin);
         if (!head_done) {
+            const size_t e = edge_idx(ch, series, seg, 0);
 #pragma unroll
             for (int c = 0; c < NC; c++) store_part(ch.edges[c], e, parts[c]);
             head_done = true; head_b = cur_b;
         } else if (final) {
+            const size_t et = edge_idx(ch, series, seg, 1);
 #pragma unroll
-            for (int c = 0; c < NC; c++) store_part(ch.edges[c], e + 1, parts[c]);
+            for (int c = 0; c < NC; c++) store_part(ch.edges[c], et, parts[c]);
         } else {
 #pragma unroll
             for (int c = 0; c < NC; c++) if (parts[c].ok) store_cell(ch, c, series, cur_b, parts[c]);
@@ -82,15 +83,16 @@
     uint32_t i = blockIdx.x * blockDim.x + threadIdx.x;
     if (i >= n) return;
     uint32_t seg = list ? list[i] : ch.seg_begin + i;
-    size_t e = 2 * (size_t)(seg - ch.seg_begin);
+    const uint32_t series = d.seg_series[seg];
+    const size_t e = edge_idx(ch, series, seg, 0), et = edge_idx(ch, series, seg, 1);
     uint32_t rows = d.seg_rows[seg];
     if (d.seg_tmax[seg] < q.tmin || d.seg_tmin[seg] > q.tmax || rows == 0) {
-        ch.edge_bucket[e] = OG_NO_BUCKET; ch.edge_bucket[e + 1] = OG_NO_BUCKET; return;
+        ch.edge_bucket[e] = OG_NO_BUCKET; ch.edge_bucket[et] = OG_NO_BUCKET; return;
     }
     size_t ti_idx = (size_t)d.n_columns * d.n_segments + seg;
     TimeDesc td;
     int rc = parse_time_page(d.data + d.page_off[ti_idx], d.page_len[ti_idx], td);
-    if (rc != D_OK) { report_err(ch.err, rc, seg); ch.edge_bucket[e] = OG_NO_BUCKET; ch.edge_bucket[e + 1] = OG_NO_BUCKET; return; }
+    if (rc != D_OK) { report_err(ch.err, rc, seg); ch.edge_bucket[e] = OG_NO_BUCKET; ch.edge_bucket[et] = OG_NO_BUCKET; return; }
     int col = q.col_index[0], type = q.col_type[0];
     size_t pi = (size_t)col * d.n_segments + seg;
     uint32_t len = d.page_len[pi];
@@ -98,11 +100,11 @@
     if (len == 0) { h.rows = rows; h.nil_count = rows; h.bitmap = nullptr; h.bm_off = 0; h.block = nullptr; h.block_len = 0; h.one_row = 0; }
     else {
         rc = parse_field_header(d.data + d.page_off[pi], len, type, rows, h);
-        if (rc != D_OK) { report_err(ch.err, rc, seg); ch.edge_bucket[e] = OG_NO_BUCKET; ch.edge_bucket[e + 1] = OG_NO_BUCKET; return; }
+        if (rc != D_OK) { report_err(ch.err, rc, seg); ch.edge_bucket[e] = OG_NO_BUCKET; ch.edge_bucket[et] = OG_NO_BUCKET; return; }
     }
     FusedState<NC> st(q, ch, h);
     st.ti.init(td);
-    st.seg = seg; st.series = d.seg_series[seg]; st.row = 0; st.cur_b = OG_NO_BUCKET; st.head_b = OG_NO_BUCKET; st.we = 0; st.head_done = false;
+    st.seg = seg; st.series = series; st.row = 0; st.cur_b = OG_NO_BUCKET; st.head_b = OG_NO_BUCKET; st.we = 0; st.head_done = false;
     if (h.nil_count < h.rows) {
         rc = decode_block(type, h, st);
         if (rc != D_OK) report_err(ch.err, rc, seg);
@@ -112,7 +114,7 @@
     bool single = !st.head_done;
     st.flush(true);
     ch.edge_bucket[e] = st.head_b;
-    ch.edge_bucket[e + 1] = (single || st.head_b == OG_NO_BUCKET) ? OG_NO_BUCKET : last_b;
+    ch.edge_bucket[et] = (single || st.head_b == OG_NO_BUCKET) ? OG_NO_BUCKET : last_b;
 }
 
 }
diff --git a/opengemini_b200/csrc/fused_cols.cuh b/opengemini_b200/csrc/fused_cols.cuh
--- a/opengemini_b200/csrc/fused_cols.cuh
+++ b/opengemini_b200/csrc/fused_cols.cuh
@@ -180,7 +180,7 @@
             if (j >= nm) break;
             if (SIMPLE) { parts[j].t = 0; parts[j].ok = cnt != 0; parts[j].v = op[j] == 0 ? cnt : op[j] == 1 ? d2u(fsum) : isum; }
             if (w == 0) store_part(ch.edges[mc[j]], sg.e, parts[j]);
-            else if (final) store_part(ch.edges[mc[j]], sg.e + 1, parts[j]);
+            else if (final) store_part(ch.edges[mc[j]], sg.e + edge_tail_off(ch), parts[j]);
             else if (parts[j].ok) store_cell(ch, mc[j], sg.series, cur_b, parts[j]);
         }
         w++;
@@ -229,9 +229,9 @@
     ColsSeg sg;
     sg.seg = ch.seg_begin + i;
     if (sg.seg >= ch.seg_end) return;
-    sg.e = 2 * (size_t)(sg.seg - ch.seg_begin);
     sg.rows = d.seg_rows[sg.seg]; sg.series = d.seg_series[sg.seg];
-    auto no_rows = [&]() { ch.edge_bucket[sg.e] = OG_NO_BUCKET; ch.edge_bucket[sg.e + 1] = OG_NO_BUCKET; };
+    sg.e = edge_idx(ch, sg.series, sg.seg, 0);
+    auto no_rows = [&]() { ch.edge_bucket[sg.e] = OG_NO_BUCKET; ch.edge_bucket[sg.e + edge_tail_off(ch)] = OG_NO_BUCKET; };
     if (d.seg_tmax[sg.seg] < q.tmin || d.seg_tmin[sg.seg] > q.tmax || sg.rows == 0) { no_rows(); return; }
     const size_t ti_idx = (size_t)d.n_columns * d.n_segments + sg.seg;
     TimeDesc td;
@@ -274,7 +274,7 @@
         for (int k = 0; k < (int)q.n_cols; k++) cols_column<0, SIMPLE>(d, q, ch, sg, k, keep);
     }
     ch.edge_bucket[sg.e] = sg.b_first;
-    ch.edge_bucket[sg.e + 1] = b_last == sg.b_first ? OG_NO_BUCKET : b_last;
-}
-
-}
+    ch.edge_bucket[sg.e + edge_tail_off(ch)] = b_last == sg.b_first ? OG_NO_BUCKET : b_last;
+}
+
+}
diff --git a/opengemini_b200/csrc/fused_il.cuh b/opengemini_b200/csrc/fused_il.cuh
--- a/opengemini_b200/csrc/fused_il.cuh
+++ b/opengemini_b200/csrc/fused_il.cuh
@@ -22,7 +22,6 @@
     return false;
 }
 
-enum { FM_COUNT = 1, FM_SUM = 2, FM_MIN = 4, FM_MAX = 8, FM_FIRST = 16, FM_LAST = 32 };
 enum { SEG_GENERAL = 0, SEG_FAST = 1, SEG_RAWX = 2 };
 
 #ifndef OG_FAST_THREADS
@@ -129,7 +128,6 @@
     const uint32_t seg = il.lane_seg[slot];
     bool active = seg != OG_IL_NONE && seg >= ch.seg_begin && seg < ch.seg_end;
     if (!__any_sync(FULL, active)) return;
-    const size_t e = 2 * (size_t)(seg - ch.seg_begin);
 
     uint32_t rows = 0, series = 0, r_lo = 0, r_hi = 0; bool rawx = false;
     int64_t t0 = 0, dt = 1; uint64_t dtu = 1; double inv_dt = 1.0;
@@ -142,7 +140,7 @@
         r_lo = 0; r_hi = rows - 1;
         if (t0 < q.tmin) { uint64_t k = udiv_est((uint64_t)(q.tmin - t0) + dtu - 1, dtu, inv_dt); r_lo = k > rows ? rows : (uint32_t)k; }
         { int64_t t_last = t0 + (int64_t)(rows - 1) * dt; if (t_last > q.tmax) { if (q.tmax < t0) r_lo = rows; else r_hi = (uint32_t)udiv_est((uint64_t)(q.tmax - t0), dtu, inv_dt); } }
-        if (r_lo > r_hi || r_lo >= rows) { ch.edge_bucket[e] = OG_NO_BUCKET; ch.edge_bucket[e + 1] = OG_NO_BUCKET; active = false; }
+        if (r_lo > r_hi || r_lo >= rows) { ch.edge_bucket[edge_idx(ch, series, seg, 0)] = OG_NO_BUCKET; ch.edge_bucket[edge_idx(ch, series, seg, 1)] = OG_NO_BUCKET; active = false; }
     }
     if (!__any_sync(FULL, active)) return;
 
@@ -237,12 +235,18 @@
         for (uint32_t c = 0; c < q.n_calls; c++) {
             const Part pp = part_of(q.calls[c].func, cnt);
             if (kind == 2) { if (pp.ok) store_cell(ch, (int)c, series, cur_b, pp); }
-            else store_part(ch.edges[c], e + kind, pp);
+            else {
+                const Tri &ed = ch.edges[c]; const size_t i = edge_idx(ch, series, seg, kind);
+                ed.val[i] = pp.v; ed.ok[i] = (uint8_t)pp.ok;
+                if (TIMES && ed.tim) ed.tim[i] = pp.t;
+            }
         }
         if (kind == 0) { head_done = true; head_b = cur_b; }
     };
     auto flush_fold = [&](bool ev) {
         uint32_t pend = __ballot_sync(FULL, ev);
+        const bool multi = q.multi != 0;
+        const bool mm_time = TIMES && !multi;
 #pragma unroll 1
         while (pend) {
             const int leader = __ffs(pend) - 1;
@@ -250,15 +254,22 @@
             const bool mine = ev && cur_b == bL;
             const uint32_t cnt = mine ? stop - w_row0 : 0;
             const uint32_t w = bL - b0;
-#pragma unroll 1
-            for (uint32_t c = 0; c < q.n_calls; c++) {
-                const int func = q.calls[c].func, ftype = func == OG_AGG_COUNT ? OG_TYPE_INT : q.calls[c].type;
-                const bool wt = func >= OG_AGG_MIN && !(q.multi && func <= OG_AGG_MAX);
-                Part pp = fold32(func, ftype, q.multi != 0, part_of(func, cnt), wt);
-                if ((int)lane == leader && pp.ok) {
+            Part f[6];
+            f[0] = fold32(OG_AGG_COUNT, OG_TYPE_INT, multi, part_of(OG_AGG_COUNT, cnt), false);
+            if (FM & FM_SUM) f[1] = fold32(OG_AGG_SUM, OG_TYPE_FLOAT, multi, part_of(OG_AGG_SUM, cnt), false);
+            if (FM & FM_MIN) f[2] = fold32(OG_AGG_MIN, OG_TYPE_FLOAT, multi, part_of(OG_AGG_MIN, cnt), mm_time);
+            if (FM & FM_MAX) f[3] = fold32(OG_AGG_MAX, OG_TYPE_FLOAT, multi, part_of(OG_AGG_MAX, cnt), mm_time);
+            if (FM & FM_FIRST) f[4] = fold32(OG_AGG_FIRST, OG_TYPE_FLOAT, multi, part_of(OG_AGG_FIRST, cnt), true);
+            if (FM & FM_LAST) f[5] = fold32(OG_AGG_LAST, OG_TYPE_FLOAT, multi, part_of(OG_AGG_LAST, cnt), true);
+            if ((int)lane == leader && f[0].ok) {
+#pragma unroll 1
+                for (uint32_t c = 0; c < q.n_calls; c++) {
                     const uint32_t i = c * OG_IL_WCAP + w;
                     Part a; a.ok = acc_k[i]; a.v = a.ok ? acc_v[i] : 0; a.t = (TIMES && a.ok) ? acc_t[i] : 0;
-                    group_update(func, ftype, q.multi != 0, a, pp);
+                    with_agg<FM>(q.calls[c].func, [&](auto fc) {
+                        constexpr int func = decltype(fc)::value;
+                        group_update(func, func == OG_AGG_COUNT ? OG_TYPE_INT : OG_TYPE_FLOAT, multi, a, f[func - 1]);
+                    });
                     acc_v[i] = a.v; acc_k[i] = 1; if (TIMES) acc_t[i] = a.t;
                 }
             }
@@ -440,9 +451,9 @@
     }
     if (active) {
         if (bad) report_err(ch.err, D_CORRUPT, seg);
-        ch.edge_bucket[e] = head_b;
-        ch.edge_bucket[e + 1] = (head_b == OG_NO_BUCKET || cur_b == head_b) ? OG_NO_BUCKET : cur_b;
-    }
-}
-
-}
+        ch.edge_bucket[edge_idx(ch, series, seg, 0)] = head_b;
+        ch.edge_bucket[edge_idx(ch, series, seg, 1)] = (head_b == OG_NO_BUCKET || cur_b == head_b) ? OG_NO_BUCKET : cur_b;
+    }
+}
+
+}
diff --git a/opengemini_b200/csrc/fused_multi.cuh b/opengemini_b200/csrc/fused_multi.cuh
--- a/opengemini_b200/csrc/fused_multi.cuh
+++ b/opengemini_b200/csrc/fused_multi.cuh
@@ -145,9 +145,9 @@
     const uint32_t i = blockIdx.x * blockDim.x + threadIdx.x;
     const uint32_t seg = ch.seg_begin + i;
     if (seg >= ch.seg_end) return;
-    const size_t e = 2 * (size_t)(seg - ch.seg_begin);
     const uint32_t rows = d.seg_rows[seg], series = d.seg_series[seg];
-    auto no_rows = [&]() { ch.edge_bucket[e] = OG_NO_BUCKET; ch.edge_bucket[e + 1] = OG_NO_BUCKET; };
+    const size_t e = edge_idx(ch, series, seg, 0), et = edge_idx(ch, series, seg, 1);
+    auto no_rows = [&]() { ch.edge_bucket[e] = OG_NO_BUCKET; ch.edge_bucket[et] = OG_NO_BUCKET; };
     if (d.seg_tmax[seg] < q.tmin || d.seg_tmin[seg] > q.tmax || rows == 0) { no_rows(); return; }
     const size_t ti_idx = (size_t)d.n_columns * d.n_segments + seg;
     TimeDesc td;
@@ -169,7 +169,7 @@
 #pragma unroll
         for (int c = 0; c < NCALL; c++) {
             if (!head_done) store_part(ch.edges[c], e, parts[c]);
-            else if (final) store_part(ch.edges[c], e + 1, parts[c]);
+            else if (final) store_part(ch.edges[c], et, parts[c]);
             else if (parts[c].ok) store_cell(ch, (int)c, series, cur_b, parts[c]);
         }
         if (!head_done) { head_done = true; head_b = cur_b; }
@@ -233,7 +233,7 @@
     const bool single = !head_done;
     flush(true);
     ch.edge_bucket[e] = head_b;
-    ch.edge_bucket[e + 1] = (single || head_b == OG_NO_BUCKET) ? OG_NO_BUCKET : last_b;
+    ch.edge_bucket[et] = (single || head_b == OG_NO_BUCKET) ? OG_NO_BUCKET : last_b;
 }
 
 }
```

Measured after the change: 711.5 billion (median of 6 runs). 12.0% higher.
